# dsforza96/yocto-hair

Measured on AMD Instinct MI355X. Metric: Msamples/sec (whole node), 720x720x1536spp sphere-hairblock; per-pixel L2 vs CPU ref, higher is better.
Workload: dtype f32

## Files before the change

### include/yhair.h

```cpp
#ifndef YHAIR_H_
#define YHAIR_H_

#include <stdint.h>

#ifdef __cplusplus
extern "C" {
#endif

#define YH_OK 0
#define YH_E_INVALID -1
#define YH_E_DEVICE -2
#define YH_E_STATE -3
#define YH_E_IO -4
#define YH_E_SELFTEST -5


typedef struct yh_shape {
  int          num_vertices;
  const float* positions;
  const float* normals;
  const float* radius;
  int          num_lines;
  const int*   lines;
  int          num_triangles;
// ... 40 lines not shown
  float        emission[3];
  int          tex_width, tex_height;
  const float* texels;
} yh_environment;

typedef struct yh_camera {
  float frame[12];
  float lens;
  float film[2];
  float focus;
  float aperture;
} yh_camera;

typedef struct yh_scene_desc {
  int                   num_shapes;
  const yh_shape*       shapes;
  int                   num_materials;
  const yh_material*    materials;
  int                   num_objects;
  const yh_object*      objects;
  int                   num_environments;
  const yh_environment* environments;
  yh_camera             camera;
  int                   num_textures;
  const yh_texture*     textures;
} yh_scene_desc;

enum {
  YH_SHADER_NAIVE    = 0,
  YH_SHADER_PATH     = 1,
  YH_SHADER_EYELIGHT = 2,
  YH_SHADER_NORMAL   = 3,
  YH_SHADER_COUNT    = 4
};

typedef struct yh_trace_params {
  int      resolution;
  int      bounces;
  float    clamp;
  uint64_t seed;
  int      shader;
  int      hair_exact;
} yh_trace_params;

typedef struct yh_workcounts {
  uint64_t samples;
  uint64_t rays;
  uint64_t nodes;
  uint64_t seg_tests;
  uint64_t tri_tests;
  uint64_t hair_shades;
  uint64_t surf_shades;
  uint64_t env_lookups;
  uint64_t env_samples;
  uint64_t cyc_trace, cyc_shade, ticks_tile, wave_iters, wave_steps, lane_steps, lane_iters;
  uint64_t cyc_geom, cyc_sample, cyc_eval, cyc_rest;
  uint64_t branch[10];
} yh_workcounts;

typedef struct yh_context yh_context;


yh_context* yh_create(int device);
void        yh_destroy(yh_context* ctx);
const char* yh_last_error(const yh_context* ctx);
const char* yh_version(void);


int yh_upload_scene(yh_context* ctx, const yh_scene_desc* scene);
int yh_upload_scene_maps(yh_context* ctx, const yh_scene_desc* scene, const yh_material_maps* maps);

int yh_init_state(yh_context* ctx, const yh_trace_params* params);
int yh_image_size(const yh_context* ctx, int* width, int* height);

int yh_set_shard(yh_context* ctx, int rank, int world);

int yh_trace_samples(yh_context* ctx, int nsamples);
int yh_trace_samples_async(yh_context* ctx, int nsamples);
int yh_synchronize(yh_context* ctx);

int yh_download(yh_context* ctx, float* rgba);
int yh_pack_tiles_device(yh_context* ctx, void* device_rgba, int64_t capacity,
    int64_t* count);
int yh_unpack_tiles_device(yh_context* ctx, const void* device_packed,
    int src_rank, int world, void* device_image);
int64_t yh_shard_pixels(const yh_context* ctx, int rank, int world);

int yh_gather_framebuffer(yh_context** contexts, int n, float* rgba);

int yh_download_rng(yh_context* ctx, uint64_t* state_inc);

int yh_trace_samples_counted(yh_context* ctx, int nsamples, yh_workcounts* out);

int yh_last_trace_ms(const yh_context* ctx, float* ms, int* launches);

int yh_launch_shape(const yh_context* ctx);
int yh_kernel_trials(const yh_context* ctx, double* ms_per_sample, int* trials, int count);
int yh_trials_pending(const yh_context* ctx);
int         yh_set_trial_cache_dir(const char* dir);
const char* yh_default_trial_cache_dir(void);

int yh_tile_costs(yh_context* ctx, uint32_t* ticks, int count);
int yh_item_costs(yh_context* ctx, uint32_t* costs, int count);


#define YH_HAIR_BRDF_FLOATS 30

enum {
  YH_LOBE_DIFFUSE            = 0,
  YH_LOBE_SPECULAR           = 1,
  YH_LOBE_METAL              = 2,
  YH_LOBE_TRANSMISSION       = 3,
  YH_LOBE_REFRACTION         = 4,
  YH_LOBE_DELTA_SPECULAR     = 5,
  YH_LOBE_DELTA_METAL        = 6,
  YH_LOBE_DELTA_TRANSMISSION = 7,
  YH_LOBE_DELTA_REFRACTION   = 8,
  YH_LOBE_COUNT              = 9
};
#define YH_SURFACE_BSDF_FLOATS 29

int yh_hair_brdf_batch(yh_context* ctx, int n, const yh_material* materials,
    const float* v, const float* normal, const float* tangent, float* brdf);
int yh_hair_eval_batch(yh_context* ctx, int n, const float* brdf,
    const float* outgoing, const float* incoming, float* f);
int yh_hair_sample_batch(yh_context* ctx, int n, const float* brdf,
    const float* outgoing, const float* rn, float* incoming);
int yh_hair_pdf_batch(yh_context* ctx, int n, const float* brdf,
    const float* outgoing, const float* incoming, float* pdf);
int yh_hair_eval_pdf_batch(yh_context* ctx, int n, const float* brdf,
    const float* outgoing, const float* incoming, float* pdf);

int yh_curves_to_lines(yh_context* ctx, int n, const float* P, const float* width0,
    const float* width1, int base_vertex, float* positions, float* normals,
    float* radius, int* lines);

int yh_bvh_build(int n, const float* boxes, float* nodes, int* primitives);
int yh_bvh_build_wide(int n, const float* boxes, int width, float* slots);

int yh_bvh_build_gpu(yh_context* ctx, int n, const float* boxes, float* nodes, int* primitives);
int yh_bvh_build_wide_gpu(yh_context* ctx, int n, const float* boxes, int width, float* slots);

int yh_surface_lobe_batch(yh_context* ctx, int kind, int n, const float* params,
    const float* normal, const float* outgoing, const float* incoming,
    const float* rn, float* out);
int yh_surface_bsdf_batch(yh_context* ctx, int n, const yh_material* materials,
    const float* normal, const float* outgoing, const float* incoming,
    const float* rn, float* out);
int yh_intersect_batch(yh_context* ctx, int n, const float* rays, int* object,
    int* element, float* uv, float* distance);

int yh_selftest(yh_context* ctx, int which, float* worst);

typedef struct yh_scene_file yh_scene_file;
yh_scene_file*       yh_scene_load(const char* json_path, const char* camera,
          char* error, int error_len);
const yh_scene_desc* yh_scene_get(const yh_scene_file* scene);
const yh_material_maps* yh_scene_get_maps(const yh_scene_file* scene);
void                 yh_scene_free(yh_scene_file* scene);
int yh_save_image(const char* path, int width, int height, const float* rgba,
    char* error, int error_len);

#ifdef __cplusplus
}
#endif
#endif
```

### yocto-hair_amd/csrc/dev_hair.h

```cpp
#ifndef YH_DEV_HAIR_H_
#define YH_DEV_HAIR_H_
#include "dev_math.h"

namespace yhd {

constexpr int p_max = 3;

struct hair_hit {
  float h, gamma_o;
  frame w2b;
};

#ifndef YH_HAIR_FAST
#define YH_HAIR_FAST 1
#endif
#define YH_FAST_DIV YH_HAIR_FAST
#define YH_FAST_EXP 0
#define YH_FAST_LOG YH_HAIR_FAST
#define YH_FAST_TRIG YH_HAIR_FAST
#define YH_FAST_ASIN YH_HAIR_FAST
YH_DEV float h_rcp(float x) { return YH_FAST_DIV ? __builtin_amdgcn_rcpf(x) : 1 / x; }
YH_DEV float h_div(float a, float b) { return YH_FAST_DIV ? a * __builtin_amdgcn_rcpf(b) : a / b; }
YH_DEV float h_div_n(float a, float b) {
  if (!YH_FAST_DIV) return a / b;
  float r = __builtin_amdgcn_rcpf(b);
  r       = __builtin_fmaf(__builtin_fmaf(-b, r, 1.0f), r, r);
  return a * r;
}
YH_DEV float h_sqrt(float x) { return YH_FAST_DIV ? __builtin_amdgcn_sqrtf(x) : sqrtf(x); }
YH_DEV float h_exp(float x) { return YH_FAST_EXP ? __builtin_amdgcn_exp2f(x * 1.44269504f) : expf(x); }
YH_DEV float h_log(float x) { return YH_FAST_LOG ? __builtin_amdgcn_logf(x) * 0.693147181f : logf(x); }
YH_DEV float h_sin(float x) { return YH_FAST_TRIG ? __builtin_amdgcn_sinf(x * 0.159154943f) : sinf(x); }
YH_DEV float h_cos(float x) { return YH_FAST_TRIG ? __builtin_amdgcn_cosf(x * 0.159154943f) : cosf(x); }
YH_DEV float h_cos_turns(float t) { return YH_FAST_TRIG ? __builtin_amdgcn_cosf(t) : cosf(2 * pif * t); }
YH_DEV float h_asin(float x) { return YH_FAST_ASIN ? asinf(x) : (float)asin((double)x); }
YH_DEV f3    h_normalize(f3 a) {
  if (!YH_FAST_DIV) return normalize(a);
  float l2 = dot(a, a);
  return l2 != 0 ? a * __builtin_amdgcn_rsqf(l2) : a;
}
YH_DEV f3 h_div(f3 a, float b) { float r = h_rcp(b); return YH_FAST_DIV ? a * r : a / b; }
YH_DEV f3 h_transform_direction(const frame& a, f3 b) { return h_normalize(transform_vector(a, b)); }

YH_DEV float d_rcp(float x) { return 1 / x; }
YH_DEV float d_div(float a, float b) { return a / b; }
YH_DEV float d_sqrt(float x) { return sqrtf(x); }
YH_DEV float d_safe_sqrt(float x) { return d_sqrt(fmax_(0.0f, x)); }
YH_DEV float d_log(float x) { return logf(x); }
YH_DEV float d_sin(float x) { return sinf(x); }
YH_DEV float d_cos(float x) { return cosf(x); }
YH_DEV float d_cos_turns(float t) { return cosf(2 * pif * t); }
YH_DEV f3    d_transform_direction(const frame& a, f3 b) { return normalize(transform_vector(a, b)); }

YH_DEV float sqr(float v) { return v * v; }
YH_DEV float safe_asin(float x) { return h_asin(fclamp(x, -1.0f, 1.0f)); }
YH_DEV float safe_sqrt(float x) { return h_sqrt(fmax_(0.0f, x)); }
YH_DEV float exact_safe_sqrt(float x) { return sqrtf(fmax_(0.0f, x)); }

template <bool QUAD = false>
YH_DEV hair_hit hair_setup(float v, f3 normal, f3 tangent) {
  hair_hit hh;
  hh.h       = -1 + 2 * v;
  hh.gamma_o = safe_asin(hh.h);
  f3 z       = QUAD ? quad_normalize(normal) : normalize(normal);
  f3 x       = QUAD ? quad_orthonormalize(tangent, z) : orthonormalize(tangent, z);
  f3 y       = QUAD ? quad_normalize(cross(z, x)) : normalize(cross(z, x));
  hh.w2b     = transpose_rot(frame{x, y, z, mk3(0.0f)});
  return hh;
}

YH_DEV float i0(float x) {
  const float den[10] = {1.0f, 4.0f, 64.0f, 2304.0f, 147456.0f, 14745600.0f,
      2123366400.0f, 416179814400.0f, 106542032486400.0f, 34519618525593600.0f};
  float val = 0, x2i = 1;
#pragma unroll
  for (int i = 0; i < 10; i++) {
    val += YH_FAST_DIV ? x2i * (1.0f / den[i]) : x2i / den[i];
    x2i *= x * x;
  }
  return val;
}
YH_DEV float log_i0(float x) {
  if (x > 12)
    return x + 0.5f * (-logf(2 * pif) + logf(1 / x) + 1 / (8 * x));
  else
    return logf(i0(x));
}
YH_DEV float mp(const yhd_material& m, int p, float cos_theta_i, float cos_theta_o,
    float sin_theta_i, float sin_theta_o) {
  float v = m.v[p];
  float a = cos_theta_i * cos_theta_o / v;
  float b = sin_theta_i * sin_theta_o / v;
  if (v <= 0.1f) {
    return h_exp(log_i0(a) - b - m.inv_v[p] + 0.6931f + m.log_inv_2v[p]);
  } else {
    if (YH_HAIR_FAST) return h_div(h_exp(-b) * i0(a), (float)m.mp_den[p]);
    return (float)((double)(expf(-b) * i0(a)) / m.mp_den[p]);
  }
}
YH_DEV float fresnel_dielectric_cos(float eta, float cosw_) {
  float cosw  = fabs_(cosw_);
  float sin2  = 1 - cosw * cosw;
  float eta2  = eta * eta;
  float cos2t = 1 - sin2 / eta2;
  if (cos2t < 0) return 1;
  float t0 = sqrtf(cos2t);
  float t1 = eta * t0;
  float t2 = eta * cosw;
  float rs = (cosw - t1) / (cosw + t1);
  float rp = (t0 - t2) / (t0 + t2);
  return (rs * rs + rp * rp) / 2;
}
YH_DEV float h_fresnel_dielectric_cos(float eta, float cosw_) {
  float cosw  = fabs_(cosw_);
  float sin2  = 1 - cosw * cosw;
  float eta2  = eta * eta;
  float cos2t = 1 - h_div(sin2, eta2);
  if (cos2t < 0) return 1;
  float t0 = h_sqrt(cos2t);
  float t1 = eta * t0;
  float t2 = eta * cosw;
  float rs = h_div(cosw - t1, cosw + t1);
  float rp = h_div(t0 - t2, t0 + t2);
  return (rs * rs + rp * rp) / 2;
}
YH_DEV void ap(float cos_theta_o, float eta, float h, f3 T, f3 out[p_max + 1]) {
  float cos_gamma_o = safe_sqrt(1 - h * h);
  float cos_theta   = cos_theta_o * cos_gamma_o;
  float f = h_fresnel_dielectric_cos(eta, 0.0f * 0.0f + 0.0f * 0.0f + 1.0f * cos_theta);
  out[0]  = mk3(f);
  out[1]  = sqr(1 - f) * T;
  out[2]  = out[1] * T * f;
  f3 den  = mk3(1.f) - T * f;
  f3 num  = out[2] * f * T;
  out[3]  = f3{h_div(num.x, den.x), h_div(num.y, den.y), h_div(num.z, den.z)};
}
YH_DEV f3 transmittance(const yhd_material& m, float h, float sin_theta_o, float cos_theta_o,
    float& gamma_t) {
  float sin_theta_t = h_div(sin_theta_o, m.eta);
  float cos_theta_t = safe_sqrt(1 - sqr(sin_theta_t));
  float etap        = d_div(d_sqrt(m.eta * m.eta - sqr(sin_theta_o)), cos_theta_o);
  float sin_gamma_t = d_div(h, etap);
  float cos_gamma_t = safe_sqrt(1 - sqr(sin_gamma_t));
  gamma_t           = safe_asin(sin_gamma_t);
  float k           = h_div_n(2 * cos_gamma_t, cos_theta_t);
  f3    sa          = ld3(m.sigma_a);
  return f3{h_exp(-sa.x * k), h_exp(-sa.y * k), h_exp(-sa.z * k)};
}
YH_DEV float phi_fn(int p, float gamma_o, float gamma_t) {
  return 2 * p * gamma_t - 2 * gamma_o + p * pif;
}
YH_DEV float np(const yhd_material& m, float phi, int p, float gamma_o, float gamma_t) {
  float dphi = phi - phi_fn(p, gamma_o, gamma_t);
  while (dphi > pif) dphi -= 2 * pif;
  while (dphi < -pif) dphi += 2 * pif;
  float x = fabs_(dphi);
  float e = h_exp(-h_div_n(x, m.s));
  return h_div(h_div(e, m.s * sqr(1 + e)), m.tl_norm);
}
YH_DEV void tilt(const yhd_material& m, int p, float sin_theta_o, float cos_theta_o,
    float& sin_theta_op, float& cos_theta_op) {
  if (p == 0) {
    sin_theta_op = sin_theta_o * m.cos_2k_alpha[1] - cos_theta_o * m.sin_2k_alpha[1];
    cos_theta_op = cos_theta_o * m.cos_2k_alpha[1] + sin_theta_o * m.sin_2k_alpha[1];
  } else if (p == 1) {
    sin_theta_op = sin_theta_o * m.cos_2k_alpha[0] + cos_theta_o * m.sin_2k_alpha[0];
    cos_theta_op = cos_theta_o * m.cos_2k_alpha[0] - sin_theta_o * m.sin_2k_alpha[0];
  } else if (p == 2) {
    sin_theta_op = sin_theta_o * m.cos_2k_alpha[2] + cos_theta_o * m.sin_2k_alpha[2];
    cos_theta_op = cos_theta_o * m.cos_2k_alpha[2] - sin_theta_o * m.sin_2k_alpha[2];
  } else {
    sin_theta_op = sin_theta_o;
    cos_theta_op = cos_theta_o;
  }
}
YH_DEV void compute_ap_pdf(const yhd_material& m, float h, float cos_theta_o,
    float ap_pdf[p_max + 1]) {
  float sin_theta_o = safe_sqrt(1 - cos_theta_o * cos_theta_o);
  float gamma_t;
  f3    T = transmittance(m, h, sin_theta_o, cos_theta_o, gamma_t);
  f3    apv[p_max + 1];
  ap(cos_theta_o, m.eta, h, T, apv);
  float sum_y = 0.0f;
#pragma unroll
  for (int i = 0; i <= p_max; i++) sum_y += luminance(apv[i]);
#pragma unroll
  for (int i = 0; i <= p_max; i++) ap_pdf[i] = h_div(luminance(apv[i]), sum_y);
}

template <bool WANT_F, bool WANT_PDF>
YH_DEV void hair_eval_pdf(const yhd_material& m, const hair_hit& hh, f3 outgoing_, f3 incoming_,
    f3& f, float& pdf) {
  f3    outgoing    = transform_direction(hh.w2b, outgoing_);
  f3    incoming    = transform_direction(hh.w2b, incoming_);
  float sin_theta_o = outgoing.x;
  float cos_theta_o = exact_safe_sqrt(1 - sqr(sin_theta_o));
  float phi_o       = atan2f(outgoing.z, outgoing.y);
  float sin_theta_i = incoming.x;
  float cos_theta_i = exact_safe_sqrt(1 - sqr(sin_theta_i));
  float phi_i       = atan2f(incoming.z, incoming.y);
  float gamma_t;
  f3    T   = transmittance(m, hh.h, sin_theta_o, cos_theta_o, gamma_t);
  float phi = phi_i - phi_o;
  f3    apv[p_max + 1];
  float ap_pdf[p_max + 1];
  if (WANT_F) ap(cos_theta_o, m.eta, hh.h, T, apv);
  if (WANT_PDF) compute_ap_pdf(m, hh.h, cos_theta_o, ap_pdf);
  f   = mk3(0.0f);
  pdf = 0.0f;
#pragma unroll
  for (int p = 0; p < p_max; p++) {
    float sin_theta_op, cos_theta_op;
    tilt(m, p, sin_theta_o, cos_theta_o, sin_theta_op, cos_theta_op);
    cos_theta_op = fabs_(cos_theta_op);
    float mpv    = mp(m, p, cos_theta_i, cos_theta_op, sin_theta_i, sin_theta_op);
    float npv    = np(m, phi, p, hh.gamma_o, gamma_t);
    if (WANT_F) f = f + mpv * apv[p] * npv;
    if (WANT_PDF) pdf += mpv * ap_pdf[p] * npv;
  }
  float mpl = mp(m, p_max, cos_theta_i, cos_theta_o, sin_theta_i, sin_theta_o);
  if (WANT_F) f = f + h_div(mpl * apv[p_max], 2 * pif);
  if (WANT_PDF) pdf += mpl * ap_pdf[p_max] * (1 / (2 * pif));
}

struct hair_out {
  float sin_theta_o, cos_theta_o, phi_o, gamma_t;
  f3    ap0, ap1, ap2, ap3;
  float pdf0, pdf1, pdf2, pdf3;
};
template <bool QUAD = false>
YH_DEV hair_out hair_prepare(const yhd_material& m, const hair_hit& hh, f3 outgoing_) {
  hair_out o;
  f3 outgoing   = QUAD ? quad_normalize(transform_vector(hh.w2b, outgoing_)) : transform_direction(hh.w2b, outgoing_);
  o.sin_theta_o = outgoing.x;
  o.cos_theta_o = exact_safe_sqrt(1 - sqr(o.sin_theta_o));
  o.phi_o       = atan2f(outgoing.z, outgoing.y);
  if (QUAD) {
    const bool for_pdf = (__lane_id() & 2u) != 0;
    float      st      = for_pdf ? safe_sqrt(1 - o.cos_theta_o * o.cos_theta_o) : o.sin_theta_o;
    float      gt;
    f3         T = transmittance(m, hh.h, st, o.cos_theta_o, gt);
    f3         a[p_max + 1];
    ap(o.cos_theta_o, m.eta, hh.h, T, a);
    float l0 = luminance(a[0]), l1 = luminance(a[1]), l2 = luminance(a[2]), l3 = luminance(a[3]);
    float sum_y = 0.0f + l0 + l1 + l2 + l3;
    o.gamma_t = quad_bcast_f<0>(gt);
    o.ap0 = f3{quad_bcast_f<0>(a[0].x), quad_bcast_f<0>(a[0].y), quad_bcast_f<0>(a[0].z)};
    o.ap1 = f3{quad_bcast_f<0>(a[1].x), quad_bcast_f<0>(a[1].y), quad_bcast_f<0>(a[1].z)};
    o.ap2 = f3{quad_bcast_f<0>(a[2].x), quad_bcast_f<0>(a[2].y), quad_bcast_f<0>(a[2].z)};
    o.ap3 = f3{quad_bcast_f<0>(a[3].x), quad_bcast_f<0>(a[3].y), quad_bcast_f<0>(a[3].z)};
    o.pdf0 = quad_bcast_f<2>(h_div(l0, sum_y)), o.pdf1 = quad_bcast_f<2>(h_div(l1, sum_y));
    o.pdf2 = quad_bcast_f<2>(h_div(l2, sum_y)), o.pdf3 = quad_bcast_f<2>(h_div(l3, sum_y));
    return o;
  }
  f3 T          = transmittance(m, hh.h, o.sin_theta_o, o.cos_theta_o, o.gamma_t);
  f3    apv[p_max + 1];
  float ap_pdf[p_max + 1];
  ap(o.cos_theta_o, m.eta, hh.h, T, apv);
  compute_ap_pdf(m, hh.h, o.cos_theta_o, ap_pdf);
  o.ap0 = apv[0], o.ap1 = apv[1], o.ap2 = apv[2], o.ap3 = apv[3];
  o.pdf0 = ap_pdf[0], o.pdf1 = ap_pdf[1], o.pdf2 = ap_pdf[2], o.pdf3 = ap_pdf[3];
  return o;
}

YH_DEV void hair_eval_pdf_quad(const yhd_material& m, const hair_hit& hh, const hair_out& ho, f3 incoming_,
    f3& f, float& pdf) {
  const int p       = (int)(__lane_id() & 3u);
  f3    incoming    = quad_normalize(transform_vector(hh.w2b, incoming_));
  float sin_theta_o = ho.sin_theta_o, cos_theta_o = ho.cos_theta_o;
  float sin_theta_i = incoming.x;
  float cos_theta_i = exact_safe_sqrt(1 - sqr(sin_theta_i));
  float phi_i       = atan2f(incoming.z, incoming.y);
  float phi         = phi_i - ho.phi_o;
  float sin_theta_op, cos_theta_op;
  tilt(m, p, sin_theta_o, cos_theta_o, sin_theta_op, cos_theta_op);
  if (p < p_max) cos_theta_op = fabs_(cos_theta_op);
  float mpv  = mp(m, p, cos_theta_i, cos_theta_op, sin_theta_i, sin_theta_op);
  float npv  = p < p_max ? np(m, phi, p, hh.gamma_o, ho.gamma_t) : 0.0f;
  const f3    a0 = ho.ap0, a1 = ho.ap1, a2 = ho.ap2, a3 = ho.ap3;
  const float q0 = ho.pdf0, q1 = ho.pdf1, q2 = ho.pdf2, q3 = ho.pdf3;
  const bool  is0 = p == 0, is1 = p == 1, is2 = p == 2;
  f3    apq  = f3{is0 ? a0.x : is1 ? a1.x : is2 ? a2.x : a3.x, is0 ? a0.y : is1 ? a1.y : is2 ? a2.y : a3.y,
      is0 ? a0.z : is1 ? a1.z : is2 ? a2.z : a3.z};
  float appq = is0 ? q0 : is1 ? q1 : is2 ? q2 : q3;
  f3    tf   = p < p_max ? mpv * apq * npv : h_div(mpv * apq, 2 * pif);
  float tp   = p < p_max ? mpv * appq * npv : mpv * appq * (1 / (2 * pif));
  f   = mk3(0.0f);
  pdf = 0.0f;
  f   = f + f3{quad_bcast_f<0>(tf.x), quad_bcast_f<0>(tf.y), quad_bcast_f<0>(tf.z)};
  pdf += quad_bcast_f<0>(tp);
  f   = f + f3{quad_bcast_f<1>(tf.x), quad_bcast_f<1>(tf.y), quad_bcast_f<1>(tf.z)};
  pdf += quad_bcast_f<1>(tp);
  f   = f + f3{quad_bcast_f<2>(tf.x), quad_bcast_f<2>(tf.y), quad_bcast_f<2>(tf.z)};
  pdf += quad_bcast_f<2>(tp);
  f   = f + f3{quad_bcast_f<3>(tf.x), quad_bcast_f<3>(tf.y), quad_bcast_f<3>(tf.z)};
  pdf += quad_bcast_f<3>(tp);
}
YH_DEV void hair_eval_pdf_lane(const yhd_material& m, const hair_hit& hh, const hair_out& ho, f3 incoming_,
    f3& f, float& pdf) {
  f3    incoming    = normalize(transform_vector(hh.w2b, incoming_));
  float sin_theta_o = ho.sin_theta_o, cos_theta_o = ho.cos_theta_o;
  float sin_theta_i = incoming.x;
  float cos_theta_i = exact_safe_sqrt(1 - sqr(sin_theta_i));
  float phi_i       = atan2f(incoming.z, incoming.y);
  float phi         = phi_i - ho.phi_o;
  f   = mk3(0.0f);
  pdf = 0.0f;
  const f3    apv[p_max]  = {ho.ap0, ho.ap1, ho.ap2};
  const float appv[p_max] = {ho.pdf0, ho.pdf1, ho.pdf2};
#pragma unroll
  for (int p = 0; p < p_max; p++) {
    float sin_theta_op, cos_theta_op;
    tilt(m, p, sin_theta_o, cos_theta_o, sin_theta_op, cos_theta_op);
    cos_theta_op = fabs_(cos_theta_op);
    float mpv    = mp(m, p, cos_theta_i, cos_theta_op, sin_theta_i, sin_theta_op);
    float npv    = np(m, phi, p, hh.gamma_o, ho.gamma_t);
    f            = f + mpv * apv[p] * npv;
    pdf += mpv * appv[p] * npv;
  }
  float mpl = mp(m, p_max, cos_theta_i, cos_theta_o, sin_theta_i, sin_theta_o);
  f         = f + h_div(mpl * ho.ap3, 2 * pif);
  pdf += mpl * ho.pdf3 * (1 / (2 * pif));
}
YH_DEV void hair_eval_pdf_quad(const yhd_material& m, const hair_hit& hh, f3 outgoing_, f3 incoming_,
    f3& f, float& pdf) {
  hair_out ho = hair_prepare<true>(m, hh, outgoing_);
  hair_eval_pdf_quad(m, hh, ho, incoming_, f, pdf);
}

YH_DEV uint32_t compact1by1(uint32_t x) {
  x &= 0x55555555;
  x = (x ^ (x >> 1)) & 0x33333333;
  x = (x ^ (x >> 2)) & 0x0f0f0f0f;
  x = (x ^ (x >> 4)) & 0x00ff00ff;
  x = (x ^ (x >> 8)) & 0x0000ffff;
  return x;
}
YH_DEV void demux_float(float f, float& a, float& b) {
  uint64_t v = (uint64_t)(f * 4294967296.0f);
  a          = (float)compact1by1((uint32_t)v) / 65536.0f;
  b          = (float)compact1by1((uint32_t)(v >> 1)) / 65536.0f;
}

YH_DEV f3 hair_sample(const yhd_material& m, const hair_hit& hh, const hair_out& ho, float rnx, float rny) {
  float sin_theta_o = ho.sin_theta_o, cos_theta_o = ho.cos_theta_o, phi_o = ho.phi_o;
  float u00, u01, u10, u11;
  demux_float(rnx, u00, u01);
  demux_float(rny, u10, u11);
  int   p  = 0;
  float u1 = u00 - ho.pdf0, u2 = u1 - ho.pdf1;
  if (!(u00 < ho.pdf0)) p = !(u1 < ho.pdf1) ? (!(u2 < ho.pdf2) ? 3 : 2) : 1;
  float sin_theta_op, cos_theta_op;
  tilt(m, p, sin_theta_o, cos_theta_o, sin_theta_op, cos_theta_op);
  u10 = fmax_(u10, 1e-5f);
  float vp = 0, em2v = 0;
  vp   = p == 0 ? m.v[0] : p == 1 ? m.v[1] : m.v[2];
  em2v = p == 0 ? m.exp_m2_inv_v[0] : p == 1 ? m.exp_m2_inv_v[1] : m.exp_m2_inv_v[2];
  float cos_theta   = 1 + vp * d_log(u10 + (1 - u10) * em2v);
  float sin_theta   = d_safe_sqrt(1 - sqr(cos_theta));
  float cos_phi     = d_cos_turns(u11);
  float sin_theta_i = -cos_theta * sin_theta_op + sin_theta * cos_phi * cos_theta_op;
  float cos_theta_i = d_safe_sqrt(1 - sqr(sin_theta_i));
  float dphi;
  if (p < p_max) {
    float x = -m.s * d_log(d_rcp(u01 * m.tl_norm + m.tl_cdf_a) - 1);
    dphi    = phi_fn(p, hh.gamma_o, ho.gamma_t) + fclamp(x, -pif, pif);
  } else {
    dphi = 2 * pif * u01;
  }
  float phi_i    = phi_o + dphi;
  f3    incoming = f3{sin_theta_i, cos_theta_i * d_cos(phi_i), cos_theta_i * d_sin(phi_i)};
  return d_transform_direction(transpose_rot(hh.w2b), incoming);
}
YH_DEV f3 hair_sample(const yhd_material& m, const hair_hit& hh, f3 outgoing_, float rnx, float rny) {
  hair_out ho = hair_prepare(m, hh, outgoing_);
  return hair_sample(m, hh, ho, rnx, rny);
}

YH_DEV void derive_material(yhd_material& m) {
#pragma unroll
  for (int p = 0; p <= p_max; p++) {
    m.inv_v[p]        = 1 / m.v[p];
    m.log_inv_2v[p]   = logf(1 / (2 * m.v[p]));
    m.exp_m2_inv_v[p] = expf(-2 / m.v[p]);
    m.mp_den[p]       = sinh((double)(1 / m.v[p])) * 2 * m.v[p];
  }
  float cb   = 1 / (1 + expf(-pif / m.s));
  float ca   = 1 / (1 + expf(-(-pif) / m.s));
  m.tl_cdf_a = ca;
  m.tl_norm  = cb - ca;
}

}
#endif
```

### yocto-hair_amd/csrc/dev_path.h

```cpp
#ifndef YH_DEV_PATH_H_
#define YH_DEV_PATH_H_
#include "dev_hair.h"
#include "dev_surface.h"
#include "dev_trace.h"
#if YH_LANE
#include "dev_lane.h"
#endif

namespace yhd {

YH_DEV ray_t sample_camera(const yhd_camera& cam, int i, int j, int w, int h, float pu, float pv,
    float lu, float lv) {
  const unsigned int ql = __lane_id() & 3u;
  float uvq = (ql == 0 ? (float)i + pu : (float)j + pv) / (ql == 0 ? (float)w : (float)h);
  float uvx = quad_bcast_f<0>(uvq), uvy = quad_bcast_f<1>(uvq);
  f3    q  = {cam.film_x * (0.5f - uvx), cam.film_y * (uvy - 0.5f), cam.lens};
  f3    dc = -quad_normalize(q);
  f3    e  = mk3(0.0f);
  if (cam.aperture != 0) {
    float r   = sqrtf(lv);
    float phi = 2 * pif * lu;
    float lx = cosf(phi) * r, ly = sinf(phi) * r;
    e = f3{lx * cam.aperture / 2, ly * cam.aperture / 2, 0};
  }
  f3    p  = quad_div(dc * cam.focus, fabs_(dc.z));
  f3    d  = quad_normalize(p - e);
  frame f  = ldframe(cam.frame);
  return mkray(transform_point(f, e), quad_normalize(transform_vector(f, d)));
}

YH_DEV ray_t sample_camera_lane(const yhd_camera& cam, int i, int j, int w, int h, float pu, float pv, float lu, float lv) {
  float uvx = ((float)i + pu) / (float)w, uvy = ((float)j + pv) / (float)h;
  f3    q   = {cam.film_x * (0.5f - uvx), cam.film_y * (uvy - 0.5f), cam.lens};
  f3    dc  = -normalize(q);
  f3    e   = mk3(0.0f);
  if (cam.aperture != 0) {
    float r   = sqrtf(lv);
    float phi = 2 * pif * lu;
    float lx = cosf(phi) * r, ly = sinf(phi) * r;
    e = f3{lx * cam.aperture / 2, ly * cam.aperture / 2, 0};
  }
  f3    p = (dc * cam.focus) / fabs_(dc.z);
  f3    d = normalize(p - e);
  frame f = ldframe(cam.frame);
  return mkray(transform_point(f, e), normalize(transform_vector(f, d)));
}

YH_DEV f3 transform_normal(const frame& a, f3 b) { return normalize(transform_vector(a, b)); }
YH_DEV f3 quad_transform_normal(const frame& a, f3 b) { return quad_normalize(transform_vector(a, b)); }

YH_DEV f3 eval_position(const yhd_scene& sc, const yhd_object& o, int element, float u, float v) {
  frame    fr = ldframe(o.frame);
  yhd_int4 e  = sc.elems[o.elem_base + element];
  if (o.kind == YH_KIND_TRIANGLES) {
    f3 p0 = xyz(sc.vpos[o.vert_base + e.x]), p1 = xyz(sc.vpos[o.vert_base + e.y]),
       p2 = xyz(sc.vpos[o.vert_base + e.z]);
    return transform_point(fr, p0 * (1 - u - v) + p1 * u + p2 * v);
  } else {
    f3 p0 = xyz(sc.vpos[o.vert_base + e.x]), p1 = xyz(sc.vpos[o.vert_base + e.y]);
    return transform_point(fr, p0 * (1 - u) + p1 * u);
  }
}

struct hit_geom {
  f3 position, normal, element_normal;
};
YH_DEV hit_geom eval_hit(const yhd_scene& sc, const yhd_object& o, int slot, float u, float v) {
  frame    fr = ldframe(o.frame);
  hit_geom g;
  if (o.kind == YH_KIND_TRIANGLES) {
    const yhd_float4* rec = sc.prims + (size_t)o.prim_base + (size_t)slot * 6;
    f3 p0 = xyz(ldg4(rec)), p1 = xyz(ldg4(rec + 1)), p2 = xyz(ldg4(rec + 2));
    g.position       = transform_point(fr, p0 * (1 - u - v) + p1 * u + p2 * v);
    g.element_normal = quad_transform_normal(fr, quad_normalize(cross(p1 - p0, p2 - p0)));
    if (o.has_normals) {
      f3 n0 = xyz(ldg4(rec + 3)), n1 = xyz(ldg4(rec + 4)), n2 = xyz(ldg4(rec + 5));
      g.normal = quad_transform_normal(fr, quad_normalize(n0 * (1 - u - v) + n1 * u + n2 * v));
    } else {
      g.normal = g.element_normal;
    }
  } else {
    const yhd_float4* rec = sc.prims + (size_t)o.prim_base + (size_t)slot * 4;
    f3 p0 = xyz(ldg4(rec)), p1 = xyz(ldg4(rec + 1));
    g.position       = transform_point(fr, p0 * (1 - u) + p1 * u);
    g.element_normal = quad_transform_normal(fr, quad_normalize(p1 - p0));
    if (o.has_normals) {
      f3 n0 = xyz(ldg4(rec + 2)), n1 = xyz(ldg4(rec + 3));
      g.normal = quad_transform_normal(fr, quad_normalize(n0 * (1 - u) + n1 * u));
    } else {
      g.normal = g.element_normal;
    }
  }
  return g;
}

YH_DEV f3 eval_env_texture(const yhd_scene& sc, const yhd_environment& env, float u_, float v_) {
  if (env.tex_w == 0) return mk3(1.0f);
  int   sx = env.tex_w, sy = env.tex_h;
  float s = fmodf(u_, 1.0f) * sx;
  if (s < 0) s += sx;
  float t = fmodf(v_, 1.0f) * sy;
  if (t < 0) t += sy;
  int   i = iclamp((int)s, 0, sx - 1), j = iclamp((int)t, 0, sy - 1);
  int   ii = (i + 1) % sx, jj = (j + 1) % sy;
  float u = s - i, v = t - j;
  const yhd_float4* tx = sc.env_texels + env.texel_base;
  f3 a = xyz(tx[(size_t)j * sx + i]), b = xyz(tx[(size_t)jj * sx + i]);
  f3 c = xyz(tx[(size_t)j * sx + ii]), d = xyz(tx[(size_t)jj * sx + ii]);
  return a * (1 - u) * (1 - v) + b * (1 - u) * v + c * u * (1 - v) + d * u * v;
}
template <bool COUNT>
YH_DEV f3 eval_environment(const trace_ctx& tc, f3 dir) {
  const yhd_scene& sc = *tc.sc;
  f3 emission = mk3(0.0f);
  for (int k = 0; k < sc.num_environments; k++) {
    const yhd_environment& env = sc.environments[k];
    if (COUNT) count_quad<COUNT>(tc.stats->envl);
    if (env.tex_w == 0) {
      emission = emission + ld3(env.emission) * mk3(1.0f);
      continue;
    }
    f3    wl = transform_direction(ldframe(env.inv_frame), dir);
    float tx = atan2f(wl.z, wl.x) / (2 * pif);
    float ty = acosf(fclamp(wl.y, -1.0f, 1.0f)) / pif;
    if (tx < 0) tx += 1;
    emission = emission + ld3(env.emission) * eval_env_texture(sc, env, tx, ty);
  }
  return emission;
}

template <typename P>
YH_DEV int cdf_upper_bound(P cdf, int lo, int len, float r) {
  while (len > 0) {
    int half = len >> 1;
    if (!(r < cdf[lo + half])) {
      lo += half + 1;
      len -= half + 1;
    } else {
      len = half;
    }
  }
  return lo;
}
template <typename P>
YH_DEV int sample_discrete_cdf(P cdf, int n, float r) {
  float back = cdf[n - 1];
  r          = fclamp(r * back, 0.0f, back - 0.00001f);
  return iclamp(cdf_upper_bound(cdf, 0, n, r), 0, n - 1);
}
YH_DEV int sample_discrete_cdf_indexed(const float* cdf, int n, const YH_LDS float* tab, int K, int S, float r) {
  float back = tab[K - 1];
  r          = fclamp(r * back, 0.0f, back - 0.00001f);
  int k      = cdf_upper_bound(tab, 0, K, r);
  if (k >= K) return n - 1;
  int lo = k * S;
  return iclamp(cdf_upper_bound(cdf, lo, min(S, n - lo), r), 0, n - 1);
}

YH_DEV void object_frames(const trace_ctx& tc, int object, frame& fr, frame& inv) {
  if (tc.lds_scene) {
    const YH_LDS v4f* ob = tc.lds_scene + YH_OBJECT_F4 * object;
    v4f a = ob[0], b = ob[1], c = ob[2], d = ob[3], e = ob[4], g = ob[5];
    fr.x = {a.x, a.y, a.z}, fr.y = {a.w, b.x, b.y}, fr.z = {b.z, b.w, c.x}, fr.o = {c.y, c.z, c.w};
    inv.x = {d.x, d.y, d.z}, inv.y = {d.w, e.x, e.y}, inv.z = {e.z, e.w, g.x}, inv.o = {g.y, g.z, g.w};
  } else {
    const yhd_object& o = tc.sc->objects[object];
    fr = ldframe(o.frame), inv = ldframe(o.inv_frame);
  }
}
YH_DEV bool small_light_hit(const YH_LDS v4f* L, const frame& inv, f3 ro, f3 rd, int& slot, float& uu, float& vv) {
  f3  lo = transform_point(inv, ro), ld = transform_vector(inv, rd);
  f3  ldinv = quad_rcp(ld);
  v4f b0 = L[0], b1 = L[1];
  if (!intersect_bbox(lo, ldinv, ray_eps, flt_max, xyz(b0), xyz(b1))) return false;
  const int num  = __float_as_int(b0.w);
  float     tmax = flt_max;
  bool      hit  = false;
  for (int i = 0; i < num; i++) {
    float u = 0, v = 0, d = 0;
    if (intersect_triangle(lo, ld, ray_eps, tmax, xyz(L[2 + 3 * i]), xyz(L[3 + 3 * i]), xyz(L[4 + 3 * i]), u, v, d)) hit = true, slot = i, uu = u, vv = v, tmax = d;
  }
  return hit;
}

template <bool COUNT, bool BIG_LIGHTS>
YH_DEV f3 sample_lights(const trace_ctx& tc, f3 position, float rl, float rel, float ruvx,
    float ruvy) {
  const yhd_scene& sc = *tc.sc;
  int n        = sc.num_lights;
  int light_id = iclamp((int)(rl * n), 0, n - 1);
  const yhd_light& light = sc.lights[light_id];
  if (light.object >= 0 && (!BIG_LIGHTS || (light.small_base >= 0 && tc.lds_lights))) {
    const YH_LDS v4f* L = tc.lds_lights + light.small_base;
    int   element = sample_discrete_cdf((const YH_LDS float*)(L + 14), light.cdf_count, rel);
    int   rec     = 0;
    for (int i = 1; i < __float_as_int(L[0].w); i++)
      if (__float_as_int(L[2 + 3 * i].w) == element) rec = i;
    float su = sqrtf(ruvx);
    float u = 1 - su, v = ruvy * su;
    frame fr, inv;
    object_frames(tc, light.object, fr, inv);
    f3 p0 = xyz(L[2 + 3 * rec]), p1 = xyz(L[3 + 3 * rec]), p2 = xyz(L[4 + 3 * rec]);
    f3 lposition = transform_point(fr, p0 * (1 - u - v) + p1 * u + p2 * v);
    return normalize(lposition - position);
  } else if (BIG_LIGHTS && light.object >= 0) {
    int   element = sample_discrete_cdf(sc.light_cdf + light.cdf_base, light.cdf_count, rel);
    float su      = sqrtf(ruvx);
    float u = 1 - su, v = ruvy * su;
    f3 lposition = eval_position(sc, sc.objects[light.object], element, u, v);
    return normalize(lposition - position);
  } else if (light.environment >= 0) {
    const yhd_environment& env = sc.environments[light.environment];
    if (env.tex_w) {
      if (COUNT) count_quad<COUNT>(tc.stats->envs);
      int   idx = (tc.lds_envtab && light_id == sc.env_tab_light)
                      ? sample_discrete_cdf_indexed(sc.light_cdf + light.cdf_base, light.cdf_count, tc.lds_envtab, sc.env_tab_k, sc.env_tab_stride, rel)
                      : sample_discrete_cdf(sc.light_cdf + light.cdf_base, light.cdf_count, rel);
      float ux  = (idx % env.tex_w + 0.5f) / env.tex_w;
      float uy  = (idx / env.tex_w + 0.5f) / env.tex_h;
      return transform_direction(ldframe(env.frame),
          f3{cosf(ux * 2 * pif) * sinf(uy * pif), cosf(uy * pif), sinf(ux * 2 * pif) * sinf(uy * pif)});
    } else {
      float z   = 2 * ruvy - 1;
      float r   = sqrtf(fclamp(1 - z * z, 0.0f, 1.0f));
      float phi = 2 * pif * ruvx;
      return f3{r * cosf(phi), r * sinf(phi), z};
    }
  }
  return mk3(0.0f);
}

template <bool COUNT, int STRIDE, bool BIG_LIGHTS>
YH_DEV float sample_lights_pdf(const trace_ctx& tc, f3 position, f3 direction) {
  const yhd_scene& sc = *tc.sc;
  float pdf = 0.0f;
  for (int k = 0; k < sc.num_lights; k++) {
    const yhd_light& light = sc.lights[k];
    if (light.object >= 0 && (!BIG_LIGHTS || (light.small_base >= 0 && tc.lds_lights))) {
      const YH_LDS v4f* L = tc.lds_lights + light.small_base;
      frame fr, inv;
      object_frames(tc, light.object, fr, inv);
      const float area = L[1].w;
      float lpdf = 0.0f;
      f3    next_position = position;
      for (int bounce = 0; bounce < 100; bounce++) {
        int   slot = 0;
        float uu = 0, vv = 0;
        if (!small_light_hit(L, inv, next_position, direction, slot, uu, vv)) break;
        f3 p0 = xyz(L[2 + 3 * slot]), p1 = xyz(L[3 + 3 * slot]), p2 = xyz(L[4 + 3 * slot]);
        f3 lposition = transform_point(fr, p0 * (1 - uu - vv) + p1 * uu + p2 * vv);
        f3 lnormal   = quad_transform_normal(fr, quad_normalize(cross(p1 - p0, p2 - p0)));
        f3 dp        = lposition - position;
        lpdf += dot(dp, dp) / (fabs_(dot(lnormal, direction)) * area);
        next_position = lposition + direction * 1e-3f;
      }
      pdf += lpdf;
    } else if (BIG_LIGHTS && light.object >= 0) {
      const yhd_object& o = sc.objects[light.object];
      float lpdf = 0.0f;
      f3    next_position = position;
      for (int bounce = 0; bounce < 100; bounce++) {
        hit_t isec;
#if YH_LANE
        isec = lane_trace(tc, *tc.ls, next_position, direction, light.object);
#else
        isec = trace_ray<COUNT, STRIDE>(tc, mkray(next_position, direction), light.object);
#endif
        if (isec.object < 0) break;
        hit_geom lg        = eval_hit(sc, o, isec.slot, isec.u, isec.v);
        f3       lposition = lg.position;
        f3       lnormal   = lg.element_normal;
        float area      = sc.light_cdf[light.cdf_base + light.cdf_count - 1];
        f3    dp        = lposition - position;
        lpdf += dot(dp, dp) / (fabs_(dot(lnormal, direction)) * area);
        next_position = lposition + direction * 1e-3f;
      }
      pdf += lpdf;
    } else if (light.environment >= 0) {
      const yhd_environment& env = sc.environments[light.environment];
      if (env.tex_w) {
        f3    wl = transform_direction(ldframe(env.inv_frame), direction);
        float tx = atan2f(wl.z, wl.x) / (2 * pif);
        float ty = acosf(fclamp(wl.y, -1.0f, 1.0f)) / pif;
        if (tx < 0) tx += 1;
        int   i   = iclamp((int)(tx * env.tex_w), 0, env.tex_w - 1);
        int   j   = iclamp((int)(ty * env.tex_h), 0, env.tex_h - 1);
        int   idx = j * env.tex_w + i;
        const float* cdf = sc.light_cdf + light.cdf_base;
        float prob = (idx == 0 ? cdf[0] : cdf[idx] - cdf[idx - 1]) / cdf[light.cdf_count - 1];
        float angle = (2 * pif / env.tex_w) * (pif / env.tex_h) * sinf(pif * (j + 0.5f) / env.tex_h);
        pdf += prob / angle;
      } else {
        pdf += 1 / (4 * pif);
      }
    }
  }
  pdf *= (float)1 / (float)sc.num_lights;
  return pdf;
}

#if YH_LANE
struct lane_lights_pdf_result {
  float pdf;
  int   base;
};
__device__ __attribute__((noinline)) lane_lights_pdf_result lane_lights_pdf_general(const yhd_scene* sc, const YH_LDS v4f* lds_scene, const YH_LDS v4f* lds_lights,
    const YH_LDS float* lds_envtab, YH_LDS unsigned int* lds, unsigned int* ovf, int sp, int base, f3 position, f3 direction) {
  trace_ctx tc;
  tc.sc = sc, tc.sc_dev = sc, tc.lds_stack = nullptr, tc.lds_scene = lds_scene, tc.stats = nullptr;
  tc.lds_lights = lds_lights, tc.lds_envtab = lds_envtab, tc.lds_mats = nullptr;
  lane_stack s;
  s.lds = lds, s.ovf = ovf, s.sp = sp, s.base = base;
  tc.ls = &s;
  const float pdf = sample_lights_pdf<false, 64, true>(tc, position, direction);
  return lane_lights_pdf_result{pdf, s.base};
}
template <bool GENERAL>
YH_DEV float lane_lights_pdf(const trace_ctx& tc, f3 position, f3 direction) {
  if constexpr (GENERAL) {
    const lane_lights_pdf_result r = lane_lights_pdf_general(tc.sc_dev, tc.lds_scene, tc.lds_lights, tc.lds_envtab, tc.ls->lds, tc.ls->ovf, tc.ls->sp, tc.ls->base, position, direction);
    tc.ls->base = r.base;
    return r.pdf;
  } else {
    return sample_lights_pdf<false, 64, false>(tc, position, direction);
  }
}
#endif

struct path_t {
  ray_t ray;
  f3    radiance, weight;
  int   bounce;
  bool  hit;
  bool   in_medium;
  vsdf_t medium;
#if YH_LANE
  yhd_float4* medium_mem;
#endif
};

YH_DEV bool path_continue(path_t& ps, rng_t& rng, int bounces) {
  if (is_zero(ps.weight) || !finite3(ps.weight)) return false;
  if (ps.bounce > 3) {
    float rr_prob = fmin_(0.99f, hmax(ps.weight));
    if (rand1f(rng) >= rr_prob) return false;
    ps.weight = ps.weight * (1 / rr_prob);
  }
  ps.bounce++;
  return ps.bounce < bounces;
}

YH_DEV void eval_texcoord(const yhd_scene& sc, const yhd_object& o, const hit_t& isec, float& tu, float& tv) {
  tu = isec.u, tv = isec.v;
  if (!o.has_texcoords) return;
  const bool lines   = o.kind == YH_KIND_LINES;
  int        element = __float_as_int(lines ? sc.prims[(size_t)o.prim_base + (size_t)isec.slot * 4 + 2].w
                                            : sc.prims[(size_t)o.prim_base + (size_t)isec.slot * 6].w);
  yhd_int4   e       = sc.elems[o.elem_base + element];
  const float* t0 = sc.vtex + 2 * (size_t)(o.vert_base + e.x);
  const float* t1 = sc.vtex + 2 * (size_t)(o.vert_base + e.y);
  if (lines) {
    tu = t0[0] * (1 - isec.u) + t1[0] * isec.u, tv = t0[1] * (1 - isec.u) + t1[1] * isec.u;
  } else {
    const float* t2 = sc.vtex + 2 * (size_t)(o.vert_base + e.z);
    tu = t0[0] * (1 - isec.u - isec.v) + t1[0] * isec.u + t2[0] * isec.v;
    tv = t0[1] * (1 - isec.u - isec.v) + t1[1] * isec.u + t2[1] * isec.v;
  }
}

YH_DEV surface_maps eval_maps(const yhd_scene& sc, const yhd_maps& mp, float tu, float tv) {
  surface_maps f;
  if (mp.specular_tex >= 0) f.specular = eval_texture(sc, mp.specular_tex, true, tu, tv).x;
  if (mp.metallic_tex >= 0) f.metallic = eval_texture(sc, mp.metallic_tex, true, tu, tv).x;
  if (mp.roughness_tex >= 0) f.roughness = eval_texture(sc, mp.roughness_tex, true, tu, tv).x;
  if (mp.opacity_tex >= 0) {
    f3 o      = eval_texture(sc, mp.opacity_tex, true, tu, tv);
    f.opacity = mp.opacity * ((o.x + o.y + o.z) / 3);
    if (f.opacity > 0.999f) f.opacity = 1;
  }
  return f;
}

YH_DEV f3 eval_normalmap(const yhd_scene& sc, const yhd_object& o, const hit_t& isec, f3 normal, int normal_tex, float tu, float tv) {
  f3 nm = eval_texture(sc, normal_tex, true, tu, tv);
  nm    = f3{-1 + 2 * nm.x, -1 + 2 * nm.y, -1 + 2 * nm.z};
  f3 tgu = mk3(0.0f), tgv = mk3(0.0f);
  if (o.has_texcoords) {
    const yhd_float4* rec = sc.prims + (size_t)o.prim_base + (size_t)isec.slot * 6;
    const yhd_float4  r0  = rec[0];
    yhd_int4          e   = sc.elems[o.elem_base + __float_as_int(r0.w)];
    f3 p0 = xyz(r0), p1 = xyz(rec[1]), p2 = xyz(rec[2]);
    const float* t0 = sc.vtex + 2 * (size_t)(o.vert_base + e.x);
    const float* t1 = sc.vtex + 2 * (size_t)(o.vert_base + e.y);
    const float* t2 = sc.vtex + 2 * (size_t)(o.vert_base + e.z);
    f3    p = p1 - p0, q = p2 - p0;
    float sx = t1[0] - t0[0], sy = t2[0] - t0[0];
    float tx = t1[1] - t0[1], ty = t2[1] - t0[1];
    float div = sx * ty - sy * tx;
    f3    u = {1, 0, 0}, v = {0, 1, 0};
    if (div != 0) {
      u = f3{ty * p.x - tx * q.x, ty * p.y - tx * q.y, ty * p.z - tx * q.z} / div;
      v = f3{sx * q.x - sy * p.x, sx * q.y - sy * p.y, sx * q.z - sy * p.z} / div;
    }
    frame fr = ldframe(o.frame);
    tgu = transform_direction(fr, u), tgv = transform_direction(fr, v);
  }
  frame f;
  f.z = normal;
  f.x = orthonormalize(tgu, f.z);
  f.y = normalize(cross(f.z, f.x));
  nm.y *= dot(f.y, tgv) < 0 ? 1.0f : -1.0f;
  return normalize(transform_vector(f, nm));
}

struct hit_maps {
  float        tu, tv;
  bool         have_tc;
  surface_maps f;
};
YH_DEV hit_maps eval_hit_maps(const yhd_scene& sc, const yhd_object& o, const hit_t& isec, bool mapped, f3& nrm) {
  hit_maps h;
  h.tu = isec.u, h.tv = isec.v, h.have_tc = false;
  if (!mapped || !sc.maps) return h;
  const yhd_maps mp = sc.maps[o.material];
  if (!mp.any) return h;
  eval_texcoord(sc, o, isec, h.tu, h.tv);
  h.have_tc = true;
  if (mp.normal_tex >= 0 && o.kind == YH_KIND_TRIANGLES) nrm = eval_normalmap(sc, o, isec, nrm, mp.normal_tex, h.tu, h.tv);
  h.f = eval_maps(sc, mp, h.tu, h.tv);
  return h;
}

YH_DEV void medium_crossing(const yhd_scene& sc, path_t& ps, const yhd_material& mat, f3 normal, f3 outgoing,
    f3 incoming, f3 color_tex, float emission_tex_x, float tu, float tv) {
  if (!mat.has_volume || !(dot(normal, outgoing) * dot(normal, incoming) < 0)) return;
  if (!ps.in_medium) {
    if (mat.color_tex >= 0 || mat.emission_tex >= 0) {
      f3    base         = ld3(mat.color) * color_tex;
      float transmission = mat.transmission * emission_tex_x;
      ps.medium.density  = mk3(0.0f);
      if (transmission) {
        f3 c = {fclamp(base.x, 0.0001f, 1.0f), fclamp(base.y, 0.0001f, 1.0f), fclamp(base.z, 0.0001f, 1.0f)};
        ps.medium.density = -f3{logf(c.x), logf(c.y), logf(c.z)} / mat.trdepth;
      }
    } else {
      ps.medium.density = ld3(mat.vol_density);
    }
    ps.medium.scatter    = ld3(mat.vol_scatter) * eval_texture(sc, mat.scattering_tex, false, tu, tv);
    ps.medium.anisotropy = mat.vol_anisotropy;
#if YH_LANE
    ps.medium_mem[0] = yhd_float4{ps.medium.density.x, ps.medium.density.y, ps.medium.density.z, ps.medium.anisotropy};
    ps.medium_mem[1] = yhd_float4{ps.medium.scatter.x, ps.medium.scatter.y, ps.medium.scatter.z, 0.0f};
#endif
  }
  ps.in_medium = !ps.in_medium;
}

template <bool COUNT, int STRIDE, bool GENERAL>
YH_DEV bool path_step(const trace_ctx& tc, path_t& ps, const hit_t& isec, rng_t& rng, int bounces) {
  const yhd_scene& sc = *tc.sc;
  unsigned long long k0 = 0, k1 = 0, k2 = 0, k3 = 0;
  if (COUNT) k0 = clock64();
#if YH_LANE
  if (isec.object < 0) return false;
#else
  if (isec.object < 0) {
    ps.radiance = ps.radiance + ps.weight * eval_environment<COUNT>(tc, ps.ray.d);
    if (COUNT) tc.stats->c_rest += clock64() - k0;
    return false;
  }
#endif
  f3 outgoing = -ps.ray.d;
  if (GENERAL && ps.in_medium) {
#if YH_LANE
    {
      const yhd_float4 m0 = ps.medium_mem[0], m1 = ps.medium_mem[1];
      ps.medium.density = f3{m0.x, m0.y, m0.z}, ps.medium.anisotropy = m0.w, ps.medium.scatter = f3{m1.x, m1.y, m1.z};
    }
#endif
    float rd = rand1f(rng), rl = rand1f(rng);
    float dist = sample_transmittance(ps.medium.density, isec.distance, rl, rd);
    ps.weight  = ps.weight * (eval_transmittance(ps.medium.density, dist) /
                                sample_transmittance_pdf(ps.medium.density, dist, isec.distance));
    if (dist < isec.distance) {
      f3 position = ps.ray.o + ps.ray.d * dist;
      ps.hit      = true;
      f3 incoming;
      if (rand1f(rng) < 0.5f) {
        float rnx = rand1f(rng), rny = rand1f(rng);
        float rnl = rand1f(rng);
        (void)rnl;
        incoming = sample_scattering(ps.medium, outgoing, rnx, rny);
      } else {
        float ruvx = rand1f(rng), ruvy = rand1f(rng);
        float rel = rand1f(rng);
        float rl2 = rand1f(rng);
        incoming  = sample_lights<COUNT, GENERAL>(tc, position, rl2, rel, ruvx, ruvy);
      }
      f3    f         = eval_scattering(ps.medium, outgoing, incoming);
      float pdf       = sample_scattering_pdf(ps.medium, outgoing, incoming);
#if YH_LANE
      float light_pdf = lane_lights_pdf<GENERAL>(tc, position, incoming);
#else
      float light_pdf = sample_lights_pdf<COUNT, STRIDE, GENERAL>(tc, position, incoming);
#endif
      ps.weight = ps.weight * (f / (0.5f * pdf + 0.5f * light_pdf));
      ps.ray    = mkray(position, incoming);
      if (COUNT) tc.stats->c_rest += clock64() - k0;
      return path_continue(ps, rng, bounces);
    }
  }
  constexpr bool from_lds = !GENERAL && (YH_LANE || STRIDE != 64);
  const yhd_object&   o   = !from_lds ? sc.objects[isec.object] : *(const yhd_object*)(const YH_LDS yhd_object*)(tc.lds_scene + YH_OBJECT_F4 * isec.object);
  const yhd_material& mat = !from_lds ? sc.materials[o.material] : *(const yhd_material*)(const YH_LDS yhd_material*)(tc.lds_mats + YH_MATERIAL_F4 * o.material);
  hit_geom hg = eval_hit(sc, o, isec.slot, isec.u, isec.v);
  f3 position = hg.position;
  f3 nrm      = hg.normal;
  hit_maps hm;
  if constexpr (GENERAL) hm = eval_hit_maps(sc, o, isec, !mat.plain, nrm);
  f3 normal;
  bool is_hair = o.kind == YH_KIND_LINES;
  if (is_hair) {
    normal = quad_orthonormalize(outgoing, nrm);
  } else {
    normal = (!mat.thin || dot(nrm, outgoing) >= 0) ? nrm : -nrm;
  }
  if (COUNT) count_quad<COUNT>(is_hair ? tc.stats->hair : tc.stats->surf);
  const bool     general = GENERAL && !mat.plain;
  surface_brdf_t sb;
  float          tu = isec.u, tv = isec.v, etex_x = 1.0f;
  f3             ctex = mk3(1.0f), etex = mk3(1.0f);
  if (general) {
    if constexpr (GENERAL) tu = hm.tu, tv = hm.tv;
    if (mat.color_tex >= 0 || mat.emission_tex >= 0 || mat.scattering_tex >= 0) {
      if constexpr (GENERAL) {
        if (!hm.have_tc) eval_texcoord(sc, o, isec, tu, tv);
      }
      ctex = eval_texture(sc, mat.color_tex, false, tu, tv);
      if (mat.emission_tex >= 0) {
        etex   = eval_texture(sc, mat.emission_tex, false, tu, tv);
        etex_x = eval_texture(sc, mat.emission_tex, true, tu, tv).x;
      }
    }
    if constexpr (GENERAL) sb = surface_brdf(mat, normal, outgoing, ctex, etex_x, hm.f);
    else sb = surface_brdf(mat, normal, outgoing, ctex, etex_x);
    if (sb.opacity < 1 && rand1f(rng) >= sb.opacity) {
      ps.ray = mkray(position + ps.ray.d * 1e-2f, ps.ray.d);
      if (COUNT) tc.stats->c_rest += clock64() - k0;
      return true;
    }
  }
  ps.hit      = true;
  ps.radiance = ps.radiance + ps.weight * (ld3(mat.emission) * etex);
  if (general && is_delta(sb)) {
    f3    incoming = surface_sample_delta(sb, normal, outgoing, rand1f(rng));
    f3    brdfcos;
    float pdf;
    surface_eval_pdf_delta(sb, normal, outgoing, incoming, brdfcos, pdf);
    ps.weight = ps.weight * (brdfcos / pdf);
    medium_crossing(sc, ps, mat, normal, outgoing, incoming, ctex, etex_x, tu, tv);
    ps.ray    = mkray(position, incoming);
    if (COUNT) tc.stats->c_rest += clock64() - k0;
    return path_continue(ps, rng, bounces);
  }
  hair_hit hh;
  hair_out ho;
  if (is_hair) {
    hh = hair_setup<!YH_LANE>(isec.v, normal, nrm);
    ho = hair_prepare<!YH_LANE>(mat, hh, outgoing);
  }

  if (COUNT) k1 = clock64(), tc.stats->c_geom += k1 - k0;
  f3 incoming;
  if (rand1f(rng) < 0.5f) {
    float rnx = rand1f(rng), rny = rand1f(rng);
    float rnl = rand1f(rng);
    if (is_hair) {
      incoming = hair_sample(mat, hh, ho, rnx, rny);
    } else if (general) {
      incoming = surface_sample(sb, normal, outgoing, rnl, rnx, rny);
    } else {
      incoming = mk3(0.0f);
      if (mat.diffuse_pdf != 0 && rnl < 0.0f + mat.diffuse_pdf) {
        if (!(dot(normal, outgoing) <= 0)) incoming = sample_hemisphere_cos(normal, rnx, rny);
      }
    }
  } else {
    float ruvx = rand1f(rng), ruvy = rand1f(rng);
    float rel = rand1f(rng);
    float rl  = rand1f(rng);
    incoming  = sample_lights<COUNT, GENERAL>(tc, position, rl, rel, ruvx, ruvy);
  }
  if (COUNT) k2 = clock64(), tc.stats->c_sample += k2 - k1;
  f3    brdfcos;
  float brdf_pdf;
  if (is_hair) {
#if YH_LANE
    hair_eval_pdf_lane(mat, hh, ho, incoming, brdfcos, brdf_pdf);
#else
    hair_eval_pdf_quad(mat, hh, ho, incoming, brdfcos, brdf_pdf);
#endif
  } else if (general) {
    surface_eval_pdf(sb, normal, outgoing, incoming, brdfcos, brdf_pdf);
  } else {
    brdfcos  = mk3(0.0f);
    brdf_pdf = 0.0f;
    f3 diffuse = ld3(mat.color);
    bool below = dot(normal, incoming) <= 0 || dot(normal, outgoing) <= 0;
    if (!is_zero(diffuse)) {
      f3 lobe = below ? mk3(0.0f) : mk3(1.0f) / pif * dot(normal, incoming);
      brdfcos = brdfcos + diffuse * lobe;
    }
    if (mat.diffuse_pdf != 0) {
      float lobe = 0.0f;
      if (!below) {
        float cosw = dot(normal, incoming);
        lobe       = (cosw <= 0) ? 0 : cosw / pif;
      }
      brdf_pdf += mat.diffuse_pdf * lobe;
    }
  }
  if (COUNT) k3 = clock64(), tc.stats->c_eval += k3 - k2;
#if YH_LANE
  float light_pdf = lane_lights_pdf<GENERAL>(tc, position, incoming);
#else
  float light_pdf = sample_lights_pdf<COUNT, STRIDE, GENERAL>(tc, position, incoming);
#endif
  ps.weight = ps.weight * (brdfcos / (0.5f * brdf_pdf + 0.5f * light_pdf));
  if (general) medium_crossing(sc, ps, mat, normal, outgoing, incoming, ctex, etex_x, tu, tv);
  ps.ray    = mkray(position, incoming);
  if (COUNT) tc.stats->c_rest += clock64() - k3;
  return path_continue(ps, rng, bounces);
}

template <bool COUNT, int STRIDE, int SHADER>
YH_DEV bool shade_step(const trace_ctx& tc, path_t& ps, const hit_t& isec, rng_t& rng, int bounces) {
  const yhd_scene& sc = *tc.sc;
  if (isec.object < 0) {
    f3 env = eval_environment<COUNT>(tc, ps.ray.d);
    if (SHADER == YH_SHADER_NORMAL) ps.radiance = env, ps.hit = true;
    else ps.radiance = ps.radiance + ps.weight * env;
    return false;
  }
  f3 outgoing = -ps.ray.d;
  const yhd_object&   o   = sc.objects[isec.object];
  const yhd_material& mat = sc.materials[o.material];
  hit_geom hg = eval_hit(sc, o, isec.slot, isec.u, isec.v);
  f3   position = hg.position, nrm = hg.normal;
  const hit_maps hm = eval_hit_maps(sc, o, isec, true, nrm);
  bool is_hair  = o.kind == YH_KIND_LINES;
  f3   normal   = is_hair ? quad_orthonormalize(outgoing, nrm) : ((!mat.thin || dot(nrm, outgoing) >= 0) ? nrm : -nrm);
  if (SHADER == YH_SHADER_NORMAL) {
    ps.radiance = normal * 0.5f + mk3(0.5f), ps.hit = true;
    return false;
  }
  if (COUNT) count_quad<COUNT>(is_hair ? tc.stats->hair : tc.stats->surf);
  float tu = hm.tu, tv = hm.tv, etex_x = 1.0f;
  f3    ctex = mk3(1.0f), etex = mk3(1.0f);
  if (mat.color_tex >= 0 || mat.emission_tex >= 0) {
    if (!hm.have_tc) eval_texcoord(sc, o, isec, tu, tv);
    ctex = eval_texture(sc, mat.color_tex, false, tu, tv);
    if (mat.emission_tex >= 0) {
      etex   = eval_texture(sc, mat.emission_tex, false, tu, tv);
      etex_x = eval_texture(sc, mat.emission_tex, true, tu, tv).x;
    }
  }
  surface_brdf_t sb = surface_brdf(mat, normal, outgoing, ctex, etex_x, hm.f);
  if (sb.opacity < 1 && rand1f(rng) >= sb.opacity) {
    ps.ray = mkray(position + ps.ray.d * 1e-2f, ps.ray.d);
    return true;
  }
  ps.hit      = true;
  ps.radiance = ps.radiance + ps.weight * (ld3(mat.emission) * etex);
  hair_hit hh;
  hair_out ho;
  if (is_hair) {
    hh = hair_setup<true>(isec.v, normal, nrm);
    ho = hair_prepare<true>(mat, hh, outgoing);
  }
  f3    incoming, brdfcos;
  float pdf;
  if (SHADER == YH_SHADER_EYELIGHT) {
    if (is_hair) hair_eval_pdf_quad(mat, hh, ho, outgoing, brdfcos, pdf);
    else surface_eval_pdf(sb, normal, outgoing, outgoing, brdfcos, pdf);
    ps.radiance = ps.radiance + ps.weight * pif * brdfcos;
    if (!is_delta(sb)) return false;
    incoming = surface_sample_delta(sb, normal, outgoing, rand1f(rng));
    surface_eval_pdf_delta(sb, normal, outgoing, incoming, brdfcos, pdf);
    ps.weight = ps.weight * (brdfcos / pdf);
    if (is_zero(ps.weight) || !finite3(ps.weight)) return false;
    ps.ray = mkray(position, incoming);
    ps.bounce++;
    return ps.bounce < (bounces > 4 ? bounces : 4);
  }
  if (!is_delta(sb)) {
    float rnx = rand1f(rng), rny = rand1f(rng);
    float rnl = rand1f(rng);
    if (is_hair) {
      incoming = hair_sample(mat, hh, ho, rnx, rny);
      hair_eval_pdf_quad(mat, hh, ho, incoming, brdfcos, pdf);
    } else {
      incoming = surface_sample(sb, normal, outgoing, rnl, rnx, rny);
      surface_eval_pdf(sb, normal, outgoing, incoming, brdfcos, pdf);
    }
  } else {
    incoming = surface_sample_delta(sb, normal, outgoing, rand1f(rng));
    surface_eval_pdf_delta(sb, normal, outgoing, incoming, brdfcos, pdf);
  }
  ps.weight = ps.weight * (brdfcos / pdf);
  ps.ray    = mkray(position, incoming);
  return path_continue(ps, rng, bounces);
}

YH_DEV void path_begin(const yhd_camera& cam, path_t& ps, rng_t& rng, int i, int j, int w, int h) {
  float lu = rand1f(rng), lv = rand1f(rng);
  float pu = rand1f(rng), pv = rand1f(rng);
  ps.ray      = sample_camera(cam, i, j, w, h, pu, pv, lu, lv);
  ps.radiance = mk3(0.0f), ps.weight = mk3(1.0f);
  ps.bounce   = 0;
  ps.hit      = false;
  ps.in_medium = false;
}
YH_DEV void path_end(const path_t& ps, float clamp, yhd_float4& acc) {
  f3 rgb = ps.radiance;
  if (!finite3(rgb)) rgb = mk3(0.0f);
  if (hmax(rgb) > clamp) rgb = rgb * (clamp / hmax(rgb));
  acc.x += rgb.x, acc.y += rgb.y, acc.z += rgb.z, acc.w += ps.hit ? 1.0f : 0.0f;
}

}
#endif
```

### yocto-hair_amd/csrc/kernels.hip

```cpp
#include <hip/hip_runtime.h>

#include <algorithm>
#include <cstdlib>
#include <cstring>

#include "yhair.h"
#include "dev_items.h"

template <int SHADER>
__global__ __launch_bounds__(YH_BLOCK, YH_MIN_WAVES) void k_trace_shader(const yhd_scene sc, const yhd_state st,
    int nsamples, yhd_counters* counters) {
  trace_items<false, true, YH_BLOCK, SHADER>(sc, st, nsamples, counters);
}

__global__ void k_resolve(const yhd_state st, int samples, yhd_float4* image) {
  int lane = threadIdx.x;
  int tile = st.shard_rank + blockIdx.x * st.shard_world;
  int i    = (tile % st.tiles_x) * YH_TILE + (lane & 7);
  int j    = (tile / st.tiles_x) * YH_TILE + (lane >> 3);
  if (i >= st.width || j >= st.height) return;
  size_t     pix = (size_t)j * st.width + i;
  yhd_float4 a   = st.accum[pix];
  float      n   = (float)samples;
  image[pix]     = samples > 0 ? yhd_float4{a.x / n, a.y / n, a.z / n, a.w / n} : yhd_float4{0, 0, 0, 0};
// ... 185 lines not shown
    derive_material(m);
    hair_hit hh = hair_setup(h, f3{0, 0, 1}, f3{1, 0, 0});
    f3 wo = ld3(a.wo);
    if (a.which == 2) {
      float wx = rand1f(rng), wy = rand1f(rng);
      wo = sample_sphere(wx, wy);
    }
    float rx = rand1f(rng), ry = rand1f(rng);
    f3    f;
    float pdf;
    if (a.which == 0) {
      f3 wi = sample_sphere(rx, ry);
      hair_eval_pdf<true, false>(m, hh, wo, wi, f, pdf);
      s0[0] = f.x, s0[1] = f.y, s0[2] = f.z;
    } else {
      f3 wi = hair_sample(m, hh, wo, rx, ry);
      hair_eval_pdf<true, true>(m, hh, wo, wi, f, pdf);
      if (a.which == 1) {
        if (pdf > 0) s0[0] = f.x / pdf, s0[1] = f.y / pdf, s0[2] = f.z / pdf;
      } else if (a.which == 2) {
        if (pdf > 0) dev = fabs_(luminance(f) / pdf - 1);
      } else {
        float li = wi.z * wi.z;
        if (pdf > 0) s0[0] = f.x * li / pdf, s0[1] = f.y * li / pdf, s0[2] = f.z * li / pdf;
        f3 wu = sample_sphere(rx, ry);
        f3 fu;
        hair_eval_pdf<true, false>(m, hh, wo, wu, fu, pdf);
        float lu = wu.z * wu.z;
        s1[0] = fu.x * lu, s1[1] = fu.y * lu, s1[2] = fu.z * lu;
      }
    }
  }
  for (int k = 0; k < 3; k++) {
    double a0 = s0[k], a1 = s1[k];
    for (int off = 32; off > 0; off >>= 1) {
      a0 += __shfl_down(a0, off, 64);
      a1 += __shfl_down(a1, off, 64);
    }
    if ((threadIdx.x & 63) == 0) {
      atomicAdd(&sums[k], a0);
      atomicAdd(&sums[3 + k], a1);
    }
  }
  for (int off = 32; off > 0; off >>= 1) dev = fmaxf(dev, __shfl_down(dev, off, 64));
  if ((threadIdx.x & 63) == 0) atomicMax(worst_bits, __float_as_uint(dev));
}

__global__ void k_surface_lobe(int kind, int n, const float* params, const float* normal, const float* wo_,
    const float* wi_, const float* rn, float* out) {
  int i = blockIdx.x * blockDim.x + threadIdx.x;
  if (i >= n) return;
  const float* q = params + 8 * (size_t)i;
  float ior = q[0], rough = q[1];
  f3    eta = ld3(q + 2), etak = ld3(q + 5);
  f3    nn = ld3(normal + 3 * (size_t)i), wo = ld3(wo_ + 3 * (size_t)i), wi = ld3(wi_ + 3 * (size_t)i);
  float rnl = rn[3 * (size_t)i], rx = rn[3 * (size_t)i + 1], ry = rn[3 * (size_t)i + 2];
  f3    f = mk3(0.0f), w = mk3(0.0f);
  float pdf = 0;
  switch (kind) {
    case 0:
      f = eval_diffuse_reflection(nn, wo, wi), pdf = sample_diffuse_reflection_pdf(nn, wo, wi);
      w = sample_diffuse_reflection(nn, wo, rx, ry);
      break;
    case 1:
      f = eval_microfacet_reflection(ior, rough, nn, wo, wi), pdf = sample_microfacet_reflection_pdf(rough, nn, wo, wi);
      w = sample_microfacet_reflection(rough, nn, wo, rx, ry);
      break;
    case 2:
      f   = eval_microfacet_reflection(eta, etak, rough, nn, wo, wi);
      pdf = sample_microfacet_reflection_pdf(rough, nn, wo, wi);
      w   = sample_microfacet_reflection(rough, nn, wo, rx, ry);
      break;
    case 3:
      f = eval_microfacet_transmission(rough, nn, wo, wi), pdf = sample_microfacet_transmission_pdf(rough, nn, wo, wi);
      w = sample_microfacet_transmission(rough, nn, wo, rx, ry);
      break;
    case 4:
      f   = eval_microfacet_refraction(ior, rough, nn, wo, wi);
      pdf = sample_microfacet_refraction_pdf(ior, rough, nn, wo, wi);
      w   = sample_microfacet_refraction(ior, rough, nn, wo, rnl, rx, ry);
      break;
    case 5:
      f = eval_delta_reflection(ior, nn, wo, wi), pdf = sample_delta_reflection_pdf(nn, wo, wi);
      w = sample_delta_reflection(nn, wo);
      break;
    case 6:
      f = eval_delta_reflection(eta, etak, nn, wo, wi), pdf = sample_delta_reflection_pdf(nn, wo, wi);
      w = sample_delta_reflection(nn, wo);
      break;
    case 7:
      f = eval_delta_transmission(nn, wo, wi), pdf = sample_delta_transmission_pdf(nn, wo, wi);
      w = sample_delta_transmission(nn, wo);
      break;
    case 8:
      f = eval_delta_refraction(ior, nn, wo, wi), pdf = sample_delta_refraction_pdf(ior, nn, wo, wi);
      w = sample_delta_refraction(ior, nn, wo, rnl);
      break;
    default: break;
  }
  float* o = out + 7 * (size_t)i;
  o[0] = f.x, o[1] = f.y, o[2] = f.z, o[3] = pdf, o[4] = w.x, o[5] = w.y, o[6] = w.z;
}
__global__ void k_surface_bsdf(int n, const yhd_material* mats, const float* normal, const float* wo_,
    const float* wi_, const float* rn, float* out) {
  int i = blockIdx.x * blockDim.x + threadIdx.x;
  if (i >= n) return;
  f3    nn = ld3(normal + 3 * (size_t)i), wo = ld3(wo_ + 3 * (size_t)i), wi = ld3(wi_ + 3 * (size_t)i);
  float rnl = rn[3 * (size_t)i], rx = rn[3 * (size_t)i + 1], ry = rn[3 * (size_t)i + 2];
  surface_brdf_t b = surface_brdf(mats[i], nn, wo);
  float* o = out + 29 * (size_t)i;
  f3 lobes[5] = {b.diffuse, b.specular, b.metal, b.transmission, b.refraction};
  for (int k = 0; k < 5; k++) o[3 * k] = lobes[k].x, o[3 * k + 1] = lobes[k].y, o[3 * k + 2] = lobes[k].z;
  o[15] = b.roughness, o[16] = b.opacity;
  o[17] = b.diffuse_pdf, o[18] = b.specular_pdf, o[19] = b.metal_pdf, o[20] = b.transmission_pdf;
  o[21] = b.refraction_pdf;
  f3    f, w;
  float pdf;
  if (!is_delta(b)) {
    surface_eval_pdf(b, nn, wo, wi, f, pdf);
    w = surface_sample(b, nn, wo, rnl, rx, ry);
  } else {
    surface_eval_pdf_delta(b, nn, wo, wi, f, pdf);
    w = surface_sample_delta(b, nn, wo, rnl);
  }
  o[22] = f.x, o[23] = f.y, o[24] = f.z, o[25] = pdf, o[26] = w.x, o[27] = w.y, o[28] = w.z;
}

__global__ void k_curves_to_lines(int n, const float* P, const float* width0, const float* width1, int base_vertex,
    float* positions, float* normals, float* radius, int* lines) {
  long long t = (long long)blockIdx.x * blockDim.x + threadIdx.x;
  if (t >= 5ll * n) return;
  int c = (int)(t / 5), i = (int)(t % 5);
  const float* q = P + 12 * (size_t)c;
  f3 p0 = ld3(q), p1 = ld3(q + 3), p2 = ld3(q + 6), p3 = ld3(q + 9);
  f3    pos, tan;
  float rad;
  if (i == 0) {
    pos = p0, tan = normalize(p1 - p0), rad = width0[c];
  } else if (i == 4) {
    pos = p3, tan = normalize(p3 - p2), rad = width1[c];
  } else {
    float u = (float)i / 4;
    pos = p0 * (1 - u) * (1 - u) * (1 - u) + p1 * 3 * u * (1 - u) * (1 - u) + p2 * 3 * u * u * (1 - u) + p3 * u * u * u;
    tan = normalize((p1 - p0) * 3 * (1 - u) * (1 - u) + (p2 - p1) * 6 * u * (1 - u) + (p3 - p2) * 3 * u * u);
    rad = width0[c] * (1 - u) + width1[c] * u;
  }
  size_t v = (size_t)t;
  positions[3 * v] = pos.x, positions[3 * v + 1] = pos.y, positions[3 * v + 2] = pos.z;
  normals[3 * v] = tan.x, normals[3 * v + 1] = tan.y, normals[3 * v + 2] = tan.z;
  radius[v] = rad;
  if (i < 4) lines[8 * (size_t)c + 2 * i] = base_vertex + (int)t, lines[8 * (size_t)c + 2 * i + 1] = base_vertex + (int)t + 1;
}

extern "C" {

trace_kernel_t yhk_wide_kernel(int counted, int general, int shape);
#define YH_DENSE_WAVES 5
static_assert(yhd_shapes[YH_SHAPE_QUAD].block_threads == YH_BLOCK && yhd_shapes[YH_SHAPE_OCT].block_threads == YH_OCT_BLOCK && yhd_shapes[YH_SHAPE_HEX].block_threads == YH_OCT_BLOCK, "yhd_shapes");
static int shape_block(int shape) { return yhd_shapes[shape].block_threads; }
static int shape_groups(int shape) { return shape_block(shape) / yhd_shapes[shape].lanes_per_path; }
static trace_kernel_t trace_kernel(bool counted, bool general, int shape, int shader = YH_SHADER_PATH) {
  if (shader == YH_SHADER_NAIVE) return k_trace_shader<YH_SHADER_NAIVE>;
  if (shader == YH_SHADER_EYELIGHT) return k_trace_shader<YH_SHADER_EYELIGHT>;
  if (shader == YH_SHADER_NORMAL) return k_trace_shader<YH_SHADER_NORMAL>;
  if (yhd_shapes[shape].kind == YH_SHAPE_KIND_WIDE) return yhk_wide_kernel(counted ? 1 : 0, general ? 1 : 0, shape);
  if (yhd_shapes[shape].kind == YH_SHAPE_KIND_RETIRED) return nullptr;
  if (general && !counted && shape == YH_SHAPE_QUAD_DENSE) return k_trace<false, true, 256, YH_DENSE_WAVES - 1>;
  if (shape == YH_SHAPE_QUAD_DENSE)
    return counted ? (general ? k_trace<true, true, 256, YH_DENSE_WAVES> : k_trace<true, false, 256, YH_DENSE_WAVES>)
                   : (general ? k_trace<false, true, 256, YH_DENSE_WAVES> : k_trace<false, false, 256, YH_DENSE_WAVES>);
  return counted ? (general ? k_trace<true, true, YH_BLOCK, YH_MIN_WAVES> : k_trace<true, false, YH_BLOCK, YH_MIN_WAVES>)
                 : (general ? k_trace<false, true, YH_BLOCK, YH_MIN_WAVES> : k_trace<false, false, YH_BLOCK, YH_MIN_WAVES>);
}
static size_t trace_lds(const yhd_scene* sc, int shape) {
  const int lanes   = yhd_shapes[shape].lanes_per_path;
  const int entries = lanes == 16 ? sc->stack_entries16 : lanes == 8 ? sc->stack_entries8 : sc->stack_entries;
  return (size_t)(entries + YH_HITROWS) * shape_groups(shape) * 4 + (size_t)YHD_LDS_TABLES_F4(sc) * 16;
}
int yhk_trace(const yhd_scene* sc, const yhd_state* st, int nsamples, yhd_counters* counters, int shape,
    int grid_blocks, hipStream_t stream) {
  const bool path  = st->shader == YH_SHADER_PATH;
  if (!path) shape = YH_SHAPE_QUAD;
  if (!path && counters) return (int)hipErrorInvalidValue;
  if ((unsigned)shape >= YH_SHAPES || yhd_shapes[shape].kind == YH_SHAPE_KIND_STREAM || yhd_shapes[shape].kind == YH_SHAPE_KIND_SBS) return (int)hipErrorInvalidValue;
  size_t    lds   = trace_lds(sc, shape);
  trace_kernel_t k     = trace_kernel(counters != nullptr, sc->general_materials != 0, shape, st->shader);
  if (!k) return (int)hipErrorInvalidValue;
  if (lds > 64 * 1024) {
    hipError_t e = hipFuncSetAttribute((const void*)k, hipFuncAttributeMaxDynamicSharedMemorySize, (int)lds);
    if (e != hipSuccess) return (int)e;
  }
  hipLaunchKernelGGL(k, dim3(grid_blocks), dim3(shape_block(shape)), lds, stream, *sc, *st, nsamples, counters);
  return (int)hipGetLastError();
}
int yhk_block_threads(int shape) { return shape_block(shape); }
int yhk_stack_entries(void) { return YH_QSTACK; }
int yhk_trace_lds_bytes(const yhd_scene* sc, int shape) { return (int)trace_lds(sc, shape); }
int yhk_trace_occupancy(int lds_bytes, int general, int shape) {
  int            blocks = 0;
  trace_kernel_t k      = trace_kernel(false, general != 0, shape);
  if (!k) return 0;
  if (lds_bytes > 64 * 1024 &&
      hipFuncSetAttribute((const void*)k, hipFuncAttributeMaxDynamicSharedMemorySize, lds_bytes) != hipSuccess)
    return 0;
  if (hipOccupancyMaxActiveBlocksPerMultiprocessor(&blocks, k, shape_block(shape), lds_bytes) != hipSuccess) return 1;
  return blocks < 1 ? 0 : blocks;
}
int yhk_resolve(const yhd_state* st, int owned_tiles, int samples, void* image, hipStream_t stream) {
  if (owned_tiles) hipLaunchKernelGGL(k_resolve, dim3(owned_tiles), dim3(64), 0, stream, *st, samples, (yhd_float4*)image);
  return (int)hipGetLastError();
}
int yhk_pack(const yhd_state* st, int owned_tiles, int samples, void* packed, hipStream_t stream) {
  if (owned_tiles) hipLaunchKernelGGL(k_pack, dim3(owned_tiles), dim3(64), 0, stream, *st, samples, (yhd_float4*)packed);
  return (int)hipGetLastError();
}
int yhk_unpack(const void* packed, int src_rank, int world, int ntiles_src, int num_tiles_total, int tiles_x,
    int width, int height, void* image, hipStream_t stream) {
  if (ntiles_src)
    hipLaunchKernelGGL(k_unpack, dim3(ntiles_src), dim3(64), 0, stream, (const yhd_float4*)packed, src_rank, world,
        num_tiles_total, tiles_x, width, height, (yhd_float4*)image);
  return (int)hipGetLastError();
}
int yhk_curves_to_lines(int n, const float* P, const float* w0, const float* w1, int base_vertex, float* positions,
    float* normals, float* radius, int* lines, hipStream_t s) {
  long long threads = 5ll * n;
  hipLaunchKernelGGL(k_curves_to_lines, dim3((unsigned)((threads + 255) / 256)), dim3(256), 0, s, n, P, w0, w1, base_vertex,
      positions, normals, radius, lines);
  return (int)hipGetLastError();
}
int yhk_surface_lobe(int kind, int n, const float* params, const float* normal, const float* wo, const float* wi,
    const float* rn, float* out, hipStream_t s) {
  hipLaunchKernelGGL(k_surface_lobe, dim3((n + 255) / 256), dim3(256), 0, s, kind, n, params, normal, wo, wi, rn, out);
  return (int)hipGetLastError();
}
int yhk_surface_bsdf(int n, const void* mats, const float* normal, const float* wo, const float* wi, const float* rn,
    float* out, hipStream_t s) {
  hipLaunchKernelGGL(k_surface_bsdf, dim3((n + 255) / 256), dim3(256), 0, s, n, (const yhd_material*)mats, normal, wo, wi, rn, out);
  return (int)hipGetLastError();
}
int yhk_hair_brdf(int n, const void* mats, const float* v, const float* nrm, const float* tng, float* out, hipStream_t s) {
  hipLaunchKernelGGL(k_hair_brdf, dim3((n + 255) / 256), dim3(256), 0, s, n, (const yh_material_in*)mats, v, nrm, tng, out);
  return (int)hipGetLastError();
}
int yhk_hair_eval(int n, const float* brdf, const float* wo, const float* wi, float* out, hipStream_t s) {
  hipLaunchKernelGGL(k_hair_eval, dim3((n + 63) / 64), dim3(256), 0, s, n, brdf, wo, wi, out);
  return (int)hipGetLastError();
}
int yhk_hair_pdf(int n, const float* brdf, const float* wo, const float* wi, float* out, hipStream_t s) {
  hipLaunchKernelGGL(k_hair_pdf, dim3((n + 63) / 64), dim3(256), 0, s, n, brdf, wo, wi, out);
  return (int)hipGetLastError();
}
int yhk_hair_sample(int n, const float* brdf, const float* wo, const float* rn, float* out, hipStream_t s) {
  hipLaunchKernelGGL(k_hair_sample, dim3((n + 255) / 256), dim3(256), 0, s, n, brdf, wo, rn, out);
  return (int)hipGetLastError();
}
int yhk_intersect(const yhd_scene* sc, int n, const float* rays, int* object, int* element, float* uv, float* dist,
    hipStream_t s) {
  hipLaunchKernelGGL(k_intersect, dim3((n + 63) / 64), dim3(256), 0, s, *sc, n, rays, object, element, uv, dist);
  return (int)hipGetLastError();
}
int yhk_selftest(int which, float beta_m, float beta_n, uint64_t state, uint64_t inc, int count, const float* wo,
    double* sums, unsigned int* worst_bits, hipStream_t s) {
  selftest_args a;
  a.which = which, a.beta_m = beta_m, a.beta_n = beta_n, a.state = state, a.inc = inc, a.count = count;
  a.wo[0] = wo[0], a.wo[1] = wo[1], a.wo[2] = wo[2];
  hipLaunchKernelGGL(k_selftest, dim3((count + 255) / 256), dim3(256), 0, s, a, sums, worst_bits);
  return (int)hipGetLastError();
}
}
```

### yocto-hair_amd/csrc/yh_device.h

```cpp
#ifndef YH_DEVICE_H_
#define YH_DEVICE_H_
#include <stdint.h>

#define YH_KIND_LINES 1
#define YH_KIND_TRIANGLES 2
#define YH_TILE 8
#define YH_MAX_LIGHTS 16
#define YH_MAX_ENVS 4

typedef struct yhd_float4 { float x, y, z, w; } yhd_float4;
typedef struct yhd_int4 { int x, y, z, w; } yhd_int4;

typedef struct yhd_object {
  float frame[12];
  float inv_frame[12];
  int   kind;
  int   node_base;
  int   prim_base;
  int   vert_base;
  int   elem_base;
  int   has_normals;
  int   material;
  int   has_texcoords;
  float wbox_min[4], wbox_max[4];
  int   lane_root, lane_test;
  int   lane_root8, lane_root16;
} yhd_object;
#define YH_OBJECT_F4 11

typedef struct yhd_material {
  float  emission[3];
  float  color[3];
  float  diffuse_pdf;
  int    thin;
  float  sigma_a[3];
  float  alpha, eta;
  float  v[4];
  float  s;
  float  sin_2k_alpha[3], cos_2k_alpha[3];
  float  inv_v[4];
  float  log_inv_2v[4];
  float  exp_m2_inv_v[4];
  double mp_den[4];
  float  tl_cdf_a;
  float  tl_norm;
  int    plain;
  float  specular, metallic, roughness, ior, transmission;
  float  opacity;
  float  meta[3];
  int    has_volume;
  float  vol_density[3];
  float  vol_scatter[3];
  float  vol_anisotropy;
  int    emission_tex, color_tex, scattering_tex;
  float  trdepth;
} yhd_material;

typedef struct yhd_texture {
  int width, height;
  int srgb_base, linear_base;
} yhd_texture;

typedef struct yhd_maps {
  int   specular_tex, metallic_tex, roughness_tex, opacity_tex;
  int   normal_tex;
  int   any;
  float opacity;
  int   pad;
} yhd_maps;

typedef struct yhd_light {
  int object;
  int environment;
  int cdf_base;
  int cdf_count;
  int small_base;
} yhd_light;
#define YH_SMALL_LIGHT_TRIS 4
#define YH_SMALL_LIGHT_F4 15

typedef struct yhd_environment {
  float frame[12];
  float inv_frame[12];
  float emission[3];
  int   tex_w, tex_h;
  int   texel_base;
  int   pad0, pad1;
} yhd_environment;

typedef struct yhd_camera {
  float frame[12];
  float lens, film_x, film_y, focus, aperture;
} yhd_camera;

typedef struct yhd_scene {
  const yhd_maps*   maps;
  const yhd_float4* prims;
  const yhd_float4* vpos;
  const yhd_int4*   elems;
  const yhd_object* objects;
  const yhd_material* materials;
  const yhd_float4* scene_nodes;
  const int*        scene_prims;
  int               num_scene_nodes;
  int               num_objects;
  int               num_lights;
  int               num_environments;
  yhd_light         lights[YH_MAX_LIGHTS];
  yhd_environment   environments[YH_MAX_ENVS];
  const float*      light_cdf;
  const yhd_float4* env_texels;
  const yhd_texture* textures;
  const yhd_float4* tex_texels;
  const float*      vtex;
  yhd_camera        camera;
  int               num_nodes_total;
  int               num_prim_f4;
  int               lds_scene_f4;
  int               general_materials;
  int               stack_entries;
  const yhd_float4* light_table;
  int               light_table_f4;
  int               scene_wide_root;
  const float*      env_tab;
  int               env_tab_light;
  int               env_tab_k, env_tab_stride;
  int               lds_materials;
  int               stack_entries8;
  int               stack_entries16;
  const yhd_float4* lane_blob;
  long long         lane_blob_units;
} yhd_scene;
#define YH_MATERIAL_F4 17
#define YHD_LDS_TABLES_F4(sc) ((sc)->lds_scene_f4 + 5 + (sc)->light_table_f4 + ((sc)->env_tab_k + 3) / 4 + YH_MATERIAL_F4 * (sc)->lds_materials)

typedef struct yhd_state {
  uint64_t*   rng_state;
  uint64_t*   rng_inc;
  yhd_float4* accum;
  const int*  tiles;
  int*        tile_cursor;
  int         num_groups;
  int         group_begin[9];
  unsigned int* tile_cost;
  int         num_tiles;
  int         shader;
  int         launch_shape;
  int         width, height;
  int         tiles_x;
  int         samples_done;
  int         bounces;
  float       clamp;
  int         shard_rank, shard_world;
} yhd_state;

enum yhd_shape {
  YH_SHAPE_QUAD       = 0,
  YH_SHAPE_QUAD_DENSE = 1,
  YH_SHAPE_RETIRED    = 2,
  YH_SHAPE_STREAM     = 3,
  YH_SHAPE_OCT        = 4,
  YH_SHAPE_SBS        = 5,
  YH_SHAPE_HEX        = 6,
  YH_SHAPE_OCT_PAIRS  = 7,
  YH_SHAPE_HEX_GROUPS = 8,
  YH_SHAPES
};
enum yhd_shape_kind { YH_SHAPE_KIND_QUAD, YH_SHAPE_KIND_WIDE, YH_SHAPE_KIND_STREAM, YH_SHAPE_KIND_SBS, YH_SHAPE_KIND_RETIRED };
typedef struct yhd_shape_info {
  const char* name;
  int kind;
  int entries_per_item;
  int block_threads, lanes_per_path;
  int counted_plain, counted_general;
  int fallback;
  int tie_rank;
} yhd_shape_info;
static constexpr yhd_shape_info yhd_shapes[YH_SHAPES] = {
    {"quad",       YH_SHAPE_KIND_QUAD,    1, 512, 4,  1, 1, YH_SHAPE_QUAD, 7},
    {"quad-dense", YH_SHAPE_KIND_QUAD,    1, 256, 4,  1, 1, YH_SHAPE_QUAD, 1},
    {"retired",    YH_SHAPE_KIND_RETIRED, 1, 512, 4,  0, 0, YH_SHAPE_QUAD, 8},
    {"stream",     YH_SHAPE_KIND_STREAM,  1, 256, 1,  0, 0, -1, 0},
    {"oct",        YH_SHAPE_KIND_WIDE,    2, 256, 8,  1, 0, YH_SHAPE_QUAD, 6},
    {"sbs",        YH_SHAPE_KIND_SBS,     1, 512, 4,  0, 0, YH_SHAPE_QUAD, 2},
    {"hex",        YH_SHAPE_KIND_WIDE,    4, 256, 16, 1, 0, YH_SHAPE_QUAD, 5},
    {"oct-pairs",  YH_SHAPE_KIND_WIDE,    2, 256, 8,  0, 0, YH_SHAPE_QUAD, 4},
    {"hex-groups", YH_SHAPE_KIND_WIDE,    4, 256, 16, 0, 0, YH_SHAPE_QUAD, 3},
};

typedef struct yhd_path_slot {
  yhd_float4 ray_o;
  yhd_float4 ray_d;
  yhd_float4 weight;
  yhd_int4   rngw;
  yhd_int4   hit;
  yhd_int4   hit2;
  yhd_float4 radiance;
  yhd_int4   own;
} yhd_path_slot;
typedef struct yhd_stream {
  yhd_path_slot* slots;
  yhd_float4* medium;
  unsigned int* stack_ovf;
  unsigned long long* prof;
  unsigned long long* wave_log;
  const int*  wave_begin;
  int*        wave_fill;
  int         slots_per_wave;
  int         ovf_entries;
  long long   total_slots;
  int         prof_parts_only;
  int         suspend_lanes;
} yhd_stream;

typedef struct yhd_counters {
  unsigned long long samples, rays, nodes, seg, tri, hair, surf, envl, envs;
  unsigned long long cyc_trace, cyc_shade, cyc_tile, wave_iters, wave_steps, lane_steps, lane_iters;
  unsigned long long c_geom, c_sample, c_eval, c_rest;
  unsigned long long branch[10];
} yhd_counters;

#endif
```

### yocto-hair_amd/host/batch_api.cpp

```cpp
#include "context_internal.h"

namespace {
struct Staged {
  std::vector<DevBuf> bufs;
  yh_context*         ctx;
  int                 rc = YH_OK;
  explicit Staged(yh_context* c) : ctx(c) { bufs.reserve(8); }
  void* in(const void* src, size_t bytes) {
    bufs.emplace_back();
    if (rc == YH_OK) rc = upload(ctx, bufs.back(), src, bytes);
    return bufs.back().p;
  }
  void* out(size_t bytes) {
    bufs.emplace_back();
    if (rc == YH_OK) rc = alloc_zero(ctx, bufs.back(), bytes);
    return bufs.back().p;
  }
};
int finish(yh_context* ctx, int launch_err, void* dst, const void* src, size_t bytes) {
  if (launch_err) return fail(ctx, YH_E_DEVICE, "kernel launch: %s", hipGetErrorString((hipError_t)launch_err));
  YH_WAIT(ctx);
  HIPCHK(ctx, hipMemcpy(dst, src, bytes, hipMemcpyDeviceToHost));
  return YH_OK;
}
// ... 85 lines not shown
      memcpy(o + 6, &a, 4), memcpy(o + 7, &c, 4);
    }
  if (primitives && n) memcpy(primitives, tree.primitives.data(), sizeof(int) * (size_t)n);
  return (int)tree.nodes.size();
}

int yh_bvh_build_wide_gpu(yh_context* ctx, int n, const float* boxes, int width, float* slots) {
  if (!ctx || n < 1 || !boxes || (width != 4 && width != 8 && width != 16)) return YH_E_INVALID;
  HIPCHK(ctx, hipSetDevice(ctx->device));
  YH_WAIT(ctx);
  const int L = width == 4 ? 2 : width == 8 ? 3 : 4;
  DevBuf    d_boxes, d_nodes, d_pid, d_flag, d_widx, d_out;
  int       rc;
  if ((rc = upload(ctx, d_boxes, boxes, (size_t)n * 24))) return rc;
  if ((rc = alloc_zero(ctx, d_nodes, ((size_t)2 * n + 1) * 32)) || (rc = alloc_zero(ctx, d_pid, (size_t)n * 4))) return rc;
  int num_nodes = 0, levels = 0, level_first[130], count = 0;
  int e = yhk_bvh_build_resident(n, (const float*)d_boxes.p, (float*)d_nodes.p, (int*)d_pid.p, &num_nodes, &levels, level_first, ctx->stream);
  if (e) return fail(ctx, YH_E_DEVICE, "device BVH build: %s", hipGetErrorString((hipError_t)e));
  if ((rc = alloc_zero(ctx, d_flag, ((size_t)num_nodes + 1) * 4)) || (rc = alloc_zero(ctx, d_widx, ((size_t)num_nodes + 1) * 4))) return rc;
  e = yhk_wide_index(num_nodes, (const float*)d_nodes.p, levels, level_first, L, (unsigned int*)d_flag.p, (unsigned int*)d_widx.p, &count, ctx->stream);
  if (e) return fail(ctx, YH_E_DEVICE, "wide-node index: %s", hipGetErrorString((hipError_t)e));
  if (slots) {
    if ((rc = alloc_zero(ctx, d_out, (size_t)count * width * 32))) return rc;
    e = yhk_wide_collapse(L, num_nodes, (const float*)d_nodes.p, (const unsigned int*)d_flag.p, (const unsigned int*)d_widx.p, 1, 0, 0, d_out.p, ctx->stream);
    if (e) return fail(ctx, YH_E_DEVICE, "wide collapse: %s", hipGetErrorString((hipError_t)e));
    YH_WAIT(ctx);
    HIPCHK(ctx, hipMemcpy(slots, d_out.p, (size_t)count * width * 32, hipMemcpyDeviceToHost));
  }
  return count;
}

int yh_bvh_build_wide(int n, const float* boxes, int width, float* slots) {
  if (n < 0 || (n && !boxes) || (width != 4 && width != 8 && width != 16)) return YH_E_INVALID;
  std::vector<yhh::Box> b((size_t)n);
  for (int i = 0; i < n; i++)
    for (int k = 0; k < 3; k++) b[(size_t)i].min[k] = boxes[6 * (size_t)i + k], b[(size_t)i].max[k] = boxes[6 * (size_t)i + 3 + k];
  yhh::Tree tree;
  yhh::build_bvh(tree, b);
  const void* data  = nullptr;
  size_t      count = 0;
  std::vector<yhh::WideNode>   w4;
  std::vector<yhh::WideNode8>  w8;
  std::vector<yhh::WideNode16> w16;
  if (width == 4) yhh::collapse_wide(tree, w4), data = w4.data(), count = w4.size();
  if (width == 8) yhh::collapse_wide8(tree, w8), data = w8.data(), count = w8.size();
  if (width == 16) yhh::collapse_wide16(tree, w16), data = w16.data(), count = w16.size();
  if (slots && count) memcpy(slots, data, count * (size_t)width * sizeof(yhh::WideSlot));
  return (int)count;
}

int yh_bvh_build(int n, const float* boxes, float* nodes, int* primitives) {
  if (n < 0 || (n && !boxes)) return YH_E_INVALID;
  std::vector<yhh::Box> b((size_t)n);
  for (int i = 0; i < n; i++)
    for (int k = 0; k < 3; k++) b[(size_t)i].min[k] = boxes[6 * (size_t)i + k], b[(size_t)i].max[k] = boxes[6 * (size_t)i + 3 + k];
  yhh::Tree tree;
  yhh::build_bvh(tree, b);
  if (nodes)
    for (size_t i = 0; i < tree.nodes.size(); i++) {
      auto&  nd = tree.nodes[i];
      float* o  = nodes + 8 * i;
      memcpy(o, nd.bbox.min, 12), memcpy(o + 3, nd.bbox.max, 12);
      int a = nd.start, c = (int)nd.num | ((int)nd.internal << 16) | ((int)nd.axis << 24);
      memcpy(o + 6, &a, 4), memcpy(o + 7, &c, 4);
    }
  if (primitives && n) memcpy(primitives, tree.primitives.data(), sizeof(int) * (size_t)n);
  return (int)tree.nodes.size();
}

int yh_surface_lobe_batch(yh_context* ctx, int kind, int n, const float* params, const float* normal,
    const float* outgoing, const float* incoming, const float* rn, float* out) {
  if (!ctx || n < 0 || kind < 0 || kind >= YH_LOBE_COUNT || (n && (!params || !normal || !outgoing || !incoming || !rn || !out)))
    return YH_E_INVALID;
  if (n == 0) return YH_OK;
  HIPCHK(ctx, hipSetDevice(ctx->device));
  Staged s(ctx);
  auto   dp = (float*)s.in(params, 32 * (size_t)n);
  auto   dn = (float*)s.in(normal, 12 * (size_t)n);
  auto   da = (float*)s.in(outgoing, 12 * (size_t)n);
  auto   db = (float*)s.in(incoming, 12 * (size_t)n);
  auto   dr = (float*)s.in(rn, 12 * (size_t)n);
  auto   o  = (float*)s.out(28 * (size_t)n);
  if (s.rc) return s.rc;
  return finish(ctx, yhk_surface_lobe(kind, n, dp, dn, da, db, dr, o, ctx->stream), out, o, 28 * (size_t)n);
}
int yh_surface_bsdf_batch(yh_context* ctx, int n, const yh_material* materials, const float* normal,
    const float* outgoing, const float* incoming, const float* rn, float* out) {
  if (!ctx || n < 0 || (n && (!materials || !normal || !outgoing || !incoming || !rn || !out))) return YH_E_INVALID;
  if (n == 0) return YH_OK;
  HIPCHK(ctx, hipSetDevice(ctx->device));
  std::vector<yhd_material> mats((size_t)n);
  for (int i = 0; i < n; i++) make_material(materials[i], mats[(size_t)i]);
  Staged s(ctx);
  auto   dm = s.in(mats.data(), sizeof(yhd_material) * (size_t)n);
  auto   dn = (float*)s.in(normal, 12 * (size_t)n);
  auto   da = (float*)s.in(outgoing, 12 * (size_t)n);
  auto   db = (float*)s.in(incoming, 12 * (size_t)n);
  auto   dr = (float*)s.in(rn, 12 * (size_t)n);
  auto   o  = (float*)s.out(4 * YH_SURFACE_BSDF_FLOATS * (size_t)n);
  if (s.rc) return s.rc;
  return finish(ctx, yhk_surface_bsdf(n, dm, dn, da, db, dr, o, ctx->stream), out, o, 4 * YH_SURFACE_BSDF_FLOATS * (size_t)n);
}

int yh_intersect_batch(yh_context* ctx, int n, const float* rays, int* object, int* element, float* uv,
    float* distance) {
  if (!ctx || n < 0 || (n && (!rays || !object || !element || !uv || !distance))) return YH_E_INVALID;
  if (!ctx->have_scene) return fail(ctx, YH_E_STATE, "yh_intersect_batch before yh_upload_scene");
  if (n == 0) return YH_OK;
  HIPCHK(ctx, hipSetDevice(ctx->device));
  Staged s(ctx);
  auto   dr = (float*)s.in(rays, 32 * (size_t)n);
  auto   dob = (int*)s.out(4 * (size_t)n);
  auto   del = (int*)s.out(4 * (size_t)n);
  auto   duv = (float*)s.out(8 * (size_t)n);
  auto   dd  = (float*)s.out(4 * (size_t)n);
  if (s.rc) return s.rc;
  const char* mode  = getenv("YHAIR_INTERSECT");
  int         waves = 5;
  bool        lanes = n >= 65536 && lane_kernels_can_address(ctx);
  if (mode && !strcmp(mode, "quad")) lanes = false;
  else if (mode && !strncmp(mode, "lane", 4)) {
    if (!lane_kernels_can_address(ctx))
      return fail(ctx, YH_E_INVALID, "YHAIR_INTERSECT=%s: the one-lane kernel reads the scene's trees through 32-bit byte offsets and this scene's exceed 4 GB", mode);
    lanes = true, waves = std::max(4, std::min(8, atoi(mode + 4)));
  }
  for (int i = 0; lanes && i < n; i++) lanes = rays[8 * (size_t)i + 6] == 1e-4f;
  HIPCHK(ctx, hipEventRecord(ctx->ev0, ctx->stream));
  if (lanes) {
    const int occupancy = std::min(waves, yhk_intersect_lanes_occupancy(&ctx->scene, waves));
    if (occupancy < 1) return fail(ctx, YH_E_DEVICE, "k_intersect_lanes cannot run with its LDS layout on this device");
    const int    grid        = (int)std::max<int64_t>(1, std::min<int64_t>(((int64_t)n + 255) / 256, (int64_t)ctx->num_cus * occupancy));
    const int    ovf_entries = 2 * std::max(8, ctx->stack_need);
    auto         dcur        = (int*)s.out(16);
    auto         dovf        = (unsigned int*)s.out((size_t)grid * 4 * ovf_entries * 64 * 4);
    if (s.rc) return s.rc;
    if (!ctx->d_scene_copy.p) {
      int rc = upload(ctx, ctx->d_scene_copy, &ctx->scene, sizeof(yhd_scene));
      if (rc) return rc;
    }
    int e = yhk_intersect_lanes(&ctx->scene, (const yhd_scene*)ctx->d_scene_copy.p, n, dr, dcur, dovf, ovf_entries, dob, del, duv, dd, waves, grid, ctx->stream);
    if (e) return fail(ctx, YH_E_DEVICE, "k_intersect_lanes launch: %s", hipGetErrorString((hipError_t)e));
  } else {
    int e = yhk_intersect(&ctx->scene, n, dr, dob, del, duv, dd, ctx->stream);
    if (e) return fail(ctx, YH_E_DEVICE, "k_intersect launch: %s", hipGetErrorString((hipError_t)e));
  }
  HIPCHK(ctx, hipEventRecord(ctx->ev1, ctx->stream));
  YH_WAIT(ctx);
  HIPCHK(ctx, hipEventElapsedTime(&ctx->last_ms, ctx->ev0, ctx->ev1));
  ctx->last_launches = 1;
  HIPCHK(ctx, hipMemcpy(object, dob, 4 * (size_t)n, hipMemcpyDeviceToHost));
  HIPCHK(ctx, hipMemcpy(element, del, 4 * (size_t)n, hipMemcpyDeviceToHost));
  HIPCHK(ctx, hipMemcpy(uv, duv, 8 * (size_t)n, hipMemcpyDeviceToHost));
  HIPCHK(ctx, hipMemcpy(distance, dd, 4 * (size_t)n, hipMemcpyDeviceToHost));
  return YH_OK;
}

int yh_selftest(yh_context* ctx, int which, float* worst) {
  if (!ctx) return YH_E_INVALID;
  if (which < 0 || which > 3) return fail(ctx, YH_E_INVALID, "unknown self-test %d", which);
  HIPCHK(ctx, hipSetDevice(ctx->device));
  DevBuf sums, wbits;
  int    rc;
  if ((rc = alloc_zero(ctx, sums, 6 * sizeof(double)))) return rc;
  if ((rc = alloc_zero(ctx, wbits, 4))) return rc;
  auto lum = [](const double* s) { return (float)(0.2126 * s[0] + 0.7152 * s[1] + 0.0722 * s[2]); };
  auto sample_sphere = [](float rx, float ry, float* w) {
    float z = 2 * ry - 1;
    float r = std::sqrt(fmin_(fmax_(1 - z * z, 0.0f), 1.0f));
    float phi = 2 * pif * rx;
    w[0] = r * std::cos(phi), w[1] = r * std::sin(phi), w[2] = z;
  };
  Rng   rng = make_rng(199382389514ULL);
  float wo[3] = {0, 0, 1};
  if (which == 0 || which == 1) {
    float x = rand1f(rng), y = rand1f(rng);
    sample_sphere(x, y, wo);
  }
  bool  ok  = true;
  float dev = 0;
  auto run = [&](float bm, float bn, int count, int per_iter, double* out, float* dmax) -> int {
    HIPCHK(ctx, hipMemsetAsync(sums.p, 0, 6 * sizeof(double), ctx->stream));
    HIPCHK(ctx, hipMemsetAsync(wbits.p, 0, 4, ctx->stream));
    int e = yhk_selftest(which, bm, bn, rng.state, rng.inc, count, wo, (double*)sums.p, (unsigned int*)wbits.p, ctx->stream);
    if (e) return fail(ctx, YH_E_DEVICE, "k_selftest launch: %s", hipGetErrorString((hipError_t)e));
    YH_WAIT(ctx);
    HIPCHK(ctx, hipMemcpy(out, sums.p, 6 * sizeof(double), hipMemcpyDeviceToHost));
    unsigned int bits;
    HIPCHK(ctx, hipMemcpy(&bits, wbits.p, 4, hipMemcpyDeviceToHost));
    memcpy(dmax, &bits, 4);
    skip_rng(rng, (uint64_t)count * per_iter);
    return YH_OK;
  };
  double s[6];
  float  d;
  if (which == 0 || which == 1) {
    for (float bm = 0.1f; bm < 1.0f; bm += 0.2f)
      for (float bn = 0.1f; bn < 1.0f; bn += 0.2f) {
        const int count = 300000;
        if ((rc = run(bm, bn, count, 3, s, &d))) return rc;
        float avg = which == 0 ? lum(s) / (count * (1 / (4 * pif))) : lum(s) / count;
        float lo = which == 0 ? 0.95f : 0.99f, hi = which == 0 ? 1.05f : 1.01f;
        if (!(avg >= lo && avg <= hi)) ok = false;
        dev = fmax_(dev, std::fabs(avg - 1));
      }
  } else if (which == 2) {
    for (float bm = 0.1f; bm < 1.0f; bm += 0.2f)
      for (float bn = 0.4f; bn < 1.0f; bn += 0.2f) {
        if ((rc = run(bm, bn, 10000, 5, s, &d))) return rc;
        if (!(d <= 0.001f)) ok = false;
        dev = fmax_(dev, d);
      }
  } else {
    for (float bm = 0.2f; bm < 1.0f; bm += 0.2f)
      for (float bn = 0.4f; bn < 1.0f; bn += 0.2f) {
        const int count = 64 * 1024;
        float x = rand1f(rng), y = rand1f(rng);
        sample_sphere(x, y, wo);
        if ((rc = run(bm, bn, count, 3, s, &d))) return rc;
        float fi = lum(s) / count, fu = lum(s + 3) / (count * (1 / (4 * pif)));
        float err = std::fabs(fi - fu) / fu;
        if (err >= 0.05f) ok = false;
        dev = fmax_(dev, err);
      }
  }
  if (worst) *worst = dev;
  if (!ok) return fail(ctx, YH_E_SELFTEST, "TEST FAILED! (self-test %d, worst deviation %g)", which, dev);
  return YH_OK;
}
```

### yocto-hair_amd/host/context_internal.h

```cpp
#ifndef YH_CONTEXT_INTERNAL_H_
#define YH_CONTEXT_INTERNAL_H_
#include <hip/hip_runtime_api.h>
#include <dlfcn.h>
#include <fcntl.h>
#include <sys/stat.h>
#include <unistd.h>
#include <rccl/rccl.h>

#include <algorithm>
#include <chrono>
#include <cmath>
#include <cstdarg>
#include <cstddef>
#include <cstdio>
#include <cstdlib>
#include <cstring>
#include <limits>
#include <map>
#include <mutex>
#include <tuple>
#include <string>
#include <memory>
#include <thread>
#include <vector>

#include "../csrc/yh_device.h"
#include "bvh_build.h"
#include "deadline.h"
#include "yhair.h"

extern "C" {
int yhk_trace(const yhd_scene*, const yhd_state*, int, yhd_counters*, int shape, int grid_blocks, hipStream_t);
int yhk_trace_exact(const yhd_scene*, const yhd_state*, int nsamples, int lds_bytes, int grid_blocks, hipStream_t);
int yhk_trace_exact_occupancy(int lds_bytes, int general);
int yhk_block_threads(int shape);
int yhk_trace_occupancy(int lds_bytes, int general, int shape);
int yhk_trace_sbs(const yhd_scene*, const yhd_state*, int nsamples, int oct_blocks, int quad_items, int oct_entries, int grid_blocks, hipStream_t);
int yhk_trace_sbs_lds_bytes(const yhd_scene* sc);
int yhk_trace_sbs_occupancy(int lds_bytes, int general);
int yhk_trace_lds_bytes(const yhd_scene* sc, int shape);
int yhk_stack_entries(void);
int yhk_stream(const yhd_scene*, const yhd_scene* sc_dev, const yhd_state*, int, const yhd_stream*, int grid_blocks, hipStream_t);
int yhk_lane_tests(const yhd_float4* prims, yhd_float4* blob, int kind, int prim_base, int num_prims, long long test_off, hipStream_t);
int yhk_stream_block_threads(void);
int yhk_stream_lds_bytes(int tables_f4, int slots_per_wave);
int yhk_stream_occupancy(int lds_bytes, int general);
int yhk_intersect_lanes_occupancy(const yhd_scene* sc, int waves);
int yhk_intersect_lanes(const yhd_scene* sc, const yhd_scene* sc_dev, int n, const float* rays, int* cursor, unsigned int* stack_ovf,
    int ovf_entries, int* object, int* element, float* uv, float* dist, int waves, int grid_blocks, hipStream_t stream);
int yhk_resolve(const yhd_state*, int, int, void*, hipStream_t);
int yhk_pack(const yhd_state*, int, int, void*, hipStream_t);
int yhk_unpack(const void*, int, int, int, int, int, int, int, void*, hipStream_t);
int yhk_hair_brdf(int, const void*, const float*, const float*, const float*, float*, hipStream_t);
int yhk_hair_eval(int, const float*, const float*, const float*, float*, hipStream_t);
int yhk_hair_pdf(int, const float*, const float*, const float*, float*, hipStream_t);
int yhk_hair_sample(int, const float*, const float*, const float*, float*, hipStream_t);
int yhk_intersect(const yhd_scene*, int, const float*, int*, int*, float*, float*, hipStream_t);
int yhk_bvh_build_gpu(int n, const float* boxes, float* nodes8, int* primitives, int* num_nodes, int* depth, hipStream_t);
int yhk_prim_boxes(int lines, int n, const float* pos, const float* radius, const int* idx, float* boxes, hipStream_t);
int yhk_bvh_build_resident(int n, const float* d_boxes, float* d_nodes, int* d_pid, int* num_nodes, int* levels, int* level_first, hipStream_t);
int yhk_leaf_records(int lines, int n, const int* pid, const float* pos, const float* nrm, const float* radius, const int* idx, void* prims_out, hipStream_t);
int yhk_wide_index(int num_nodes, const float* d_nodes, int levels, const int* level_first, int L, unsigned int* d_flag, unsigned int* d_widx, int* count, hipStream_t);
int yhk_wide_collapse(int L, int num_nodes, const float* d_nodes, const unsigned int* d_flag, const unsigned int* d_widx, int lines, long long node_off, long long test_off, void* blob, hipStream_t);
int yhk_curves_to_lines(int, const float*, const float*, const float*, int, float*, float*, float*, int*, hipStream_t);
int yhk_surface_lobe(int, int, const float*, const float*, const float*, const float*, const float*, float*, hipStream_t);
int yhk_surface_bsdf(int, const void*, const float*, const float*, const float*, const float*, float*, hipStream_t);
int yhk_selftest(int, float, float, uint64_t, uint64_t, int, const float*, double*, unsigned int*, hipStream_t);
}

struct DevBuf {
  void*  p = nullptr;
  size_t bytes = 0;
  DevBuf() = default;
  DevBuf(const DevBuf&) = delete;
  DevBuf& operator=(const DevBuf&) = delete;
  DevBuf(DevBuf&& o) noexcept : p(o.p), bytes(o.bytes) { o.p = nullptr, o.bytes = 0; }
  ~DevBuf() { reset(); }
  void reset() {
    if (p) (void)hipFree(p);
    p = nullptr, bytes = 0;
  }
};

namespace {



const float pif = (float)3.14159265358979323846;

struct F3 {
  float x, y, z;
};
F3    operator+(F3 a, F3 b) { return {a.x + b.x, a.y + b.y, a.z + b.z}; }
F3    operator-(F3 a, F3 b) { return {a.x - b.x, a.y - b.y, a.z - b.z}; }
F3    operator-(F3 a) { return {-a.x, -a.y, -a.z}; }
F3    operator*(F3 a, float b) { return {a.x * b, a.y * b, a.z * b}; }
float dot(F3 a, F3 b) { return a.x * b.x + a.y * b.y + a.z * b.z; }
F3    cross(F3 a, F3 b) { return {a.y * b.z - a.z * b.y, a.z * b.x - a.x * b.z, a.x * b.y - a.y * b.x}; }
float fmin_(float a, float b) { return (a < b) ? a : b; }
float fmax_(float a, float b) { return (a > b) ? a : b; }
F3    ld3(const float* p) { return {p[0], p[1], p[2]}; }
void  st3(float* p, F3 a) { p[0] = a.x, p[1] = a.y, p[2] = a.z; }

void inverse_frame(const float* f, bool non_rigid, float* out) {
  F3 x = ld3(f), y = ld3(f + 3), z = ld3(f + 6), o = ld3(f + 9);
  F3 rx, ry, rz;
  if (non_rigid) {
    F3    c0 = cross(y, z), c1 = cross(z, x), c2 = cross(x, y);
    float det = dot(x, cross(y, z));
    float s   = 1 / det;
    rx = F3{c0.x, c1.x, c2.x} * s, ry = F3{c0.y, c1.y, c2.y} * s, rz = F3{c0.z, c1.z, c2.z} * s;
  } else {
    rx = {x.x, y.x, z.x}, ry = {x.y, y.y, z.y}, rz = {x.z, y.z, z.z};
  }
  F3 ro = -(rx * o.x + ry * o.y + rz * o.z);
  st3(out, rx), st3(out + 3, ry), st3(out + 6, rz), st3(out + 9, ro);
}
F3 transform_point(const float* f, F3 b) {
  return ld3(f) * b.x + ld3(f + 3) * b.y + ld3(f + 6) * b.z + ld3(f + 9);
}

struct Rng {
  uint64_t state, inc;
};
uint32_t advance_rng(Rng& rng) {
  uint64_t old        = rng.state;
  rng.state           = old * 6364136223846793005ULL + rng.inc;
  uint32_t xorshifted = (uint32_t)(((old >> 18u) ^ old) >> 27u);
  uint32_t rot        = (uint32_t)(old >> 59u);
  return (xorshifted >> rot) | (xorshifted << ((-rot) & 31));
}
Rng make_rng(uint64_t seed, uint64_t seq = 1) {
  Rng rng{0, (seq << 1u) | 1u};
  advance_rng(rng);
  rng.state += seed;
  advance_rng(rng);
  return rng;
}
float rand1f(Rng& rng) {
  uint32_t u = (advance_rng(rng) >> 9) | 0x3f800000u;
  float    f;
  memcpy(&f, &u, 4);
  return f - 1.0f;
}
void skip_rng(Rng& rng, uint64_t delta) {
  uint64_t cur_mult = 6364136223846793005ULL, cur_plus = rng.inc, acc_mult = 1u, acc_plus = 0u;
  while (delta > 0) {
    if (delta & 1) acc_mult *= cur_mult, acc_plus = acc_plus * cur_mult + cur_plus;
    cur_plus = (cur_mult + 1) * cur_plus;
    cur_mult *= cur_mult;
    delta /= 2;
  }
  rng.state = acc_mult * rng.state + acc_plus;
}

float sqr(float v) { return v * v; }
template <int N>
float powt(float v) {
  if constexpr (N == 0) return 1;
  else if constexpr (N == 1) return v;
  else {
    float n2 = powt<N / 2>(v);
    return n2 * n2 * powt<(N & 1)>(v);
  }
}

}

template <typename F>
void parallel_for(int n, F&& fn) {
  int nt = (int)std::min<unsigned>(16u, std::max(1u, std::thread::hardware_concurrency()));
  if (n < 65536 || nt == 1) {
    for (int i = 0; i < n; i++) fn(i);
    return;
  }
  std::vector<std::thread> pool;
  for (int t = 0; t < nt; t++)
    pool.emplace_back([=, &fn] {
      int lo = (int)((int64_t)n * t / nt), hi = (int)((int64_t)n * (t + 1) / nt);
      for (int i = lo; i < hi; i++) fn(i);
    });
  for (auto& th : pool) th.join();
}

struct yh_context {
  int         device = 0;
  hipStream_t stream = nullptr;
  hipEvent_t  ev0 = nullptr, ev1 = nullptr;
  int         hy_quad_items = 0, hy_oct_entries = 0;
  std::vector<int> hy_oct_items;
  int         num_cus = 0;
  std::string device_name;
  std::string error = "no error";
  yhh::BoundedCall sync_call;
  bool        poisoned = false;
  bool      have_scene = false;
  yhd_scene scene{};
  DevBuf    d_prims, d_vpos, d_elems, d_objects, d_materials, d_scene_nodes,
      d_scene_prims, d_light_cdf, d_env_texels, d_light_table, d_env_tab;
  int       stack_need = 0, stack_need8 = 0, stack_need16 = 0;
  struct LaneShape { int kind, num_nodes, prim_base, num_prims; long long node_off, test_off, node_off8, node_off16; };
  std::vector<LaneShape>   lane_shapes;
  long long                lane_units = 0;
  DevBuf                   d_lane_blob;
  bool             have_state = false;
  yhd_state        state{};
  yh_trace_params  params{};
  DevBuf           d_textures, d_tex_texels, d_vtex, d_maps;
  DevBuf           d_rng_state, d_rng_inc, d_accum, d_tiles, d_image, d_counters, d_tile_cursor, d_tile_cost;
  std::vector<int> owned;
  std::vector<unsigned int>  item_cost;
  int              rank = 0, world = 1;
  int              num_tiles_total = 0;
  float            last_ms = 0;
  int              last_launches = 0;
  int              last_nsamples = 0;
  unsigned         launches_of_image = 0;
  int              launch_shape = YH_SHAPE_QUAD;
  int              last_shape = -1;
  bool             async_pending = false;
  bool             last_counted = false;
  DevBuf                  d_gather_send, d_gather_recv;
  std::vector<ncclComm_t> comms;
  std::vector<int>        comm_devices;
  double           shape_ms[YH_SHAPES] = {};
  int              shape_trials[YH_SHAPES] = {};
  uint64_t         scene_key = 0;
  bool             trials_from_disk = false;
  bool             trials_on_disk = false;
  bool             have_costs = false;
  bool             costs_settled = false;
  bool             planned_settled = false;
  int              dense = -1;
  int              chain16 = -1;
  int              chain = -1;
  DevBuf           d_st_slots, d_st_medium, d_st_ovf, d_st_prof, d_st_wave_log, d_st_wave_begin, d_st_wave_fill, d_scene_copy;
  int              st_items = 0;
  size_t           st_share_waves = 0;
  int              st_share_slots = 0;
  std::vector<int>    st_share_begin, st_share_items;
  std::vector<double> st_share_cost;
  std::vector<unsigned long long> st_last_log;
  bool                st_log_fresh = false;
  std::vector<float>  st_wave_speed;
  std::vector<float>  item_scale;
  std::vector<double> stream_speed = {1.10, 1.045, 0.97, 0.885};
  size_t           st_slots = 0, st_medium_slots = 0, st_ovf_words = 0;
  yhd_stream       stream_pool{};
};

#pragma GCC visibility push(hidden)
extern std::string g_create_error;
#define HIPCHK(ctx, call)                                                                               \
  do {                                                                                                  \
    hipError_t e_ = (call);                                                                             \
    if (e_ != hipSuccess) return fail(ctx, YH_E_DEVICE, "%s: %s", #call, hipGetErrorString(e_));       \
  } while (0)

#define YH_WAIT(ctx)                                      \
  do {                                                    \
    if (int wrc_ = wait_for_launch(ctx)) return wrc_;     \
  } while (0)

constexpr int YH_TRIAL_SPP = 32;
constexpr double YH_TRIAL_TIE  = 1.15;
constexpr double YH_FINAL_TIE  = 1.05;
constexpr int    YH_TRIALS_MAX = 2;

int fail(yh_context* ctx, int code, const char* fmt, ...);
int upload(yh_context* ctx, DevBuf& buf, const void* src, size_t bytes);
int upload_keep(yh_context* ctx, DevBuf& buf, const void* src, size_t bytes);
int alloc_zero(yh_context* ctx, DevBuf& buf, size_t bytes);
yhd_float4 node_lo(const yhh::Node& n);
yhd_float4 node_hi(const yhh::Node& n);
int forced_shape();
void trials_load(yh_context* ctx);
bool trials_off();
void record_launch(yh_context* ctx, int nsamples, bool fresh_costs);
bool trial_pending(const yh_context* ctx);
int pick_launch_shape(const yh_context* ctx, int nsamples);
bool settle_launch_shape(yh_context* ctx, bool counted, int nsamples, bool sync);
void build_work_items(const yh_context* ctx, std::vector<int>& items);
void prepare_work_list(yh_context* ctx, std::vector<int>& items, int shape);
int upload_work_items(yh_context* ctx);
int expensive_items(const yh_context* ctx, const std::vector<int>& items);
bool side_by_side_grids(const yh_context* ctx, int* oct_blocks, int* quad_blocks);
void split_items_side_by_side(yh_context* ctx, std::vector<int>& items);
void lay_out_range(const yh_context* ctx, int* items, size_t n, int wpb, int G, int block_offset = 0);
int replan_after_launch(yh_context* ctx, int nsamples);
bool lane_kernels_can_address(const yh_context* ctx);
int stream_geometry(const yh_context* ctx, int num_items, int* slots_per_wave, int* grid_blocks, int* lds_out, bool* single_generation = nullptr);
void note_stream_wave_log(yh_context* ctx, const unsigned long long* log, size_t waves);
void deal_items_for_stream(yh_context* ctx, std::vector<int>& items);
int build_bvh_device(yh_context* ctx, const std::vector<yhh::Box>& boxes, yhh::Tree& tree);
int stream_impl(yh_context* ctx, int nsamples, bool sync);
int trace_impl(yh_context* ctx, int nsamples, bool counted, bool sync);
int wait_for_launch(yh_context* ctx);
int side_by_side_impl(yh_context* ctx, int nsamples, bool sync);
void destroy_communicators(yh_context* ctx);
inline int tiles_of(int n) { return (n + YH_TILE - 1) / YH_TILE; }
void make_material(const yh_material& m, yhd_material& d);
#pragma GCC visibility pop
#endif
```

### yocto-hair_amd/host/scene_upload.cpp

```cpp
#include "context_internal.h"

#include <atomic>

static int dev_alloc(yh_context* ctx, DevBuf& buf, size_t bytes) {
  buf.reset();
  HIPCHK(ctx, hipMalloc(&buf.p, std::max<size_t>(bytes, 16)));
  buf.bytes = std::max<size_t>(bytes, 16);
  return YH_OK;
}

void make_material(const yh_material& m, yhd_material& d) {
  memset(&d, 0, sizeof(d));
  memcpy(d.emission, m.emission, 12);
  memcpy(d.color, m.color, 12);
  float dmax    = fmax_(fmax_(m.color[0], m.color[1]), m.color[2]);
  d.diffuse_pdf = dmax ? dmax / dmax : 0.0f;
  d.thin        = m.thin;
  d.specular = m.specular, d.metallic = m.metallic, d.roughness = m.roughness, d.ior = m.ior;
  d.transmission = m.transmission;
  d.opacity      = m.opacity * ((1.0f + 1.0f + 1.0f) / 3);
  if (d.opacity > 0.999f) d.opacity = 1;
  d.emission_tex = m.emission_tex - 1, d.color_tex = m.color_tex - 1, d.scattering_tex = m.scattering_tex - 1;
  d.trdepth = m.trdepth;
  d.plain = m.specular == 0 && m.metallic == 0 && m.transmission == 0 && d.opacity == 1 && m.emission_tex == 0 &&
            m.color_tex == 0 && m.scattering_tex == 0;
  for (int c = 0; c < 3; c++) {
    float r   = fmin_(fmax_(m.color[c], 0.0f), 0.99f);
    d.meta[c] = (1 + std::sqrt(r)) / (1 - std::sqrt(r));
  }
  d.has_volume = !m.thin && m.transmission != 0;
  for (int c = 0; c < 3; c++) {
    d.vol_density[c] = d.has_volume ? -std::log(fmin_(fmax_(m.color[c], 0.0001f), 1.0f)) / m.trdepth : 0.0f;
    d.vol_scatter[c] = m.scattering[c];
  }
  d.vol_anisotropy = m.scanisotropy;
  F3 sa{0, 0, 0};
  if (m.sigma_a[0] || m.sigma_a[1] || m.sigma_a[2]) {
    sa = ld3(m.sigma_a);
  } else if (m.color[0] || m.color[1] || m.color[2]) {
    float bn  = m.beta_n;
    float den = 5.969f - 0.215f * bn + 2.532f * sqr(bn) - 10.73f * powt<3>(bn) + 5.574f * powt<4>(bn) +
                0.245f * powt<5>(bn);
    F3 q = {std::log(m.color[0]) / den, std::log(m.color[1]) / den, std::log(m.color[2]) / den};
    sa   = {q.x * q.x, q.y * q.y, q.z * q.z};
  } else if (m.eumelanin || m.pheomelanin) {
    F3 e = F3{0.419f, 0.697f, 1.37f}, p = F3{0.187f, 0.4f, 1.05f};
    sa   = F3{m.eumelanin * e.x, m.eumelanin * e.y, m.eumelanin * e.z} +
         F3{m.pheomelanin * p.x, m.pheomelanin * p.y, m.pheomelanin * p.z};
  }
  st3(d.sigma_a, sa);
  d.alpha = m.alpha, d.eta = m.eta;
  float bm = m.beta_m, bn = m.beta_n;
  d.v[0] = sqr(0.726f * bm + 0.812f * sqr(bm) + 3.7f * powt<20>(bm));
  d.v[1] = 0.25f * d.v[0];
  d.v[2] = 4 * d.v[0];
  d.v[3] = d.v[2];
  d.s    = 0.626657069f * (0.265f * bn + 1.194f * sqr(bn) + 5.372f * powt<22>(bn));
  d.sin_2k_alpha[0] = std::sin(pif / 180 * d.alpha);
  d.cos_2k_alpha[0] = std::sqrt(fmax_(0.0f, 1 - sqr(d.sin_2k_alpha[0])));
  for (int i = 1; i < 3; i++) {
    d.sin_2k_alpha[i] = 2 * d.cos_2k_alpha[i - 1] * d.sin_2k_alpha[i - 1];
    d.cos_2k_alpha[i] = sqr(d.cos_2k_alpha[i - 1]) - sqr(d.sin_2k_alpha[i - 1]);
  }
  for (int p = 0; p < 4; p++) {
    d.inv_v[p]        = 1 / d.v[p];
    d.log_inv_2v[p]   = std::log(1 / (2 * d.v[p]));
    d.exp_m2_inv_v[p] = std::exp(-2 / d.v[p]);
    d.mp_den[p]       = ::sinh((double)(1 / d.v[p])) * 2 * d.v[p];
  }
  float cb   = 1 / (1 + std::exp(-pif / d.s));
  float ca   = 1 / (1 + std::exp(-(-pif) / d.s));
  d.tl_cdf_a = ca;
  d.tl_norm  = cb - ca;
}


static bool has_effective_map(const yh_material_maps& m) {
  return m.specular_tex || m.metallic_tex || m.roughness_tex || m.opacity_tex || m.normal_tex;
}

static_assert(sizeof(yhd_maps) == 32, "yhd_maps");

static bool tree_levels(const yhh::Tree& tree, int& levels, int* level_first) {
  std::vector<int> level(tree.nodes.size(), 0);
  for (size_t n = 0; n < tree.nodes.size(); n++)
    if (tree.nodes[n].internal) level[(size_t)tree.nodes[n].start] = level[(size_t)tree.nodes[n].start + 1] = level[n] + 1;
  const int num_nodes = (int)tree.nodes.size();
  levels = level.empty() ? 1 : level.back() + 1;
  if (levels > 128) return false;
  for (int l = 0; l <= levels; l++) level_first[l] = num_nodes;
  for (size_t n = tree.nodes.size(); n-- > 0;) level_first[level[n]] = (int)n;
  return true;
}

int yh_upload_scene(yh_context* ctx, const yh_scene_desc* sd) { return yh_upload_scene_maps(ctx, sd, nullptr); }

int yh_upload_scene_maps(yh_context* ctx, const yh_scene_desc* sd, const yh_material_maps* maps) {
  if (!ctx) return YH_E_INVALID;
  if (!sd) return fail(ctx, YH_E_INVALID, "scene is NULL");
  HIPCHK(ctx, hipSetDevice(ctx->device));
  if (ctx->poisoned) return fail(ctx, YH_E_DEVICE, "a launch of this context exceeded its deadline: the context refuses further work, destroy it");
  YH_WAIT(ctx);
  if (sd->num_objects <= 0) return fail(ctx, YH_E_INVALID, "scene has no objects");
  if (sd->num_environments > YH_MAX_ENVS) return fail(ctx, YH_E_INVALID, "more than %d environments", YH_MAX_ENVS);
  bool any_maps = false;
  if (maps)
    for (int i = 0; i < sd->num_materials; i++) {
      const yh_material_maps& m = maps[i];
      for (int id : {m.specular_tex, m.metallic_tex, m.roughness_tex, m.transmission_tex, m.opacity_tex, m.normal_tex})
        if (id < 0 || id > sd->num_textures) return fail(ctx, YH_E_INVALID, "material %d: a map references a missing texture (%d of %d)", i, id, sd->num_textures);
      any_maps = any_maps || has_effective_map(m);
    }
  const bool timing = getenv("YHAIR_TIMING") && atoi(getenv("YHAIR_TIMING")) != 0;
  auto       t_last = std::chrono::steady_clock::now();
  auto       lap    = [&](const char* what) {
    if (!timing) return;
    auto now = std::chrono::steady_clock::now();
    fprintf(stderr, "[yhair] upload: %-28s %8.1f ms\n", what, std::chrono::duration<double, std::milli>(now - t_last).count());
    t_last = now;
  };
  struct ShapeInfo {
    int kind, prim_base, vert_base, elem_base, has_normals, depth;
    int depth8, depth16;
    yhh::Box root;
    int num_prims;
    int num_nodes = 0, levels = 1;
    int level_first[130] = {0};
    int wide_count[3] = {0, 0, 0};
    std::vector<yhd_float4> host_prims;
  };
  std::vector<ShapeInfo>  info(sd->num_shapes);
  std::vector<DevBuf>     d_tree(sd->num_shapes);
  std::vector<yhd_float4> vpos;
  std::vector<float>      vtex;
  std::vector<yhd_int4>   elems;
  size_t total_prim_f4 = 0;
  for (int si = 0; si < sd->num_shapes; si++) {
    auto& s = sd->shapes[si];
    if (s.num_vertices <= 0 || !s.positions) return fail(ctx, YH_E_INVALID, "shape %d has no vertices", si);
    const bool lines = s.num_lines > 0;
    if (!lines && s.num_triangles <= 0) return fail(ctx, YH_E_INVALID, "shape %d has no lines or triangles", si);
    const int nel = lines ? s.num_lines : s.num_triangles;
    if (nel >= (1 << 27)) return fail(ctx, YH_E_INVALID, "shape %d has %d elements (limit %d)", si, nel, (1 << 27) - 1);
    info[si].kind = lines ? YH_KIND_LINES : YH_KIND_TRIANGLES, info[si].num_prims = nel, info[si].has_normals = s.normals != nullptr;
    info[si].prim_base = (int)total_prim_f4;
    total_prim_f4 += (size_t)nel * (lines ? 4 : 6);
  }
  if (total_prim_f4 > (size_t)std::numeric_limits<int>::max()) return fail(ctx, YH_E_INVALID, "scene too large for 32-bit record offsets (%zu primitive float4)", total_prim_f4);
  int rc;
  ctx->have_scene = false, ctx->have_state = false;
  ctx->scene.lane_blob = nullptr, ctx->scene.prims = nullptr;
  ctx->d_prims.reset(), ctx->d_lane_blob.reset();
  if ((rc = dev_alloc(ctx, ctx->d_prims, total_prim_f4 * 16))) return rc;
  lap("validation, record array");
  const char* bvh_env   = getenv("YHAIR_BVH");
  const bool  host_only = bvh_env && !strcmp(bvh_env, "host"), device_all = bvh_env && !strcmp(bvh_env, "device");
  for (int si = 0; si < sd->num_shapes; si++) {
    auto&      s     = sd->shapes[si];
    auto&      I     = info[si];
    const bool lines = I.kind == YH_KIND_LINES;
    const int  nel   = I.num_prims;
    const int* idx   = lines ? s.lines : s.triangles;
    {
      std::atomic<bool> bad{false};
      parallel_for(nel * (lines ? 2 : 3), [&](int k) {
        if (idx[k] < 0 || idx[k] >= s.num_vertices) bad = true;
      });
      if (bad) return fail(ctx, YH_E_INVALID, "shape %d: vertex index out of range", si);
    }
    I.vert_base = (int)vpos.size(), I.elem_base = (int)elems.size();
    yhd_float4* d_recs = (yhd_float4*)ctx->d_prims.p + I.prim_base;
    if ((nel >= 32768 || device_all) && !host_only) {
      const size_t nv = (size_t)s.num_vertices;
      DevBuf d_pos, d_nrm, d_rad, d_idx, d_boxes, d_pid;
      auto h2d = [&](DevBuf& buf, const void* src, size_t bytes) -> int {
        if (int arc = dev_alloc(ctx, buf, bytes)) return arc;
        HIPCHK(ctx, hipMemcpyAsync(buf.p, src, bytes, hipMemcpyHostToDevice, ctx->stream));
        return YH_OK;
      };
      if ((rc = h2d(d_pos, s.positions, nv * 12))) return rc;
      if (s.radius && (rc = h2d(d_rad, s.radius, nv * 4))) return rc;
      if ((rc = h2d(d_idx, idx, (size_t)nel * (lines ? 8 : 12)))) return rc;
      if ((rc = dev_alloc(ctx, d_boxes, (size_t)nel * 24))) return rc;
      if ((rc = dev_alloc(ctx, d_pid, (size_t)nel * 4))) return rc;
      if ((rc = dev_alloc(ctx, d_tree[si], ((size_t)2 * nel + 1) * 32))) return rc;
      int e = yhk_prim_boxes(lines ? 1 : 0, nel, (const float*)d_pos.p, (const float*)d_rad.p, (const int*)d_idx.p, (float*)d_boxes.p, ctx->stream);
      if (e) return fail(ctx, YH_E_DEVICE, "primitive bounds: %s", hipGetErrorString((hipError_t)e));
      if (s.normals && (rc = h2d(d_nrm, s.normals, nv * 12))) return rc;
      e = yhk_bvh_build_resident(nel, (const float*)d_boxes.p, (float*)d_tree[si].p, (int*)d_pid.p, &I.num_nodes, &I.levels, I.level_first, ctx->stream);
      if (e) return fail(ctx, YH_E_DEVICE, "device BVH build: %s", hipGetErrorString((hipError_t)e));
      lap("device: bounds + reference tree");
      e = yhk_leaf_records(lines ? 1 : 0, nel, (const int*)d_pid.p, (const float*)d_pos.p, (const float*)d_nrm.p, (const float*)d_rad.p, (const int*)d_idx.p, d_recs, ctx->stream);
      if (e) return fail(ctx, YH_E_DEVICE, "leaf records: %s", hipGetErrorString((hipError_t)e));
      float root8[8];
      HIPCHK(ctx, hipMemcpyAsync(root8, d_tree[si].p, 32, hipMemcpyDeviceToHost, ctx->stream));
      YH_WAIT(ctx);
      memcpy(I.root.min, root8, 12), memcpy(I.root.max, root8 + 3, 12);
      lap("device: leaf records");
    } else {
      auto pos = [&](int v) { return ld3(s.positions + 3 * (size_t)v); };
      auto rad = [&](int v) { return s.radius ? s.radius[v] : 0.001f; };
      std::vector<yhh::Box> boxes(nel);
      parallel_for(nel, [&](int e) {
        if (lines) {
          int a = idx[2 * e], b = idx[2 * e + 1];
          F3  p0 = pos(a), p1 = pos(b);
          float r0 = rad(a), r1 = rad(b);
          float lo0[3] = {p0.x - r0, p0.y - r0, p0.z - r0}, lo1[3] = {p1.x - r1, p1.y - r1, p1.z - r1};
          float hi0[3] = {p0.x + r0, p0.y + r0, p0.z + r0}, hi1[3] = {p1.x + r1, p1.y + r1, p1.z + r1};
          for (int k = 0; k < 3; k++) boxes[e].min[k] = fmin_(lo0[k], lo1[k]), boxes[e].max[k] = fmax_(hi0[k], hi1[k]);
        } else {
          const float* p0 = s.positions + 3 * (size_t)idx[3 * e];
          const float* p1 = s.positions + 3 * (size_t)idx[3 * e + 1];
          const float* p2 = s.positions + 3 * (size_t)idx[3 * e + 2];
          for (int k = 0; k < 3; k++) {
            boxes[e].min[k] = fmin_(p0[k], fmin_(p1[k], p2[k]));
            boxes[e].max[k] = fmax_(p0[k], fmax_(p1[k], p2[k]));
          }
        }
      });
      yhh::Tree tree;
      yhh::build_bvh(tree, boxes);
      static_assert(sizeof(yhh::Node) == 32 && offsetof(yhh::Node, start) == 24 && offsetof(yhh::Node, num) == 28 && offsetof(yhh::Node, internal) == 30 && offsetof(yhh::Node, axis) == 31,
          "yhh::Node is the device's node record");
      I.num_nodes = (int)tree.nodes.size();
      if (!tree_levels(tree, I.levels, I.level_first)) return fail(ctx, YH_E_INVALID, "shape %d: tree of %d levels", si, I.levels);
      if ((rc = upload(ctx, d_tree[si], tree.nodes.data(), tree.nodes.size() * 32))) return rc;
      I.root = tree.nodes[0].bbox;
// ... 85 lines not shown
  }
  std::vector<DevBuf> d_wflag((size_t)sd->num_shapes * 3), d_widx((size_t)sd->num_shapes * 3);
  for (int si = 0; si < sd->num_shapes; si++)
    for (int w = 0; w < 3; w++) {
      auto&  I = info[si];
      DevBuf &f = d_wflag[(size_t)si * 3 + w], &x = d_widx[(size_t)si * 3 + w];
      if ((rc = dev_alloc(ctx, f, ((size_t)I.num_nodes + 1) * 4))) return rc;
      if ((rc = dev_alloc(ctx, x, ((size_t)I.num_nodes + 1) * 4))) return rc;
      int e = yhk_wide_index(I.num_nodes, (const float*)d_tree[si].p, I.levels, I.level_first, 2 + w, (unsigned int*)f.p, (unsigned int*)x.p, &I.wide_count[w], ctx->stream);
      if (e) return fail(ctx, YH_E_DEVICE, "wide-node index: %s", hipGetErrorString((hipError_t)e));
    }
  ctx->lane_shapes.assign((size_t)sd->num_shapes, yh_context::LaneShape{});
  long long U8 = 0, U16 = 0, blob_units = 0;
  {
    long long at = 4ll * scene_wide_count;
    for (int si = 0; si < sd->num_shapes; si++) {
      auto& L = ctx->lane_shapes[(size_t)si];
      L.kind = info[si].kind, L.num_nodes = info[si].wide_count[0], L.prim_base = info[si].prim_base, L.num_prims = info[si].num_prims;
      L.test_off = at, at += (long long)L.num_prims * (L.kind == YH_KIND_LINES ? 1 : 2);
    }
    at = (at + 3) / 4 * 4 + 4;
    if (at >= (1ll << 27)) return fail(ctx, YH_E_INVALID, "scene too large for 27-bit leaf offsets (%lld test-record units)", at);
    for (int si = 0; si < sd->num_shapes; si++) ctx->lane_shapes[(size_t)si].node_off = at, at += 4ll * info[si].wide_count[0];
    ctx->lane_units = at + 4;
    U8 = (ctx->lane_units + 3) / 4 * 4, at = U8;
    for (int si = 0; si < sd->num_shapes; si++) ctx->lane_shapes[(size_t)si].node_off8 = at, at += 8ll * info[si].wide_count[1];
    U16 = at;
    for (int si = 0; si < sd->num_shapes; si++) ctx->lane_shapes[(size_t)si].node_off16 = at, at += 16ll * info[si].wide_count[2];
    blob_units = at + 4;
    if (blob_units >= (1ll << 30)) return fail(ctx, YH_E_INVALID, "scene too large for 30-bit node offsets (%lld units)", blob_units);
    (void)U16;
  }
  if ((rc = alloc_zero(ctx, ctx->d_lane_blob, (size_t)blob_units * 32))) return rc;
  for (int si = 0; si < sd->num_shapes; si++) {
    auto& L = ctx->lane_shapes[(size_t)si];
    auto& I = info[si];
    int e = yhk_lane_tests((const yhd_float4*)ctx->d_prims.p, (yhd_float4*)ctx->d_lane_blob.p, L.kind, L.prim_base, L.num_prims, L.test_off, ctx->stream);
    const long long offs[3] = {L.node_off, L.node_off8, L.node_off16};
    for (int w = 0; w < 3 && !e; w++)
      e = yhk_wide_collapse(2 + w, I.num_nodes, (const float*)d_tree[si].p, (const unsigned int*)d_wflag[(size_t)si * 3 + w].p, (const unsigned int*)d_widx[(size_t)si * 3 + w].p,
          L.kind == YH_KIND_LINES ? 1 : 0, offs[w], L.test_off, ctx->d_lane_blob.p, ctx->stream);
    if (e) return fail(ctx, YH_E_DEVICE, "wide collapse: %s", hipGetErrorString((hipError_t)e));
  }
  if (scene_wide) {
    int e = yhk_wide_collapse(2, (int)scene_tree.nodes.size(), (const float*)d_stree.p, (const unsigned int*)d_sflag.p, (const unsigned int*)d_sidx.p, 1, 0, 0, ctx->d_lane_blob.p, ctx->stream);
    if (e) return fail(ctx, YH_E_DEVICE, "wide collapse of the scene tree: %s", hipGetErrorString((hipError_t)e));
  }
  YH_WAIT(ctx);
  d_tree.clear(), d_wflag.clear(), d_widx.clear(), d_stree.reset(), d_sflag.reset(), d_sidx.reset();
  lap("device: wide collapses, blob");
  std::vector<yhd_object> objects(sd->num_objects);
  for (int oi = 0; oi < sd->num_objects; oi++) {
    auto& o = sd->objects[oi];
    auto& I = info[o.shape];
    auto& d = objects[oi];
    memcpy(d.frame, o.frame, 48);
    inverse_frame(o.frame, true, d.inv_frame);
    d.kind = I.kind, d.node_base = 0, d.prim_base = I.prim_base, d.vert_base = I.vert_base;
    d.elem_base = I.elem_base, d.has_normals = I.has_normals, d.material = o.material, d.has_texcoords = sd->shapes[o.shape].texcoords != nullptr;
    const auto& LS = ctx->lane_shapes[(size_t)o.shape];
    d.lane_root = (int)LS.node_off, d.lane_test = (int)LS.test_off, d.lane_root8 = (int)LS.node_off8, d.lane_root16 = (int)LS.node_off16;
    {
      const float *lo = obj_boxes[oi].min, *hi = obj_boxes[oi].max;
      float ext = fmax_(fmax_(hi[0] - lo[0], hi[1] - lo[1]), hi[2] - lo[2]);
      float eps = 1e-3f * ext + 1e-5f;
      for (int k = 0; k < 3; k++) d.wbox_min[k] = lo[k] - eps, d.wbox_max[k] = hi[k] + eps;
      d.wbox_min[3] = d.wbox_max[3] = 0;
    }
  }
  if (vpos.size() > (size_t)std::numeric_limits<int>::max()) return fail(ctx, YH_E_INVALID, "scene too large for 32-bit vertex offsets (%zu)", vpos.size());
  std::vector<yhd_float4> scene_nodes;
  for (auto& n : scene_tree.nodes) scene_nodes.push_back(node_lo(n)), scene_nodes.push_back(node_hi(n));
  int max_shape_depth = 0;
  for (auto& I : info) max_shape_depth = std::max(max_shape_depth, I.depth);
  const int scene_need = scene_wide ? 3 * scene_wide_depth + 4 : scene_tree.max_depth + 4;
  ctx->stack_need = scene_need + 3 * max_shape_depth + 2;
  int max_shape_depth8 = 0;
  for (auto& I : info) max_shape_depth8 = std::max(max_shape_depth8, I.depth8);
  ctx->stack_need8 = scene_need + 7 * max_shape_depth8 + 2;
  int max_shape_depth16 = 0;
  for (auto& I : info) max_shape_depth16 = std::max(max_shape_depth16, I.depth16);
  ctx->stack_need16 = scene_need + 15 * max_shape_depth16 + 2;
  if (ctx->stack_need > yhk_stack_entries())
    return fail(ctx, YH_E_INVALID, "BVH too deep for the traversal stack (%d > %d)", ctx->stack_need, yhk_stack_entries());
  std::vector<yhd_material> materials(sd->num_materials);
  int general_materials = 0;
  std::vector<yhd_maps> mat_maps(any_maps ? (size_t)sd->num_materials : 0);
  for (int i = 0; i < sd->num_materials; i++) {
    make_material(sd->materials[i], materials[i]);
    if (any_maps) {
      const yh_material_maps& m = maps[i];
      yhd_maps&               d = mat_maps[(size_t)i];
      d.specular_tex = m.specular_tex - 1, d.metallic_tex = m.metallic_tex - 1, d.roughness_tex = m.roughness_tex - 1;
      d.opacity_tex = m.opacity_tex - 1, d.normal_tex = m.normal_tex - 1;
      d.any = has_effective_map(m) ? 1 : 0, d.opacity = sd->materials[i].opacity, d.pad = 0;
      if (d.any) materials[i].plain = 0;
    }
    if (!materials[i].plain) general_materials = 1;
  }
  yhd_scene sc{};
  std::vector<float>      light_cdf;
  std::vector<yhd_float4> env_texels;
  std::vector<int>        small_lights;
  for (int oi = 0; oi < sd->num_objects; oi++) {
    auto& o = sd->objects[oi];
    auto& m = sd->materials[o.material];
    if (m.emission[0] == 0 && m.emission[1] == 0 && m.emission[2] == 0) continue;
    auto& s = sd->shapes[o.shape];
    if (s.num_lines > 0 || s.num_triangles <= 0) continue;
    if (sc.num_lights >= YH_MAX_LIGHTS) return fail(ctx, YH_E_INVALID, "more than %d lights: object %d of %d is emissive too (each instance of an emitter counts)", YH_MAX_LIGHTS, oi, sd->num_objects);
    auto& L = sc.lights[sc.num_lights++];
    L.object = oi, L.environment = -1, L.cdf_base = (int)light_cdf.size(), L.cdf_count = s.num_triangles, L.small_base = -1;
    if (s.num_triangles <= YH_SMALL_LIGHT_TRIS) small_lights.push_back(sc.num_lights - 1);
    else general_materials = 1;
    for (int t = 0; t < s.num_triangles; t++) {
      F3 p0 = ld3(s.positions + 3 * (size_t)s.triangles[3 * t]), p1 = ld3(s.positions + 3 * (size_t)s.triangles[3 * t + 1]),
         p2 = ld3(s.positions + 3 * (size_t)s.triangles[3 * t + 2]);
      F3    c    = cross(p1 - p0, p2 - p0);
      float area = std::sqrt(dot(c, c)) / 2;
      if (t) area += light_cdf.back();
      light_cdf.push_back(area);
    }
  }
  sc.num_environments = sd->num_environments;
  for (int ei = 0; ei < sd->num_environments; ei++) {
    auto& e = sd->environments[ei];
    auto& d = sc.environments[ei];
    memcpy(d.frame, e.frame, 48);
    inverse_frame(e.frame, false, d.inv_frame);
    memcpy(d.emission, e.emission, 12);
    d.tex_w = e.texels ? e.tex_width : 0, d.tex_h = e.texels ? e.tex_height : 0;
    d.texel_base = (int)env_texels.size();
    if (e.texels)
      for (size_t t = 0; t < (size_t)e.tex_width * e.tex_height; t++)
        env_texels.push_back({e.texels[3 * t], e.texels[3 * t + 1], e.texels[3 * t + 2], 0});
    if (e.emission[0] == 0 && e.emission[1] == 0 && e.emission[2] == 0) continue;
    if (sc.num_lights >= YH_MAX_LIGHTS) return fail(ctx, YH_E_INVALID, "more than %d lights", YH_MAX_LIGHTS);
    auto& L = sc.lights[sc.num_lights++];
    L.object = -1, L.environment = ei, L.cdf_base = (int)light_cdf.size(), L.cdf_count = 0, L.small_base = -1;
    if (e.texels) {
      size_t n    = (size_t)e.tex_width * e.tex_height;
      L.cdf_count = (int)n;
      for (size_t i = 0; i < n; i++) {
        int   iy    = (int)(i / e.tex_width);
        float th    = (iy + 0.5f) * pif / e.tex_height;
        float mx    = fmax_(fmax_(e.texels[3 * i], e.texels[3 * i + 1]), e.texels[3 * i + 2]);
        float value = mx * std::sin(th);
        if (i) value += light_cdf.back();
        light_cdf.push_back(value);
      }
    }
  }
  if (sc.num_lights == 0) return fail(ctx, YH_E_INVALID, "scene has no lights (the path sampler needs at least one)");
  std::vector<yhd_float4> light_table;
  for (int li : small_lights) {
    auto& L  = sc.lights[li];
    auto& I  = info[sd->objects[L.object].shape];
    if (I.host_prims.empty()) {
      I.host_prims.resize((size_t)6 * L.cdf_count);
      HIPCHK(ctx, hipMemcpy(I.host_prims.data(), (const yhd_float4*)ctx->d_prims.p + I.prim_base, I.host_prims.size() * 16, hipMemcpyDeviceToHost));
    }
    const yhd_float4* rec = I.host_prims.data();
    L.small_base = (int)light_table.size();
    yhd_float4 b0{I.root.min[0], I.root.min[1], I.root.min[2], 0}, b1{I.root.max[0], I.root.max[1], I.root.max[2], light_cdf[(size_t)L.cdf_base + L.cdf_count - 1]};
    memcpy(&b0.w, &L.cdf_count, 4);
    light_table.push_back(b0), light_table.push_back(b1);
    for (int t = 0; t < YH_SMALL_LIGHT_TRIS; t++)
      for (int k = 0; k < 3; k++) light_table.push_back(t < L.cdf_count ? rec[6 * t + k] : yhd_float4{0, 0, 0, 0});
    yhd_float4 cdf{0, 0, 0, 0};
    for (int t = 0; t < L.cdf_count; t++) (&cdf.x)[t] = light_cdf[(size_t)L.cdf_base + t];
    light_table.push_back(cdf);
  }
  std::vector<float> env_tab;
  sc.env_tab_light = -1, sc.env_tab_k = 0, sc.env_tab_stride = 0;
  for (int li = 0; li < sc.num_lights && sc.env_tab_light < 0; li++) {
    auto& L = sc.lights[li];
    if (L.environment < 0 || L.cdf_count < 4096) continue;
    const int n = L.cdf_count, S = (n + 2047) / 2048, K = (n + S - 1) / S;
    env_tab.resize((size_t)K);
    for (int k = 0; k < K; k++) env_tab[(size_t)k] = light_cdf[(size_t)L.cdf_base + (size_t)std::min<int64_t>(n, (int64_t)(k + 1) * S) - 1];
    sc.env_tab_light = li, sc.env_tab_k = K, sc.env_tab_stride = S;
  }
  std::vector<yhd_texture> textures((size_t)std::max(0, sd->num_textures));
  std::vector<yhd_float4>  tex_texels;
  {
    std::vector<char> need_linear(textures.size(), 0);
    for (int i = 0; i < sd->num_materials; i++) {
      auto& m = sd->materials[i];
      for (int id : {m.emission_tex, m.color_tex, m.scattering_tex})
        if (id < 0 || id > sd->num_textures) return fail(ctx, YH_E_INVALID, "material %d references a missing texture", i);
      if (m.emission_tex > 0) need_linear[(size_t)m.emission_tex - 1] = 1;
      if (any_maps)
        for (int id : {maps[i].specular_tex, maps[i].metallic_tex, maps[i].roughness_tex, maps[i].opacity_tex, maps[i].normal_tex})
          if (id > 0) need_linear[(size_t)id - 1] = 1;
    }
    auto srgb_to_rgb = [](float srgb) {
      return (srgb <= 0.04045) ? srgb / 12.92f : std::pow((srgb + 0.055f) / (1.0f + 0.055f), 2.4f);
    };
    std::vector<char> used(textures.size(), !any_maps);
    if (any_maps)
      for (int i = 0; i < sd->num_materials; i++) {
        auto& m = sd->materials[i];
        for (int id : {m.emission_tex, m.color_tex, m.scattering_tex})
          if (id > 0) used[(size_t)id - 1] = 1;
      }
    for (size_t t = 0; t < textures.size(); t++) used[t] = used[t] || need_linear[t];
    for (size_t t = 0; t < textures.size(); t++) {
      auto& src = sd->textures[t];
      if (src.width <= 0 || src.height <= 0 || !src.pixels) return fail(ctx, YH_E_INVALID, "texture %d is empty", (int)t);
      size_t n = (size_t)src.width * src.height;
      auto&  d = textures[t];
      d.width = src.width, d.height = src.height, d.srgb_base = (int)tex_texels.size(), d.linear_base = -1;
      if (!used[t]) {
        d.srgb_base = -1;
        continue;
      }
      tex_texels.resize(tex_texels.size() + n);
      yhd_float4* out = tex_texels.data() + d.srgb_base;
      if (src.is_byte) {
        auto b = (const unsigned char*)src.pixels;
        parallel_for((int)n, [&](int i) {
          out[i] = {srgb_to_rgb(b[3 * (size_t)i] / 255.0f), srgb_to_rgb(b[3 * (size_t)i + 1] / 255.0f),
              srgb_to_rgb(b[3 * (size_t)i + 2] / 255.0f), 0};
        });
        if (need_linear[t]) {
          d.linear_base = (int)tex_texels.size();
          tex_texels.resize(tex_texels.size() + n);
          yhd_float4* lin = tex_texels.data() + d.linear_base;
          parallel_for((int)n, [&](int i) { lin[i] = {b[3 * (size_t)i] / 255.0f, b[3 * (size_t)i + 1] / 255.0f, b[3 * (size_t)i + 2] / 255.0f, 0}; });
        }
      } else {
        auto f = (const float*)src.pixels;
        parallel_for((int)n, [&](int i) { out[i] = {f[3 * (size_t)i], f[3 * (size_t)i + 1], f[3 * (size_t)i + 2], 0}; });
        d.linear_base = d.srgb_base;
      }
    }
  }
  lap("objects, materials, lights");
  if ((rc = upload(ctx, ctx->d_vpos, vpos.data(), vpos.size() * 16))) return rc;
  if ((rc = upload(ctx, ctx->d_elems, elems.data(), elems.size() * 16))) return rc;
  if ((rc = upload(ctx, ctx->d_objects, objects.data(), objects.size() * sizeof(yhd_object)))) return rc;
  if ((rc = upload(ctx, ctx->d_materials, materials.data(), materials.size() * sizeof(yhd_material)))) return rc;
  if ((rc = upload(ctx, ctx->d_scene_nodes, scene_nodes.data(), scene_nodes.size() * 16))) return rc;
  std::vector<int> scene_prims_padded = scene_tree.primitives;
  scene_prims_padded.resize((scene_prims_padded.size() + 3) / 4 * 4, 0);
  if ((rc = upload(ctx, ctx->d_scene_prims, scene_prims_padded.data(), scene_prims_padded.size() * 4))) return rc;
  if ((rc = upload(ctx, ctx->d_light_cdf, light_cdf.data(), light_cdf.size() * 4))) return rc;
  if ((rc = upload(ctx, ctx->d_light_table, light_table.data(), light_table.size() * 16))) return rc;
  if ((rc = upload(ctx, ctx->d_env_tab, env_tab.data(), env_tab.size() * 4))) return rc;
  if ((rc = upload(ctx, ctx->d_env_texels, env_texels.data(), env_texels.size() * 16))) return rc;
  if ((rc = upload(ctx, ctx->d_textures, textures.data(), textures.size() * sizeof(yhd_texture)))) return rc;
  if ((rc = upload(ctx, ctx->d_tex_texels, tex_texels.data(), tex_texels.size() * 16))) return rc;
  if ((rc = upload(ctx, ctx->d_vtex, vtex.data(), vtex.size() * 4))) return rc;
  if (any_maps) {
    if ((rc = upload(ctx, ctx->d_maps, mat_maps.data(), mat_maps.size() * sizeof(yhd_maps)))) return rc;
  } else {
    ctx->d_maps.reset();
  }
  lap("hipMalloc + H2D copies");
  sc.prims = (const yhd_float4*)ctx->d_prims.p;
  sc.vpos = (const yhd_float4*)ctx->d_vpos.p;
  sc.elems = (const yhd_int4*)ctx->d_elems.p;
  sc.objects = (const yhd_object*)ctx->d_objects.p, sc.materials = (const yhd_material*)ctx->d_materials.p;
  sc.scene_nodes = (const yhd_float4*)ctx->d_scene_nodes.p, sc.scene_prims = (const int*)ctx->d_scene_prims.p;
  sc.num_scene_nodes = (int)scene_tree.nodes.size(), sc.num_objects = sd->num_objects;
  sc.light_cdf = (const float*)ctx->d_light_cdf.p, sc.env_texels = (const yhd_float4*)ctx->d_env_texels.p;
  sc.light_table = (const yhd_float4*)ctx->d_light_table.p, sc.light_table_f4 = (int)light_table.size();
  sc.env_tab = (const float*)ctx->d_env_tab.p;
  sc.stack_entries = std::max(8, (ctx->stack_need + 7) / 8 * 8);
  sc.stack_entries8 = std::max(8, (ctx->stack_need8 + 7) / 8 * 8);
  sc.stack_entries16 = std::max(8, (ctx->stack_need16 + 7) / 8 * 8);
  sc.lane_blob = (const yhd_float4*)ctx->d_lane_blob.p, sc.lane_blob_units = blob_units;
  sc.textures = (const yhd_texture*)ctx->d_textures.p, sc.tex_texels = (const yhd_float4*)ctx->d_tex_texels.p;
  sc.vtex = (const float*)ctx->d_vtex.p;
  sc.maps = any_maps ? (const yhd_maps*)ctx->d_maps.p : nullptr;
  memcpy(sc.camera.frame, sd->camera.frame, 48);
  sc.camera.lens = sd->camera.lens, sc.camera.film_x = sd->camera.film[0], sc.camera.film_y = sd->camera.film[1];
  sc.camera.focus = sd->camera.focus, sc.camera.aperture = sd->camera.aperture;
  sc.num_nodes_total = 0, sc.num_prim_f4 = (int)total_prim_f4;
  for (auto& I : info) sc.num_nodes_total += I.wide_count[0];
  sc.general_materials = general_materials;
  sc.lds_scene_f4    = scene_wide ? 0 : lds_scene_f4;
  sc.scene_wide_root = scene_wide ? 0 : -1;
  {
    static_assert(sizeof(yhd_material) == 16 * YH_MATERIAL_F4, "yhd_material is staged to LDS as float4");
    sc.lds_materials = sd->num_materials <= 24 ? sd->num_materials : 0;
    if (sc.lds_materials == 0 || sc.lds_scene_f4 == 0) sc.general_materials = 1;
  }
  ctx->scene      = sc;
  {
    uint64_t h = 1469598103934665603ULL;
    auto mix = [&](const void* p, size_t n) {
      const unsigned char* b = (const unsigned char*)p;
      for (size_t i = 0; i < n; i++) h = (h ^ b[i]) * 1099511628211ULL;
    };
    mix(&sd->camera, sizeof(sd->camera));
    mix(sd->materials, sizeof(yh_material) * (size_t)sd->num_materials);
    mix(sd->objects, sizeof(yh_object) * (size_t)sd->num_objects);
    for (int i = 0; i < sd->num_shapes; i++) {
      const yh_shape& sh = sd->shapes[i];
      int counts[3] = {sh.num_vertices, sh.num_lines, sh.num_triangles};
      mix(counts, sizeof(counts));
      if (sh.positions && sh.num_vertices > 0) {
        const size_t n = (size_t)sh.num_vertices, take = std::min<size_t>(n, 256);
        mix(sh.positions, take * 12), mix(sh.positions + 3 * (n - take), take * 12);
      }
    }
    for (int i = 0; i < sd->num_environments; i++) mix(&sd->environments[i], offsetof(yh_environment, texels));
    if (any_maps) mix(maps, sizeof(yh_material_maps) * (size_t)sd->num_materials);
    ctx->scene_key = h;
  }
  ctx->d_scene_copy.reset();
  ctx->have_scene = true;
  ctx->have_state = false;
  ctx->launch_shape = YH_SHAPE_QUAD;
  ctx->item_cost.clear();
  ctx->have_costs = false, ctx->costs_settled = false, ctx->dense = -1, ctx->chain = -1, ctx->chain16 = -1;
  for (double& t : ctx->shape_ms) t = 0;
  for (int& t : ctx->shape_trials) t = 0;
  ctx->trials_from_disk = false;
  lap("scene table, fingerprint");
  return YH_OK;
}

int build_bvh_device(yh_context* ctx, const std::vector<yhh::Box>& boxes, yhh::Tree& tree) {
// ... 19 lines not shown
```

### yocto-hair_amd/python/yhair_capi.py

```python
import ctypes as C
import os

import numpy as np

ROOT = os.path.dirname(os.path.dirname(os.path.dirname(os.path.abspath(__file__))))
LIB_PATH = os.environ.get("YHAIR_LIB", os.path.join(ROOT, "yocto-hair_amd", "libyhair.so"))

YH_OK, YH_E_INVALID, YH_E_DEVICE, YH_E_STATE, YH_E_IO, YH_E_SELFTEST = 0, -1, -2, -3, -4, -5
YH_HAIR_BRDF_FLOATS = 30
SURFACE_BSDF_FLOATS = 29
(LOBE_DIFFUSE, LOBE_SPECULAR, LOBE_METAL, LOBE_TRANSMISSION, LOBE_REFRACTION, LOBE_DELTA_SPECULAR,
 LOBE_DELTA_METAL, LOBE_DELTA_TRANSMISSION, LOBE_DELTA_REFRACTION) = range(9)
LOBE_COUNT = 9

c_float_p = C.POINTER(C.c_float)
c_int_p = C.POINTER(C.c_int)


class Shape(C.Structure):
    _fields_ = [("num_vertices", C.c_int), ("positions", c_float_p), ("normals", c_float_p),
                ("radius", c_float_p), ("num_lines", C.c_int), ("lines", c_int_p),
                ("num_triangles", C.c_int), ("triangles", c_int_p), ("texcoords", c_float_p)]


class Texture(C.Structure):
    _fields_ = [("width", C.c_int), ("height", C.c_int), ("is_byte", C.c_int), ("pixels", C.c_void_p)]


class Material(C.Structure):
    _fields_ = [("emission", C.c_float * 3), ("color", C.c_float * 3), ("specular", C.c_float),
                ("metallic", C.c_float), ("roughness", C.c_float), ("transmission", C.c_float),
                ("opacity", C.c_float), ("ior", C.c_float), ("thin", C.c_int),
                ("sigma_a", C.c_float * 3), ("beta_m", C.c_float), ("beta_n", C.c_float),
                ("alpha", C.c_float), ("eta", C.c_float), ("eumelanin", C.c_float),
                ("pheomelanin", C.c_float), ("scattering", C.c_float * 3), ("scanisotropy", C.c_float),
                ("trdepth", C.c_float), ("emission_tex", C.c_int), ("color_tex", C.c_int),
                ("scattering_tex", C.c_int)]


class MaterialMaps(C.Structure):
    _fields_ = [("specular_tex", C.c_int), ("metallic_tex", C.c_int), ("roughness_tex", C.c_int),
                ("transmission_tex", C.c_int), ("opacity_tex", C.c_int), ("normal_tex", C.c_int)]


class Object(C.Structure):
    _fields_ = [("frame", C.c_float * 12), ("shape", C.c_int), ("material", C.c_int)]


class Environment(C.Structure):
    _fields_ = [("frame", C.c_float * 12), ("emission", C.c_float * 3), ("tex_width", C.c_int),
                ("tex_height", C.c_int), ("texels", c_float_p)]


class Camera(C.Structure):
    _fields_ = [("frame", C.c_float * 12), ("lens", C.c_float), ("film", C.c_float * 2),
                ("focus", C.c_float), ("aperture", C.c_float)]


class SceneDesc(C.Structure):
    _fields_ = [("num_shapes", C.c_int), ("shapes", C.POINTER(Shape)),
                ("num_materials", C.c_int), ("materials", C.POINTER(Material)),
                ("num_objects", C.c_int), ("objects", C.POINTER(Object)),
                ("num_environments", C.c_int), ("environments", C.POINTER(Environment)),
                ("camera", Camera), ("num_textures", C.c_int), ("textures", C.POINTER(Texture))]


SHADER_NAMES = ["naive", "path", "eyelight", "normal"]


class TraceParams(C.Structure):
    _fields_ = [("resolution", C.c_int), ("bounces", C.c_int), ("clamp", C.c_float),
                ("seed", C.c_uint64), ("shader", C.c_int), ("hair_exact", C.c_int)]

    @staticmethod
    def default(resolution=720, bounces=8, clamp=100.0, seed=961748941, shader="path", hair_exact=False):
        return TraceParams(resolution, bounces, clamp, seed, SHADER_NAMES.index(shader) if isinstance(shader, str) else shader,
                           1 if hair_exact else 0)


class WorkCounts(C.Structure):
    _fields_ = [(n, C.c_uint64) for n in ("samples", "rays", "nodes", "seg_tests", "tri_tests",
                                          "hair_shades", "surf_shades", "env_lookups",
                                          "env_samples", "cyc_trace", "cyc_shade", "ticks_tile",
                                          "wave_iters", "wave_steps", "lane_steps", "lane_iters", "cyc_geom", "cyc_sample",
                                          "cyc_eval", "cyc_rest")] + [("branch", C.c_uint64 * 10)]

    def as_dict(self):
        d = {n: int(getattr(self, n)) for n, _ in self._fields_ if n != "branch"}
        names = ("node", "line", "tri", "enter", "scene")
        for k, nm in enumerate(names):
            d["trips_" + nm], d["lanes_" + nm] = int(self.branch[2 * k]), int(self.branch[2 * k + 1])
        return d

    def bytes_per_sample(self, spp_per_launch, env_textured=True):
        s = max(1, self.samples)
        return (32 * self.nodes + 44 * self.seg_tests + 52 * self.tri_tests +
                104 * self.hair_shades + (48 * self.env_lookups if env_textured else 0) + 88 * self.env_samples) / s \
            + 32.0 / spp_per_launch


def fptr(a):
    return a.ctypes.data_as(c_float_p)


def iptr(a):
    return a.ctypes.data_as(c_int_p)


def hair_material_rows(mats12):
    mats12 = np.ascontiguousarray(mats12, dtype=np.float32).reshape(-1, 12)
    arr = (Material * len(mats12))()
    for i, r in enumerate(mats12):
        m = arr[i]
        m.sigma_a[:] = r[0:3].tolist()
        m.beta_m, m.beta_n, m.alpha, m.eta = map(float, r[3:7])
        m.color[:] = r[7:10].tolist()
        m.eumelanin, m.pheomelanin = float(r[10]), float(r[11])
        m.opacity, m.ior, m.thin, m.trdepth = 1.0, 1.5, 1, 0.01
    return arr


_SIGS = {
    "yh_create": (C.c_void_p, [C.c_int]),
    "yh_destroy": (None, [C.c_void_p]),
    "yh_last_error": (C.c_char_p, [C.c_void_p]),
    "yh_version": (C.c_char_p, []),
    "yh_upload_scene": (C.c_int, [C.c_void_p, C.POINTER(SceneDesc)]),
    "yh_upload_scene_maps": (C.c_int, [C.c_void_p, C.POINTER(SceneDesc), C.POINTER(MaterialMaps)]),
    "yh_init_state": (C.c_int, [C.c_void_p, C.POINTER(TraceParams)]),
    "yh_image_size": (C.c_int, [C.c_void_p, c_int_p, c_int_p]),
    "yh_set_shard": (C.c_int, [C.c_void_p, C.c_int, C.c_int]),
    "yh_trace_samples": (C.c_int, [C.c_void_p, C.c_int]),
    "yh_trace_samples_async": (C.c_int, [C.c_void_p, C.c_int]),
    "yh_synchronize": (C.c_int, [C.c_void_p]),
    "yh_download": (C.c_int, [C.c_void_p, c_float_p]),
    "yh_pack_tiles_device": (C.c_int, [C.c_void_p, C.c_void_p, C.c_int64, C.POINTER(C.c_int64)]),
    "yh_unpack_tiles_device": (C.c_int, [C.c_void_p, C.c_void_p, C.c_int, C.c_int, C.c_void_p]),
    "yh_gather_framebuffer": (C.c_int, [C.POINTER(C.c_void_p), C.c_int, c_float_p]),
    "yh_shard_pixels": (C.c_int64, [C.c_void_p, C.c_int, C.c_int]),
    "yh_download_rng": (C.c_int, [C.c_void_p, C.POINTER(C.c_uint64)]),
    "yh_trace_samples_counted": (C.c_int, [C.c_void_p, C.c_int, C.POINTER(WorkCounts)]),
    "yh_last_trace_ms": (C.c_int, [C.c_void_p, c_float_p, c_int_p]),
    "yh_launch_shape": (C.c_int, [C.c_void_p]),
    "yh_tile_costs": (C.c_int, [C.c_void_p, C.POINTER(C.c_uint32), C.c_int]),
    "yh_item_costs": (C.c_int, [C.c_void_p, C.POINTER(C.c_uint32), C.c_int]),
    "yh_kernel_trials": (C.c_int, [C.c_void_p, C.POINTER(C.c_double), C.POINTER(C.c_int), C.c_int]),
    "yh_trials_pending": (C.c_int, [C.c_void_p]),
    "yh_set_trial_cache_dir": (C.c_int, [C.c_char_p]),
    "yh_default_trial_cache_dir": (C.c_char_p, []),
    "yh_hair_brdf_batch": (C.c_int, [C.c_void_p, C.c_int, C.POINTER(Material), c_float_p,
                                     c_float_p, c_float_p, c_float_p]),
    "yh_curves_to_lines": (C.c_int, [C.c_void_p, C.c_int, c_float_p, c_float_p, c_float_p, C.c_int, c_float_p,
                                     c_float_p, c_float_p, c_int_p]),
    "yh_bvh_build_gpu": (C.c_int, [C.c_void_p, C.c_int, c_float_p, c_float_p, c_int_p]),
    "yh_bvh_build": (C.c_int, [C.c_int, c_float_p, c_float_p, c_int_p]),
    "yh_bvh_build_wide": (C.c_int, [C.c_int, c_float_p, C.c_int, c_float_p]),
    "yh_bvh_build_wide_gpu": (C.c_int, [C.c_void_p, C.c_int, c_float_p, C.c_int, c_float_p]),
    "yh_surface_lobe_batch": (C.c_int, [C.c_void_p, C.c_int, C.c_int, c_float_p, c_float_p, c_float_p, c_float_p,
                                        c_float_p, c_float_p]),
    "yh_surface_bsdf_batch": (C.c_int, [C.c_void_p, C.c_int, C.POINTER(Material), c_float_p, c_float_p, c_float_p,
                                        c_float_p, c_float_p]),
    "yh_hair_eval_batch": (C.c_int, [C.c_void_p, C.c_int, c_float_p, c_float_p, c_float_p, c_float_p]),
    "yh_hair_sample_batch": (C.c_int, [C.c_void_p, C.c_int, c_float_p, c_float_p, c_float_p, c_float_p]),
    "yh_hair_pdf_batch": (C.c_int, [C.c_void_p, C.c_int, c_float_p, c_float_p, c_float_p, c_float_p]),
    "yh_hair_eval_pdf_batch": (C.c_int, [C.c_void_p, C.c_int, c_float_p, c_float_p, c_float_p, c_float_p]),
    "yh_intersect_batch": (C.c_int, [C.c_void_p, C.c_int, c_float_p, c_int_p, c_int_p, c_float_p, c_float_p]),
    "yh_selftest": (C.c_int, [C.c_void_p, C.c_int, c_float_p]),
    "yh_scene_load": (C.c_void_p, [C.c_char_p, C.c_char_p, C.c_char_p, C.c_int]),
    "yh_scene_get": (C.POINTER(SceneDesc), [C.c_void_p]),
    "yh_scene_get_maps": (C.POINTER(MaterialMaps), [C.c_void_p]),
    "yh_scene_free": (None, [C.c_void_p]),
    "yh_save_image": (C.c_int, [C.c_char_p, C.c_int, C.c_int, c_float_p, C.c_char_p, C.c_int]),
}
EXPORTS = tuple(_SIGS)

_lib = None


def load(path=None):
    global _lib
    if _lib is None or path:
        p = path or LIB_PATH
        if not os.path.exists(p):
            raise RuntimeError(f"{p} is missing: run `python -c 'import __graft_entry__ as g; g.build()'` "
                               "(there is no CPU fallback for the product path)")
        lib = C.CDLL(p)
        for name, (res, args) in _SIGS.items():
            try:
                fn = getattr(lib, name)
            except AttributeError:
                if "YHAIR_LIB" in os.environ:
                    continue
                raise
            fn.restype, fn.argtypes = res, args
        if path:
            return lib
        _lib = lib
    return _lib


class YhError(RuntimeError):
    pass


def set_trial_cache_dir(path=None, default=False):
    lib = load()
    if not hasattr(lib, "yh_set_trial_cache_dir"):
        return None
    d = lib.yh_default_trial_cache_dir() if default else (path.encode() if path else None)
    lib.yh_set_trial_cache_dir(d)
    return d.decode() if d else None


class SceneFile:

    def __init__(self, json_path, camera=""):
        lib = load()
        err = C.create_string_buffer(512)
        self.handle = lib.yh_scene_load(str(json_path).encode(), camera.encode(), err, 512)
        if not self.handle:
            raise YhError(err.value.decode())
        self.desc = lib.yh_scene_get(self.handle)
        self.maps = lib.yh_scene_get_maps(self.handle)

    def close(self):
        if self.handle and load is not None:
            load().yh_scene_free(self.handle)
            self.handle = None

    def __del__(self):
        try:
            self.close()
        except Exception:
            pass


def gather_framebuffer(contexts):
    lib = load()
    w, h = C.c_int(), C.c_int()
    contexts[0]._chk(lib.yh_image_size(contexts[0].h, C.byref(w), C.byref(h)))
    img = np.zeros((h.value, w.value, 4), np.float32)
    arr = (C.c_void_p * len(contexts))(*[c.h for c in contexts])
    contexts[0]._chk(lib.yh_gather_framebuffer(arr, len(contexts), fptr(img)))
    return img


class Context:

    def __init__(self, device=0):
        self.lib = load()
        self.h = self.lib.yh_create(device)
        if not self.h:
            raise YhError("yh_create failed: " + self.lib.yh_last_error(None).decode())

    def _chk(self, rc):
        if rc != YH_OK:
            raise YhError(f"yhair error {rc}: " + self.lib.yh_last_error(self.h).decode())

    def close(self):
        if self.h:
            self.lib.yh_destroy(self.h)
            self.h = None

    def __del__(self):
        try:
            self.close()
        except Exception:
            pass

    def upload_scene(self, desc, maps=None):
        if maps is None:
            self._chk(self.lib.yh_upload_scene(self.h, desc))
        else:
            self._chk(self.lib.yh_upload_scene_maps(self.h, desc, C.cast(maps, C.POINTER(MaterialMaps))))

    def set_shard(self, rank, world):
        self._chk(self.lib.yh_set_shard(self.h, rank, world))

    def init_state(self, params):
        self._chk(self.lib.yh_init_state(self.h, C.byref(params)))
        w, h = C.c_int(), C.c_int()
        self._chk(self.lib.yh_image_size(self.h, C.byref(w), C.byref(h)))
        self.width, self.height = w.value, h.value
        return self.width, self.height

    def trace_samples(self, n):
        self._chk(self.lib.yh_trace_samples(self.h, n))

    def trace_samples_async(self, n):
        self._chk(self.lib.yh_trace_samples_async(self.h, n))

    def synchronize(self):
        self._chk(self.lib.yh_synchronize(self.h))

    def trace_samples_counted(self, n):
        wc = WorkCounts()
        self._chk(self.lib.yh_trace_samples_counted(self.h, n, C.byref(wc)))
        return wc

    def launch_shape(self):
        return int(self.lib.yh_launch_shape(self.h))

    def last_trace_ms(self):
        ms, n = C.c_float(), C.c_int()
        self._chk(self.lib.yh_last_trace_ms(self.h, C.byref(ms), C.byref(n)))
        return ms.value, n.value

    def tile_costs(self):
        tx, ty = (self.width + 7) // 8, (self.height + 7) // 8
        out = np.zeros(tx * ty, np.uint32)
        self._chk(self.lib.yh_tile_costs(self.h, out.ctypes.data_as(C.POINTER(C.c_uint32)), len(out)))
        return out.reshape(ty, tx)

    def kernel_trials(self):
        ms, tr = (C.c_double * 16)(), (C.c_int * 16)()
        n = self.lib.yh_kernel_trials(self.h, ms, tr, 16)
        self._chk(min(n, 0))
        return {k: (round(ms[k], 5), tr[k]) for k in range(min(n, 16)) if tr[k] or ms[k]}

    def trials_pending(self):
        n = self.lib.yh_trials_pending(self.h)
        self._chk(min(n, 0))
        return n > 0

    def item_costs(self):
        w, h = C.c_int(), C.c_int()
        self._chk(self.lib.yh_image_size(self.h, C.byref(w), C.byref(h)))
        n = ((w.value + 7) // 8) * ((h.value + 7) // 8) * 4
        out = np.zeros(n, np.uint32)
        self._chk(self.lib.yh_item_costs(self.h, out.ctypes.data_as(C.POINTER(C.c_uint32)), n))
        return out

    def download(self):
        img = np.zeros((self.height, self.width, 4), np.float32)
        self._chk(self.lib.yh_download(self.h, fptr(img)))
        return img

    def download_rng(self):
        rng = np.zeros((self.height * self.width, 2), np.uint64)
        self._chk(self.lib.yh_download_rng(self.h, rng.ctypes.data_as(C.POINTER(C.c_uint64))))
        return rng

    def shard_pixels(self, rank, world):
        return int(self.lib.yh_shard_pixels(self.h, rank, world))

    def pack_tiles_device(self, dev_ptr, capacity):
        n = C.c_int64()
        self._chk(self.lib.yh_pack_tiles_device(self.h, C.c_void_p(dev_ptr), capacity, C.byref(n)))
        return n.value

    def unpack_tiles_device(self, packed_ptr, src_rank, world, image_ptr):
        self._chk(self.lib.yh_unpack_tiles_device(self.h, C.c_void_p(packed_ptr), src_rank, world,
                                                  C.c_void_p(image_ptr)))

    def hair_brdf(self, mats12, v, normal, tangent):
        mats = hair_material_rows(mats12)
        n = len(mats)
        v = np.ascontiguousarray(v, np.float32)
        normal = np.ascontiguousarray(normal, np.float32)
        tangent = np.ascontiguousarray(tangent, np.float32)
        out = np.zeros((n, 30), np.float32)
        self._chk(self.lib.yh_hair_brdf_batch(self.h, n, mats, fptr(v), fptr(normal), fptr(tangent), fptr(out)))
        return out

    def _wowi(self, fn, brdf, a, b, width):
        brdf = np.ascontiguousarray(brdf, np.float32)
        a = np.ascontiguousarray(a, np.float32)
        b = np.ascontiguousarray(b, np.float32)
        n = len(brdf)
        out = np.zeros((n, width) if width > 1 else (n,), np.float32)
        self._chk(fn(self.h, n, fptr(brdf), fptr(a), fptr(b), fptr(out)))
        return out

    def hair_eval(self, brdf, wo, wi):
        return self._wowi(self.lib.yh_hair_eval_batch, brdf, wo, wi, 3)

    def hair_sample(self, brdf, wo, rn):
        return self._wowi(self.lib.yh_hair_sample_batch, brdf, wo, rn, 3)

    def hair_pdf(self, brdf, wo, wi):
        return self._wowi(self.lib.yh_hair_pdf_batch, brdf, wo, wi, 1)

    def curves_to_lines(self, P, width0, width1, base_vertex=0):
        P = np.ascontiguousarray(P, np.float32).reshape(-1, 12)
        w0, w1 = np.ascontiguousarray(width0, np.float32), np.ascontiguousarray(width1, np.float32)
        n = len(P)
        pos, nrm = np.zeros((5 * n, 3), np.float32), np.zeros((5 * n, 3), np.float32)
        rad, lines = np.zeros(5 * n, np.float32), np.zeros((4 * n, 2), np.int32)
        self._chk(self.lib.yh_curves_to_lines(self.h, n, fptr(P), fptr(w0), fptr(w1), base_vertex, fptr(pos), fptr(nrm),
                                              fptr(rad), iptr(lines)))
        return pos, nrm, rad, lines

    def surface_lobe(self, kind, params8, normal, wo, wi, rn3):
        a = [np.ascontiguousarray(x, np.float32) for x in (params8, normal, wo, wi, rn3)]
        out = np.zeros((len(a[0]), 7), np.float32)
        self._chk(self.lib.yh_surface_lobe_batch(self.h, kind, len(a[0]), *(fptr(x) for x in a), fptr(out)))
        return out

    def surface_bsdf(self, materials, normal, wo, wi, rn3):
        a = [np.ascontiguousarray(x, np.float32) for x in (normal, wo, wi, rn3)]
        out = np.zeros((len(a[0]), SURFACE_BSDF_FLOATS), np.float32)
        self._chk(self.lib.yh_surface_bsdf_batch(self.h, len(a[0]), materials, *(fptr(x) for x in a), fptr(out)))
        return out

    def intersect(self, rays):
        rays = np.ascontiguousarray(rays, np.float32).reshape(-1, 8)
        n = len(rays)
        obj, elem = np.zeros(n, np.int32), np.zeros(n, np.int32)
        uv, dist = np.zeros((n, 2), np.float32), np.zeros(n, np.float32)
        self._chk(self.lib.yh_intersect_batch(self.h, n, fptr(rays), iptr(obj), iptr(elem), fptr(uv), fptr(dist)))
        return obj, elem, uv, dist

    def selftest(self, which):
        worst = C.c_float()
        rc = self.lib.yh_selftest(self.h, which, C.byref(worst))
        if rc not in (YH_OK, YH_E_SELFTEST):
            self._chk(rc)
        return rc == YH_OK, worst.value
```

Before: 2585.

## Fold constant environment lights, stage light tables in LDS, prefetch hit records and randoms

When every light is an untextured environment, the host precomputes a constant light pdf and environment emission. The trace kernel then returns these from LDS and samples a uniform sphere directly instead of walking the light and environment lists. Light and environment records are copied into the LDS light table, and on the non-general path the hit record and the per-bounce random numbers are loaded or drawn before shading so their latency can overlap. It adds a device/host consistency-check entry point and a second copy of the RNG consumption order that must stay equivalent to the original.

```diff
diff --git a/include/yhair.h b/include/yhair.h
--- a/include/yhair.h
+++ b/include/yhair.h
@@ -216,6 +216,8 @@
 
 int yh_selftest(yh_context* ctx, int which, float* worst);
 
+int yh_light_constants(yh_context* ctx, int* folded, float* host4, float* device4);
+
 typedef struct yh_scene_file yh_scene_file;
 yh_scene_file*       yh_scene_load(const char* json_path, const char* camera,
           char* error, int error_len);
diff --git a/yocto-hair_amd/csrc/dev_hair.h b/yocto-hair_amd/csrc/dev_hair.h
--- a/yocto-hair_amd/csrc/dev_hair.h
+++ b/yocto-hair_amd/csrc/dev_hair.h
@@ -57,15 +57,22 @@
 YH_DEV float safe_sqrt(float x) { return h_sqrt(fmax_(0.0f, x)); }
 YH_DEV float exact_safe_sqrt(float x) { return sqrtf(fmax_(0.0f, x)); }
 
-template <bool QUAD = false>
-YH_DEV hair_hit hair_setup(float v, f3 normal, f3 tangent) {
-  hair_hit hh;
+YH_DEV void hair_setup_offset(hair_hit& hh, float v) {
   hh.h       = -1 + 2 * v;
   hh.gamma_o = safe_asin(hh.h);
+}
+template <bool QUAD = false>
+YH_DEV void hair_setup_frame(hair_hit& hh, f3 normal, f3 tangent) {
   f3 z       = QUAD ? quad_normalize(normal) : normalize(normal);
   f3 x       = QUAD ? quad_orthonormalize(tangent, z) : orthonormalize(tangent, z);
   f3 y       = QUAD ? quad_normalize(cross(z, x)) : normalize(cross(z, x));
   hh.w2b     = transpose_rot(frame{x, y, z, mk3(0.0f)});
+}
+template <bool QUAD = false>
+YH_DEV hair_hit hair_setup(float v, f3 normal, f3 tangent) {
+  hair_hit hh;
+  hair_setup_offset(hh, v);
+  hair_setup_frame<QUAD>(hh, normal, tangent);
   return hh;
 }
 
@@ -342,11 +349,8 @@
   b          = (float)compact1by1((uint32_t)(v >> 1)) / 65536.0f;
 }
 
-YH_DEV f3 hair_sample(const yhd_material& m, const hair_hit& hh, const hair_out& ho, float rnx, float rny) {
+YH_DEV f3 hair_sample_demuxed(const yhd_material& m, const hair_hit& hh, const hair_out& ho, float u00, float u01, float u10, float u11) {
   float sin_theta_o = ho.sin_theta_o, cos_theta_o = ho.cos_theta_o, phi_o = ho.phi_o;
-  float u00, u01, u10, u11;
-  demux_float(rnx, u00, u01);
-  demux_float(rny, u10, u11);
   int   p  = 0;
   float u1 = u00 - ho.pdf0, u2 = u1 - ho.pdf1;
   if (!(u00 < ho.pdf0)) p = !(u1 < ho.pdf1) ? (!(u2 < ho.pdf2) ? 3 : 2) : 1;
@@ -372,6 +376,12 @@
   f3    incoming = f3{sin_theta_i, cos_theta_i * d_cos(phi_i), cos_theta_i * d_sin(phi_i)};
   return d_transform_direction(transpose_rot(hh.w2b), incoming);
 }
+YH_DEV f3 hair_sample(const yhd_material& m, const hair_hit& hh, const hair_out& ho, float rnx, float rny) {
+  float u00, u01, u10, u11;
+  demux_float(rnx, u00, u01);
+  demux_float(rny, u10, u11);
+  return hair_sample_demuxed(m, hh, ho, u00, u01, u10, u11);
+}
 YH_DEV f3 hair_sample(const yhd_material& m, const hair_hit& hh, f3 outgoing_, float rnx, float rny) {
   hair_out ho = hair_prepare(m, hh, outgoing_);
   return hair_sample(m, hh, ho, rnx, rny);
diff --git a/yocto-hair_amd/csrc/dev_path.h b/yocto-hair_amd/csrc/dev_path.h
--- a/yocto-hair_amd/csrc/dev_path.h
+++ b/yocto-hair_amd/csrc/dev_path.h
@@ -65,6 +65,43 @@
 struct hit_geom {
   f3 position, normal, element_normal;
 };
+struct hit_record {
+  v4f r[6];
+};
+YH_DEV hit_record load_hit_record(const yhd_scene& sc, const yhd_object& o, int slot) {
+  const bool        tri = o.kind == YH_KIND_TRIANGLES;
+  const yhd_float4* rec = sc.prims + (size_t)o.prim_base + (size_t)slot * (tri ? 6 : 4);
+  hit_record h;
+  h.r[0] = ldg4(rec), h.r[1] = ldg4(rec + 1), h.r[2] = ldg4(rec + 2), h.r[3] = ldg4(rec + 3);
+  h.r[4] = ldg4(rec + (tri ? 4 : 0)), h.r[5] = ldg4(rec + (tri ? 5 : 1));
+  return h;
+}
+YH_DEV hit_geom eval_hit(const yhd_object& o, const hit_record& h, float u, float v) {
+  frame    fr = ldframe(o.frame);
+  hit_geom g;
+  if (o.kind == YH_KIND_TRIANGLES) {
+    f3 p0 = xyz(h.r[0]), p1 = xyz(h.r[1]), p2 = xyz(h.r[2]);
+    g.position       = transform_point(fr, p0 * (1 - u - v) + p1 * u + p2 * v);
+    g.element_normal = quad_transform_normal(fr, quad_normalize(cross(p1 - p0, p2 - p0)));
+    if (o.has_normals) {
+      f3 n0 = xyz(h.r[3]), n1 = xyz(h.r[4]), n2 = xyz(h.r[5]);
+      g.normal = quad_transform_normal(fr, quad_normalize(n0 * (1 - u - v) + n1 * u + n2 * v));
+    } else {
+      g.normal = g.element_normal;
+    }
+  } else {
+    f3 p0 = xyz(h.r[0]), p1 = xyz(h.r[1]);
+    g.position       = transform_point(fr, p0 * (1 - u) + p1 * u);
+    g.element_normal = quad_transform_normal(fr, quad_normalize(p1 - p0));
+    if (o.has_normals) {
+      f3 n0 = xyz(h.r[2]), n1 = xyz(h.r[3]);
+      g.normal = quad_transform_normal(fr, quad_normalize(n0 * (1 - u) + n1 * u));
+    } else {
+      g.normal = g.element_normal;
+    }
+  }
+  return g;
+}
 YH_DEV hit_geom eval_hit(const yhd_scene& sc, const yhd_object& o, int slot, float u, float v) {
   frame    fr = ldframe(o.frame);
   hit_geom g;
@@ -109,12 +146,29 @@
   f3 c = xyz(tx[(size_t)j * sx + ii]), d = xyz(tx[(size_t)jj * sx + ii]);
   return a * (1 - u) * (1 - v) + b * (1 - u) * v + c * u * (1 - v) + d * u * v;
 }
-template <bool COUNT>
+template <bool FROM_LDS>
+YH_DEV const yhd_light& light_record(const trace_ctx& tc, int k) {
+  if constexpr (FROM_LDS) return *(const yhd_light*)(const YH_LDS yhd_light*)((const YH_LDS int*)(tc.lds_lights + 1) + YH_LIGHT_DW * k);
+  else return tc.sc->lights[k];
+}
+template <bool FROM_LDS>
+YH_DEV const yhd_environment& environment_record(const trace_ctx& tc, int k) {
+  if constexpr (FROM_LDS) return *(const yhd_environment*)(const YH_LDS yhd_environment*)(tc.lds_lights + YHD_LIGHT_HEAD_F4(tc.sc) + YH_ENVIRONMENT_F4 * k);
+  else return tc.sc->environments[k];
+}
+template <bool COUNT, bool PLAIN = false>
 YH_DEV f3 eval_environment(const trace_ctx& tc, f3 dir) {
   const yhd_scene& sc = *tc.sc;
+  if constexpr (PLAIN) {
+    if (sc.light_fold & YH_FOLD_ENVS) {
+      if (COUNT && (__lane_id() & 3u) == 0) tc.stats->envl += (unsigned int)sc.num_environments;
+      const v4f c = tc.lds_lights[0];
+      return f3{c.y, c.z, c.w};
+    }
+  }
   f3 emission = mk3(0.0f);
   for (int k = 0; k < sc.num_environments; k++) {
-    const yhd_environment& env = sc.environments[k];
+    const yhd_environment& env = environment_record<PLAIN>(tc, k);
     if (COUNT) count_quad<COUNT>(tc.stats->envl);
     if (env.tex_w == 0) {
       emission = emission + ld3(env.emission) * mk3(1.0f);
@@ -187,9 +241,17 @@
 YH_DEV f3 sample_lights(const trace_ctx& tc, f3 position, float rl, float rel, float ruvx,
     float ruvy) {
   const yhd_scene& sc = *tc.sc;
+  if constexpr (!BIG_LIGHTS && !YH_LANE) {
+    if (sc.light_fold & YH_FOLD_LIGHTS) {
+      float z   = 2 * ruvy - 1;
+      float r   = sqrtf(fclamp(1 - z * z, 0.0f, 1.0f));
+      float phi = 2 * pif * ruvx;
+      return f3{r * cosf(phi), r * sinf(phi), z};
+    }
+  }
   int n        = sc.num_lights;
   int light_id = iclamp((int)(rl * n), 0, n - 1);
-  const yhd_light& light = sc.lights[light_id];
+  const yhd_light& light = light_record<!BIG_LIGHTS && !YH_LANE>(tc, light_id);
   if (light.object >= 0 && (!BIG_LIGHTS || (light.small_base >= 0 && tc.lds_lights))) {
     const YH_LDS v4f* L = tc.lds_lights + light.small_base;
     int   element = sample_discrete_cdf((const YH_LDS float*)(L + 14), light.cdf_count, rel);
@@ -210,7 +272,7 @@
     f3 lposition = eval_position(sc, sc.objects[light.object], element, u, v);
     return normalize(lposition - position);
   } else if (light.environment >= 0) {
-    const yhd_environment& env = sc.environments[light.environment];
+    const yhd_environment& env = environment_record<!BIG_LIGHTS && !YH_LANE>(tc, light.environment);
     if (env.tex_w) {
       if (COUNT) count_quad<COUNT>(tc.stats->envs);
       int   idx = (tc.lds_envtab && light_id == sc.env_tab_light)
@@ -233,9 +295,12 @@
 template <bool COUNT, int STRIDE, bool BIG_LIGHTS>
 YH_DEV float sample_lights_pdf(const trace_ctx& tc, f3 position, f3 direction) {
   const yhd_scene& sc = *tc.sc;
+  if constexpr (!BIG_LIGHTS && !YH_LANE) {
+    if (sc.light_fold & YH_FOLD_LIGHTS) return tc.lds_lights[0].x;
+  }
   float pdf = 0.0f;
   for (int k = 0; k < sc.num_lights; k++) {
-    const yhd_light& light = sc.lights[k];
+    const yhd_light& light = light_record<!BIG_LIGHTS && !YH_LANE>(tc, k);
     if (light.object >= 0 && (!BIG_LIGHTS || (light.small_base >= 0 && tc.lds_lights))) {
       const YH_LDS v4f* L = tc.lds_lights + light.small_base;
       frame fr, inv;
@@ -277,7 +342,7 @@
       }
       pdf += lpdf;
     } else if (light.environment >= 0) {
-      const yhd_environment& env = sc.environments[light.environment];
+      const yhd_environment& env = environment_record<!BIG_LIGHTS && !YH_LANE>(tc, light.environment);
       if (env.tex_w) {
         f3    wl = transform_direction(ldframe(env.inv_frame), direction);
         float tx = atan2f(wl.z, wl.x) / (2 * pif);
@@ -465,7 +530,7 @@
   if (isec.object < 0) return false;
 #else
   if (isec.object < 0) {
-    ps.radiance = ps.radiance + ps.weight * eval_environment<COUNT>(tc, ps.ray.d);
+    ps.radiance = ps.radiance + ps.weight * eval_environment<COUNT, !GENERAL>(tc, ps.ray.d);
     if (COUNT) tc.stats->c_rest += clock64() - k0;
     return false;
   }
@@ -513,7 +578,24 @@
   constexpr bool from_lds = !GENERAL && (YH_LANE || STRIDE != 64);
   const yhd_object&   o   = !from_lds ? sc.objects[isec.object] : *(const yhd_object*)(const YH_LDS yhd_object*)(tc.lds_scene + YH_OBJECT_F4 * isec.object);
   const yhd_material& mat = !from_lds ? sc.materials[o.material] : *(const yhd_material*)(const YH_LDS yhd_material*)(tc.lds_mats + YH_MATERIAL_F4 * o.material);
-  hit_geom hg = eval_hit(sc, o, isec.slot, isec.u, isec.v);
+  constexpr bool ahead = !GENERAL && !YH_LANE;
+  hit_record hr;
+  float      r_pick = 0, r_a = 0, r_b = 0, r_c = 0, r_d = 0, u00 = 0, u01 = 0, u10 = 0, u11 = 0;
+  hair_hit   hh;
+  if constexpr (ahead) {
+    hr     = load_hit_record(sc, o, isec.slot);
+    r_pick = rand1f(rng);
+    r_a = rand1f(rng), r_b = rand1f(rng), r_c = rand1f(rng);
+    const uint64_t after3 = rng.state;
+    r_d = rand1f(rng);
+    if (r_pick < 0.5f) rng.state = after3;
+    demux_float(r_a, u00, u01);
+    demux_float(r_b, u10, u11);
+    hair_setup_offset(hh, isec.v);
+  }
+  hit_geom hg;
+  if constexpr (ahead) hg = eval_hit(o, hr, isec.u, isec.v);
+  else hg = eval_hit(sc, o, isec.slot, isec.u, isec.v);
   f3 position = hg.position;
   f3 nrm      = hg.normal;
   hit_maps hm;
@@ -563,20 +645,24 @@
     if (COUNT) tc.stats->c_rest += clock64() - k0;
     return path_continue(ps, rng, bounces);
   }
-  hair_hit hh;
   hair_out ho;
   if (is_hair) {
-    hh = hair_setup<!YH_LANE>(isec.v, normal, nrm);
+    if constexpr (ahead) hair_setup_frame<!YH_LANE>(hh, normal, nrm);
+    else hh = hair_setup<!YH_LANE>(isec.v, normal, nrm);
     ho = hair_prepare<!YH_LANE>(mat, hh, outgoing);
   }
 
   if (COUNT) k1 = clock64(), tc.stats->c_geom += k1 - k0;
   f3 incoming;
-  if (rand1f(rng) < 0.5f) {
-    float rnx = rand1f(rng), rny = rand1f(rng);
-    float rnl = rand1f(rng);
+  if (ahead ? r_pick < 0.5f : rand1f(rng) < 0.5f) {
+    float rnx = r_a, rny = r_b, rnl = r_c;
+    if constexpr (!ahead) {
+      rnx = rand1f(rng), rny = rand1f(rng);
+      rnl = rand1f(rng);
+    }
     if (is_hair) {
-      incoming = hair_sample(mat, hh, ho, rnx, rny);
+      if constexpr (ahead) incoming = hair_sample_demuxed(mat, hh, ho, u00, u01, u10, u11);
+      else incoming = hair_sample(mat, hh, ho, rnx, rny);
     } else if (general) {
       incoming = surface_sample(sb, normal, outgoing, rnl, rnx, rny);
     } else {
@@ -586,9 +672,12 @@
       }
     }
   } else {
-    float ruvx = rand1f(rng), ruvy = rand1f(rng);
-    float rel = rand1f(rng);
-    float rl  = rand1f(rng);
+    float ruvx = r_a, ruvy = r_b, rel = r_c, rl = r_d;
+    if constexpr (!ahead) {
+      ruvx = rand1f(rng), ruvy = rand1f(rng);
+      rel = rand1f(rng);
+      rl  = rand1f(rng);
+    }
     incoming  = sample_lights<COUNT, GENERAL>(tc, position, rl, rel, ruvx, ruvy);
   }
   if (COUNT) k2 = clock64(), tc.stats->c_sample += k2 - k1;
diff --git a/yocto-hair_amd/csrc/kernels.hip b/yocto-hair_amd/csrc/kernels.hip
--- a/yocto-hair_amd/csrc/kernels.hip
+++ b/yocto-hair_amd/csrc/kernels.hip
@@ -361,7 +361,29 @@
   if (i < 4) lines[8 * (size_t)c + 2 * i] = base_vertex + (int)t, lines[8 * (size_t)c + 2 * i + 1] = base_vertex + (int)t + 1;
 }
 
+__global__ void k_light_constants(const yhd_scene sc, int lights, int environments, float* out) {
+  extern __shared__ v4f lds_dyn[];
+  trace_ctx tc;
+  tc.sc = &sc, tc.ls = nullptr, tc.sc_dev = nullptr, tc.stats = nullptr, tc.lds_stack = nullptr;
+  YH_LDS float* lds_cam;
+  stage_tables(sc, (YH_LDS v4f*)lds_dyn, threadIdx.x, blockDim.x, tc, lds_cam);
+  __syncthreads();
+  const f3    dir = f3{0.0f, 0.0f, 1.0f};
+  const float pdf = lights ? sample_lights_pdf<false, 128, false>(tc, mk3(0.0f), dir) : 0.0f;
+  const f3    e   = environments ? eval_environment<false, true>(tc, dir) : mk3(0.0f);
+  if (threadIdx.x == 0) out[0] = pdf, out[1] = e.x, out[2] = e.y, out[3] = e.z;
+}
+
 extern "C" {
+
+int yhk_light_constants(const yhd_scene* sc, int lights, int environments, float* out4, hipStream_t stream) {
+  const size_t lds = (size_t)YHD_LDS_TABLES_F4(sc) * 16;
+  if (lds > 64 * 1024) return (int)hipErrorInvalidValue;
+  yhd_scene walk = *sc;
+  walk.light_fold = 0;
+  hipLaunchKernelGGL(k_light_constants, dim3(1), dim3(64), lds, stream, walk, lights, environments, out4);
+  return (int)hipGetLastError();
+}
 
 trace_kernel_t yhk_wide_kernel(int counted, int general, int shape);
 #define YH_DENSE_WAVES 5
diff --git a/yocto-hair_amd/csrc/yh_device.h b/yocto-hair_amd/csrc/yh_device.h
--- a/yocto-hair_amd/csrc/yh_device.h
+++ b/yocto-hair_amd/csrc/yh_device.h
@@ -78,6 +78,9 @@
 } yhd_light;
 #define YH_SMALL_LIGHT_TRIS 4
 #define YH_SMALL_LIGHT_F4 15
+#define YH_LIGHT_DW 5
+#define YH_ENVIRONMENT_F4 8
+#define YHD_LIGHT_HEAD_F4(sc) (1 + (YH_LIGHT_DW * (sc)->num_lights + 3) / 4)
 
 typedef struct yhd_environment {
   float frame[12];
@@ -130,7 +133,13 @@
   int               stack_entries16;
   const yhd_float4* lane_blob;
   long long         lane_blob_units;
+  int               light_fold;
+  float             lights_const_pdf;
+  float             envs_const_emission[3];
+  int               pad_fold;
 } yhd_scene;
+#define YH_FOLD_LIGHTS 1
+#define YH_FOLD_ENVS 2
 #define YH_MATERIAL_F4 17
 #define YHD_LDS_TABLES_F4(sc) ((sc)->lds_scene_f4 + 5 + (sc)->light_table_f4 + ((sc)->env_tab_k + 3) / 4 + YH_MATERIAL_F4 * (sc)->lds_materials)
 
diff --git a/yocto-hair_amd/host/batch_api.cpp b/yocto-hair_amd/host/batch_api.cpp
--- a/yocto-hair_amd/host/batch_api.cpp
+++ b/yocto-hair_amd/host/batch_api.cpp
@@ -261,6 +261,26 @@
   HIPCHK(ctx, hipMemcpy(element, del, 4 * (size_t)n, hipMemcpyDeviceToHost));
   HIPCHK(ctx, hipMemcpy(uv, duv, 8 * (size_t)n, hipMemcpyDeviceToHost));
   HIPCHK(ctx, hipMemcpy(distance, dd, 4 * (size_t)n, hipMemcpyDeviceToHost));
+  return YH_OK;
+}
+
+int yh_light_constants(yh_context* ctx, int* folded, float* host4, float* device4) {
+  if (!ctx) return YH_E_INVALID;
+  if (!folded || !host4 || !device4) return fail(ctx, YH_E_INVALID, "yh_light_constants: NULL output");
+  if (!ctx->have_scene) return fail(ctx, YH_E_INVALID, "yh_light_constants before yh_upload_scene");
+  HIPCHK(ctx, hipSetDevice(ctx->device));
+  const yhd_scene& sc = ctx->scene;
+  const int lights = !sc.general_materials && (sc.light_fold & YH_FOLD_LIGHTS), envs = !sc.general_materials && (sc.light_fold & YH_FOLD_ENVS);
+  *folded  = (lights ? 1 : 0) | (envs ? 2 : 0);
+  host4[0] = lights ? sc.lights_const_pdf : 0.0f;
+  for (int c = 0; c < 3; c++) host4[1 + c] = envs ? sc.envs_const_emission[c] : 0.0f;
+  DevBuf out;
+  int    rc;
+  if ((rc = alloc_zero(ctx, out, 16))) return rc;
+  int e = yhk_light_constants(&sc, lights, envs, (float*)out.p, ctx->stream);
+  if (e) return fail(ctx, YH_E_DEVICE, "k_light_constants launch: %s", hipGetErrorString((hipError_t)e));
+  YH_WAIT(ctx);
+  HIPCHK(ctx, hipMemcpy(device4, out.p, 16, hipMemcpyDeviceToHost));
   return YH_OK;
 }
 
diff --git a/yocto-hair_amd/host/context_internal.h b/yocto-hair_amd/host/context_internal.h
--- a/yocto-hair_amd/host/context_internal.h
+++ b/yocto-hair_amd/host/context_internal.h
@@ -40,6 +40,7 @@
 int yhk_trace_sbs_occupancy(int lds_bytes, int general);
 int yhk_trace_lds_bytes(const yhd_scene* sc, int shape);
 int yhk_stack_entries(void);
+int yhk_light_constants(const yhd_scene* sc, int lights, int environments, float* out4, hipStream_t);
 int yhk_stream(const yhd_scene*, const yhd_scene* sc_dev, const yhd_state*, int, const yhd_stream*, int grid_blocks, hipStream_t);
 int yhk_lane_tests(const yhd_float4* prims, yhd_float4* blob, int kind, int prim_base, int num_prims, long long test_off, hipStream_t);
 int yhk_stream_block_threads(void);
@@ -300,5 +301,6 @@
 void destroy_communicators(yh_context* ctx);
 inline int tiles_of(int n) { return (n + YH_TILE - 1) / YH_TILE; }
 void make_material(const yh_material& m, yhd_material& d);
+void fold_light_constants(yhd_scene& sc);
 #pragma GCC visibility pop
 #endif
diff --git a/yocto-hair_amd/host/scene_upload.cpp b/yocto-hair_amd/host/scene_upload.cpp
--- a/yocto-hair_amd/host/scene_upload.cpp
+++ b/yocto-hair_amd/host/scene_upload.cpp
@@ -74,6 +74,25 @@
   d.tl_norm  = cb - ca;
 }
 
+
+void fold_light_constants(yhd_scene& sc) {
+  bool lights_const = sc.num_lights > 0, envs_const = true;
+  for (int k = 0; k < sc.num_lights; k++)
+    if (sc.lights[k].object >= 0 || sc.lights[k].environment < 0 || sc.environments[sc.lights[k].environment].tex_w != 0) lights_const = false;
+  float pdf = 0.0f;
+  for (int k = 0; k < sc.num_lights; k++) pdf += 1 / (4 * pif);
+  pdf *= (float)1 / (float)sc.num_lights;
+  F3 emission{0.0f, 0.0f, 0.0f};
+  for (int k = 0; k < sc.num_environments; k++) {
+    if (sc.environments[k].tex_w != 0) envs_const = false;
+    const float* e = sc.environments[k].emission;
+    emission       = emission + F3{e[0] * 1.0f, e[1] * 1.0f, e[2] * 1.0f};
+  }
+  sc.light_fold       = (lights_const ? YH_FOLD_LIGHTS : 0) | (envs_const ? YH_FOLD_ENVS : 0);
+  sc.lights_const_pdf = lights_const ? pdf : 0.0f;
+  st3(sc.envs_const_emission, envs_const ? emission : F3{0.0f, 0.0f, 0.0f});
+  sc.pad_fold = 0;
+}
 
 static bool has_effective_map(const yh_material_maps& m) {
   return m.specular_tex || m.metallic_tex || m.roughness_tex || m.opacity_tex || m.normal_tex;
@@ -465,7 +484,9 @@
     }
   }
   if (sc.num_lights == 0) return fail(ctx, YH_E_INVALID, "scene has no lights (the path sampler needs at least one)");
-  std::vector<yhd_float4> light_table;
+  static_assert(sizeof(yhd_light) == 4 * YH_LIGHT_DW && sizeof(yhd_environment) == 16 * YH_ENVIRONMENT_F4, "the light table's records");
+  const size_t light_head_f4 = (size_t)YHD_LIGHT_HEAD_F4(&sc) + (size_t)YH_ENVIRONMENT_F4 * sc.num_environments;
+  std::vector<yhd_float4> light_table(light_head_f4, yhd_float4{0, 0, 0, 0});
   for (int li : small_lights) {
     auto& L  = sc.lights[li];
     auto& I  = info[sd->objects[L.object].shape];
@@ -484,6 +505,10 @@
     for (int t = 0; t < L.cdf_count; t++) (&cdf.x)[t] = light_cdf[(size_t)L.cdf_base + t];
     light_table.push_back(cdf);
   }
+  fold_light_constants(sc);
+  light_table[0] = {sc.lights_const_pdf, sc.envs_const_emission[0], sc.envs_const_emission[1], sc.envs_const_emission[2]};
+  memcpy(&light_table[1], sc.lights, sizeof(yhd_light) * (size_t)sc.num_lights);
+  memcpy(&light_table[(size_t)YHD_LIGHT_HEAD_F4(&sc)], sc.environments, sizeof(yhd_environment) * (size_t)sc.num_environments);
   std::vector<float> env_tab;
   sc.env_tab_light = -1, sc.env_tab_k = 0, sc.env_tab_stride = 0;
   for (int li = 0; li < sc.num_lights && sc.env_tab_light < 0; li++) {
diff --git a/yocto-hair_amd/python/yhair_capi.py b/yocto-hair_amd/python/yhair_capi.py
--- a/yocto-hair_amd/python/yhair_capi.py
+++ b/yocto-hair_amd/python/yhair_capi.py
@@ -166,6 +166,7 @@
     "yh_hair_eval_pdf_batch": (C.c_int, [C.c_void_p, C.c_int, c_float_p, c_float_p, c_float_p, c_float_p]),
     "yh_intersect_batch": (C.c_int, [C.c_void_p, C.c_int, c_float_p, c_int_p, c_int_p, c_float_p, c_float_p]),
     "yh_selftest": (C.c_int, [C.c_void_p, C.c_int, c_float_p]),
+    "yh_light_constants": (C.c_int, [C.c_void_p, c_int_p, c_float_p, c_float_p]),
     "yh_scene_load": (C.c_void_p, [C.c_char_p, C.c_char_p, C.c_char_p, C.c_int]),
     "yh_scene_get": (C.POINTER(SceneDesc), [C.c_void_p]),
     "yh_scene_get_maps": (C.POINTER(MaterialMaps), [C.c_void_p]),
@@ -411,6 +412,12 @@
         self._chk(self.lib.yh_intersect_batch(self.h, n, fptr(rays), iptr(obj), iptr(elem), fptr(uv), fptr(dist)))
         return obj, elem, uv, dist
 
+    def light_constants(self):
+        folded = C.c_int()
+        host, dev = np.zeros(4, np.float32), np.zeros(4, np.float32)
+        self._chk(self.lib.yh_light_constants(self.h, C.byref(folded), fptr(host), fptr(dev)))
+        return folded.value, host, dev
+
     def selftest(self, which):
         worst = C.c_float()
         rc = self.lib.yh_selftest(self.h, which, C.byref(worst))
```

After: 2602 (median of 6 runs). No clear change (+0.7%).
